# lujiarui/Str2Str

Hardware: AMD Instinct MI355X
Metric: sampled conformations/sec (whole node), 256-res chain, 100 denoise steps (higher is better)
Workload: dtype f32 (matrix products on 2-way f16 split MFMA 'f16x3': 3 products per block, fp32 accumulate, fp32-equivalent); 1 GPU; configs[1]: single 256-residue synthetic chain, 128 replicas per GPU x 100 denoise steps (+1 self-conditioning forward), probability-flow ODE, seeded synthetic weights; n_res=256, replicas_per_gpu=128, denoise_steps=100, parallelism=replica-shard x1, arith=f16x3, rng=device

## Files before the change

str2str_amd/build.py:

```python
from __future__ import annotations

import os
import shutil
import subprocess
import sys
from concurrent.futures import ThreadPoolExecutor

HERE = os.path.dirname(os.path.abspath(__file__))
ROOT = os.path.dirname(HERE)
CSRC = os.path.join(HERE, "csrc")
OBJ = os.path.join(CSRC, "build")
LIB = os.path.join(HERE, "libstr2str_hip.so")

ARCH = "gfx950"
COMMON = ["-O3", "-std=c++17", "-fPIC", f"--offload-arch={ARCH}", "-I", os.path.join(ROOT, "include"), "-I", CSRC,
          "-Wno-unused-result"]
UNITS = {
    "abi.hip": [],
    "pdb_format.cpp": [],
    "host_rng.cpp": [],
    "rigid_kernels.hip": ["-ffp-contract=off"],
    "se3_step.hip": ["-ffp-contract=off"],
    "forward_marginal.hip": ["-ffp-contract=off"],
    "ensemble_metrics.hip": ["-ffp-contract=off"],
    "ensemble_rmsd.hip": [],
    "ensemble_tm.hip": [],
    "ensemble_pca.hip": [],
    "ensemble_tica.hip": [],
    "ensemble_cluster.hip": [],
    "ensemble_lddt.hip": [],
    "ensemble_contacts.hip": ["-ffp-contract=off"],
    "ensemble_violations.hip": ["-ffp-contract=off"],
    "ensemble_ss.hip": ["-ffp-contract=off"],
    "ensemble_sasa.hip": ["-ffp-contract=off"],
    "ensemble_saxs.hip": ["-ffp-contract=off"],
    "pair_mlp.hip": ["-mllvm", "-pragma-unroll-threshold=10000000"],
    "pair_mlp_f16.hip": ["-mllvm", "-pragma-unroll-threshold=10000000", "-fno-slp-vectorize"],
    "pair_mlp_f16_b.hip": ["-mllvm", "-pragma-unroll-threshold=10000000", "-fno-slp-vectorize"],
    "pair_mlp_f16_c.hip": ["-mllvm", "-pragma-unroll-threshold=10000000", "-fno-slp-vectorize"],
    "pair_mlp_f16_d.hip": ["-mllvm", "-pragma-unroll-threshold=10000000", "-fno-slp-vectorize"],
    "pair_embed_expand.hip": [],
    "ipa_attention.hip": ["-mllvm", "-pragma-unroll-threshold=10000000"],
    "ipa_attention_f16w.hip": ["-mllvm", "-pragma-unroll-threshold=10000000", "-fno-slp-vectorize"],
    "node_gemm.hip": ["-mllvm", "-pragma-unroll-threshold=10000000", "-fno-slp-vectorize"],
    "enc_attention.hip": ["-mllvm", "-pragma-unroll-threshold=10000000", "-ffp-contract=off", "-fno-slp-vectorize"],
}


def hipcc() -> str:
    for c in (os.environ.get("HIPCC"), shutil.which("hipcc"), "/opt/rocm/bin/hipcc"):
        if c and os.path.exists(c):
            return c
    raise RuntimeError("hipcc not found (set HIPCC)")


def _stale(out: str, deps) -> bool:
    if not os.path.exists(out):
        return True
    t = os.path.getmtime(out)
    return any(os.path.getmtime(d) > t for d in deps)


def build(force: bool = False, verbose: bool = True) -> str:
    os.makedirs(OBJ, exist_ok=True)
    cc = hipcc()
    headers = [os.path.join(CSRC, f) for f in os.listdir(CSRC) if f.endswith(".h")] + [
        os.path.join(ROOT, "include", "str2str_hip.h"), os.path.abspath(__file__)]

    def compile_one(item):
        src, extra = item
        s = os.path.join(CSRC, src)
        o = os.path.join(OBJ, os.path.splitext(src)[0] + ".o")
        inc = [os.path.join(CSRC, "pair_mlp_f16.hip")] if src.startswith("pair_mlp_f16_") else []
        if force or _stale(o, [s] + inc + headers):
            if src.endswith(".cpp"):
                cmd = [cc, "-x", "c++", "-c", s, "-o", o] + [c for c in COMMON if not c.startswith("--offload-arch")] + extra
            else:
                cmd = [cc, "-x", "hip", "-c", s, "-o", o] + COMMON + extra
            if verbose:
                print(" ".join(cmd), flush=True)
            subprocess.run(cmd, check=True)
        return o

    with ThreadPoolExecutor(max_workers=min(8, len(UNITS))) as ex:
        objs = list(ex.map(compile_one, UNITS.items()))
    for f in os.listdir(OBJ):
        if f.endswith(".o") and os.path.join(OBJ, f) not in objs:
            os.remove(os.path.join(OBJ, f))
    if force or _stale(LIB, objs):
        cmd = [cc, "-shared", "-fPIC", f"--offload-arch={ARCH}", "-o", LIB] + objs
        if verbose:
            print(" ".join(cmd), flush=True)
        subprocess.run(cmd, check=True)
    return LIB


if __name__ == "__main__":
    print(build(force="--force" in sys.argv))
```

str2str_amd/csrc/pair_embed_expand.hip:

```cpp
#include <hip/hip_runtime.h>

#include <cstdlib>

#include "edge_embed_class.h"
#include "str2str_hip.h"

namespace {

typedef float f32x4 __attribute__((ext_vector_type(4)));

template <bool PROJ>
__global__ void __launch_bounds__(256) edge_embed_expand_kernel(
    const float* __restrict__ table, const int* __restrict__ fixed_cls, const float* __restrict__ bin_lower,
    const long long* __restrict__ residue_idx, const float* __restrict__ ca, const float* __restrict__ mask,
    const float* __restrict__ proj_b, float* __restrict__ out, float* __restrict__ attn_bias, float* __restrict__ pair_z,
    long long M, int N, int rel_off, int n_rel, int n_bins, int out_tiled) {
    constexpr unsigned kRec = PROJ ? s2s::kEeRecProj : s2s::kEeRecPlain;
    __shared__ __attribute__((aligned(16))) float s_bins[s2s::kEeBinSlots];
    const unsigned lane = threadIdx.x & 63, h = lane >> 5, wave = threadIdx.x >> 6;
    s2s::ee_fill_bins(s_bins, bin_lower, n_bins);
    __syncthreads();
    const long long p0 = ((long long)blockIdx.x * 4 + wave) * 32;
    if (p0 >= M) return;
    long long pl = p0 + (lane & 31);
    const bool valid = pl < M;
    pl = valid ? pl : M - 1;
    const unsigned p = (unsigned)pl;
    const unsigned bi = p / (unsigned)N, j = p - bi * (unsigned)N, bb = bi / (unsigned)N, bj = bb * (unsigned)N + j;
    const int bin = s2s::ee_pair_bin(s_bins, n_bins, ca[bi * 3 + 0], ca[bi * 3 + 1], ca[bi * 3 + 2], ca[bj * 3 + 0], ca[bj * 3 + 1], ca[bj * 3 + 2]);
    const unsigned d = (unsigned)s2s::ee_rel_row(residue_idx[bi], residue_idx[bj], rel_off, n_rel);
    const unsigned row = s2s::ee_class_row((unsigned)fixed_cls[bi], (unsigned)fixed_cls[bj], d, bin, n_rel, n_bins);
    const float em = mask ? __fmul_rn(mask[bi], mask[bj]) : 1.0f;
    const float* rec = table + (unsigned long long)row * kRec;

    if (out_tiled) {
        float* o = out + (unsigned long long)(p0 >> 5) * 4096u + lane * 4u;
        f32x4 v[16];
#pragma unroll
        for (int g = 0; g < 16; ++g) v[g] = *reinterpret_cast<const f32x4*>(rec + 8 * g + 4 * h);
#pragma unroll
        for (int g = 0; g < 16; ++g) {
            const f32x4 w = {__fmul_rn(v[g].x, em), __fmul_rn(v[g].y, em), __fmul_rn(v[g].z, em), __fmul_rn(v[g].w, em)};
            __builtin_nontemporal_store(w, reinterpret_cast<f32x4*>(o + g * 256));
        }
    } else {
        const unsigned c = lane & 31;
        f32x4 v[16];
        float e[16];
#pragma unroll
        for (int it = 0; it < 16; ++it) {
            const int n = 2 * it + (int)h;
            const unsigned rn = (unsigned)__shfl((int)row, n, 64);
            e[it] = __shfl(em, n, 64);
            v[it] = *reinterpret_cast<const f32x4*>(table + (unsigned long long)rn * kRec + 4 * c);
        }
#pragma unroll
        for (int it = 0; it < 16; ++it) {
            const long long pn = p0 + 2 * it + h;
            const f32x4 w = {__fmul_rn(v[it].x, e[it]), __fmul_rn(v[it].y, e[it]), __fmul_rn(v[it].z, e[it]), __fmul_rn(v[it].w, e[it])};
            if (pn < M) __builtin_nontemporal_store(w, reinterpret_cast<f32x4*>(out + (unsigned long long)pn * 128u + 4 * c));
        }
    }
    if constexpr (PROJ) {
        {
            f32x4 a = *reinterpret_cast<const f32x4*>(rec + 128 + 4 * h);
            const f32x4 b = *reinterpret_cast<const f32x4*>(proj_b + 4 * h);
            a = em == 0.f ? b : a;
            const long long NN = (long long)N * N;
            float* o = attn_bias + ((unsigned long long)p + 7ull * bb * (unsigned long long)NN + 4ull * h * (unsigned long long)NN);
            if (valid) { o[0] = a.x; o[NN] = a.y; o[2 * NN] = a.z; o[3 * NN] = a.w; }
        }
        const unsigned c = lane & 7;
        const f32x4 b = *reinterpret_cast<const f32x4*>(proj_b + 8 + 4 * c);
#pragma unroll
        for (int it = 0; it < 4; ++it) {
            const int n = 8 * it + (int)(lane >> 3);
            const unsigned rn = (unsigned)__shfl((int)row, n, 64);
            const float en = __shfl(em, n, 64);
            f32x4 a = *reinterpret_cast<const f32x4*>(table + (unsigned long long)rn * kRec + 136 + 4 * c);
            a = en == 0.f ? b : a;
            const long long pn = p0 + n;
            if (pn < M) *reinterpret_cast<f32x4*>(pair_z + (unsigned long long)pn * 32u + 4 * c) = a;
        }
    }
}

long long tile_aligned_samples(long long NN) {
    long long q = 32;
    while (q > 1 && (NN * (32 / q)) % 32 != 0) q /= 2;
    return 32 / q;
}

}

extern "C" int s2s_edge_embed_expand(const float* table, const int* fixed_cls, const float* bin_lower, const long long* residue_idx,
                                     const float* ca_xyz, const float* mask, const float* proj_bias_cat64, float* out, int out_tiled,
                                     float* proj_attn_bias, float* proj_pair_z, int n_samples, int n_res, int rel_offset, int n_rel,
                                     int n_bins, void* stream) {
    if (n_samples <= 0 || n_res <= 0) return 0;
    if (n_bins < 1 || n_bins > 32 || (out_tiled & ~1) || n_rel < 1) return (int)hipErrorInvalidValue;
    if ((proj_attn_bias != nullptr) != (proj_pair_z != nullptr) || (proj_attn_bias && !proj_bias_cat64)) return (int)hipErrorInvalidValue;
    const long long NN = (long long)n_res * n_res;
    if (NN >= (1ll << 31)) return (int)hipErrorInvalidValue;
    const char* cap_env = getenv("S2S_EE_MAX_PAIRS");
    long long cap = cap_env ? atoll(cap_env) : 0;
    if (cap <= 0 || cap > (1ll << 31) - 1) cap = (1ll << 31) - 1;
    long long chunk = cap / NN;
    if (out_tiled && chunk < n_samples) chunk -= chunk % tile_aligned_samples(NN);
    if (chunk < 1) return (int)hipErrorInvalidValue;
    for (long long b0 = 0; b0 < n_samples; b0 += chunk) {
        const long long nb = n_samples - b0 < chunk ? n_samples - b0 : chunk;
        const long long M = nb * NN, rows0 = b0 * n_res;
        const unsigned grid = (unsigned)((M + 127) / 128);
        const float* mk = mask ? mask + rows0 : nullptr;
        if (proj_attn_bias)
            hipLaunchKernelGGL(edge_embed_expand_kernel<true>, dim3(grid), dim3(256), 0, (hipStream_t)stream, table, fixed_cls + rows0,
                               bin_lower, residue_idx + rows0, ca_xyz + rows0 * 3, mk, proj_bias_cat64, out + b0 * NN * 128, proj_attn_bias + b0 * 8 * NN,
                               proj_pair_z + b0 * NN * 32, M, n_res, rel_offset, n_rel, n_bins, out_tiled);
        else
            hipLaunchKernelGGL(edge_embed_expand_kernel<false>, dim3(grid), dim3(256), 0, (hipStream_t)stream, table, fixed_cls + rows0,
                               bin_lower, residue_idx + rows0, ca_xyz + rows0 * 3, mk, (const float*)nullptr, out + b0 * NN * 128, (float*)nullptr,
                               (float*)nullptr, M, n_res, rel_offset, n_rel, n_bins, out_tiled);
    }
    return (int)hipGetLastError();
}
```

str2str_amd/csrc/pair_mlp_f16.hip:

```cpp
#include <hip/hip_runtime.h>

#include <cstdlib>

#include "edge_embed_class.h"
#include "f16x3.h"
#include "range_flag.h"
#include "str2str_hip.h"

#ifndef S2S_PM_PART
#define S2S_PM_PART 1
#endif

namespace {

constexpr int kStageBytes = 32 * 1024;
constexpr int kStagesBase = 30;

__device__ __forceinline__ float relu1(float x) {
    float r;
    asm("v_max_f32 %0, 0, %1" : "=v"(r) : "v"(x));
    return r;
}

struct SlotDesc { int phase, t, a, b; };
constexpr SlotDesc slot_desc(int s) {
    if (s < 8) return {0, s / 4, s % 4, 0};
    if (s < 168) {
        const int tau = s - 8, blk = tau / 16, o = tau % 16;
        if (o < 12) return {1, blk, o / 6, o % 6};
        return {0, blk + 2, o - 12, 0};
    }
    if (s < 180) return {1, 10, (s - 168) / 6, (s - 168) % 6};
    if (s < 192) return {1, 11, (s - 180) % 2, (s - 180) / 2};

    if (s < 240) return {2, 0, (s - 192) / 2, (s - 192) % 2};
    return {3, 0, s - 240, 0};
}
constexpr int sched_slot(bool proj, int ns) { return !proj ? ns : (ns < 8 ? ns : (ns < 16 ? 240 + (ns - 8) : ns - 8)); }
constexpr int blob_stage(bool proj, int st) { return !proj ? st : (st == 0 ? 0 : (st == 1 ? 30 : st - 1)); }

#define S2S_LDS_BARRIER() asm volatile("s_waitcnt lgkmcnt(0)\n\ts_barrier" ::: "memory")
__device__ float s2s_one[1] = {1.0f};


template <bool PROJ, bool STAGE>
__global__ void __launch_bounds__(256) edge_transition_f16_kernel(
    const float* __restrict__ edge, const float* __restrict__ node_ab, const float* __restrict__ node_p,
    const char* __restrict__ wblob, const float* __restrict__ b2,
    const float* __restrict__ gamma, const float* __restrict__ beta, const float* __restrict__ mask,
    float* __restrict__ out, long long M, int N, float ln_eps, int io_layout, unsigned mask_stride, const float* __restrict__ proj_b,
    float* __restrict__ proj_bias_out, float* __restrict__ proj_pz_out, int* __restrict__ range_flag, float sk) {
    constexpr int kStages = kStagesBase + (PROJ ? 1 : 0);
    constexpr int kSlots = 8 * kStages;
    constexpr int kRing = PROJ ? 4 : 2, kAhead = PROJ ? 2 : 1;
    __shared__ __attribute__((aligned(16))) char s_w[kRing][kStageBytes];
    __shared__ __attribute__((aligned(16))) float s_vec[768 + 64];
    __shared__ __attribute__((aligned(16))) float s_rows[STAGE ? 4 * 2 * 384 : 4];
    const int lane = threadIdx.x & 63, h = lane >> 5, wave = threadIdx.x >> 6;

    const unsigned voff = wave * 8192 + lane * 16;
    typedef __attribute__((address_space(3))) char lds_char;
    lds_char* lds_image[2] = {(lds_char*)&s_w[0][lane * 16], (lds_char*)&s_w[kRing / 2][lane * 16]};
    asm volatile("" : "+v"(lds_image[0]), "+v"(lds_image[1]));
    auto ring_buf = [&](int r) -> lds_char* { return PROJ ? lds_image[r >> 1] + (r & 1) * kStageBytes : lds_image[r]; };
    const __amdgpu_buffer_rsrc_t wrsrc = __builtin_amdgcn_make_buffer_rsrc((void*)wblob, 0, kStages * kStageBytes, 0x00020000);
    auto ldw = [&](unsigned vo, int so) -> f32x4 {
        const u32x4 r = __builtin_amdgcn_raw_buffer_load_b128(wrsrc, vo, so, 0);
        return f32x4{__uint_as_float(r.x), __uint_as_float(r.y), __uint_as_float(r.z), __uint_as_float(r.w)};
    };
    f32x4 c0, c1, c2, c3;
    f32x4 e0, e1, e2, e3;
    typedef __attribute__((address_space(3))) f32x4 lds_f4;
    auto cp_load_a = [&](int stage) {
        const int so = blob_stage(PROJ, stage) * kStageBytes;
        c0 = ldw(voff, so); c1 = ldw(voff + 1024, so); c2 = ldw(voff + 2048, so); c3 = ldw(voff + 3072, so);
    };
    auto cp_load_b = [&](int stage) {
        const int so = blob_stage(PROJ, stage) * kStageBytes + 4096;
        e0 = ldw(voff, so); e1 = ldw(voff + 1024, so); e2 = ldw(voff + 2048, so); e3 = ldw(voff + 3072, so);
    };
    auto cp_store_a = [&](int par) {
        lds_char* d = ring_buf(par) + wave * 8192;
        *(lds_f4*)(d) = c0; *(lds_f4*)(d + 1024) = c1; *(lds_f4*)(d + 2048) = c2; *(lds_f4*)(d + 3072) = c3;
    };
    auto cp_store_b = [&](int par) {
        lds_char* d = ring_buf(par) + (wave * 8192 + 4096);
        *(lds_f4*)(d) = e0; *(lds_f4*)(d + 1024) = e1; *(lds_f4*)(d + 2048) = e2; *(lds_f4*)(d + 3072) = e3;
    };
    auto cp_load_piece = [&](auto grp, auto kc, int stage) {
        constexpr int k = decltype(kc)::value;
        const int so = blob_stage(PROJ, stage) * kStageBytes + (decltype(grp)::value ? 4096 : 0);
        const f32x4 v = ldw(voff + 1024 * k, so);
        if constexpr (decltype(grp)::value == 0) {
            if constexpr (k == 0) c0 = v; else if constexpr (k == 1) c1 = v; else if constexpr (k == 2) c2 = v; else c3 = v;
        } else {
            if constexpr (k == 0) e0 = v; else if constexpr (k == 1) e1 = v; else if constexpr (k == 2) e2 = v; else e3 = v;
        }
    };
    auto cp_store_piece = [&](auto grp, auto kc, int par) {
        constexpr int k = decltype(kc)::value;
        lds_char* d = ring_buf(par) + (wave * 8192 + (decltype(grp)::value ? 4096 : 0) + 1024 * k);
        if constexpr (decltype(grp)::value == 0)
            *(lds_f4*)(d) = k == 0 ? c0 : (k == 1 ? c1 : (k == 2 ? c2 : c3));
        else
            *(lds_f4*)(d) = k == 0 ? e0 : (k == 1 ? e1 : (k == 2 ? e2 : e3));
    };
    cp_load_a(0);
    cp_load_b(0);

    struct PairCtx {
        unsigned p, bi, bj, boff;
        unsigned r0, aoff;
        float em_i, em_j;
        bool valid;
    };
    const unsigned NNu = (unsigned)N * (unsigned)N;
    const long long NN = (long long)N * N;
    const unsigned n_magic = N >= 2 ? (unsigned)((1ull << 32) / (unsigned)N) : 0u;
    auto div_n = [&](unsigned x, unsigned& q, unsigned& r) {
        q = N >= 2 ? __umulhi(x, n_magic) : x;
        r = x - q * (unsigned)N;
        const bool fix = r >= (unsigned)N;
        q = fix ? q + 1 : q;
        r = fix ? r - (unsigned)N : r;
    };
    auto setup = [&](long long wg_tile) -> PairCtx {
        long long pl = (wg_tile * 4 + wave) * 32 + (lane & 31);
        PairCtx c;
        c.valid = pl < M;
        if (!c.valid) pl = M - 1;
        const unsigned p = (unsigned)pl;
        unsigned bi, j, bb, i;
        div_n(p, bi, j);
        div_n(bi, bb, i);
        c.p = p;
        c.bi = bi;
        c.bj = bb * (unsigned)N + j;
        c.r0 = (unsigned)__builtin_amdgcn_readfirstlane((int)bi);
        c.aoff = (unsigned)wave * 3072u + (bi != c.r0 ? 1536u : 0u) + 16u * (unsigned)h;
        c.boff = p + 7u * bb * NNu;
        c.em_i = mask[bi * mask_stride];
        c.em_j = mask[c.bj * mask_stride];
        return c;
    };
    const bool in_tiled = io_layout & 1, out_tiled = io_layout & 2, no_out = io_layout & 4;
    const int in_step = in_tiled ? 256 : 8, out_step = out_tiled ? 256 : 8;
    auto row_of = [&](const float* base, unsigned p, bool tiled) -> const float* {
        const unsigned blk = tiled ? p >> 5 : p, mul = tiled ? 4096u : 128u;
        const unsigned in_blk = tiled ? ((lane & 32) + (p & 31)) * 4 : 4 * h;
        return base + ((unsigned long long)blk * mul + in_blk);
    };
    auto erow_of = [&](const PairCtx& c) -> const float* { return row_of(edge, c.p, in_tiled); };
    auto ldrow = [&](const float* r, int g) -> float4 {
        const f32x4 v = __builtin_nontemporal_load(reinterpret_cast<const f32x4*>(r + g * in_step));
        return make_float4(v.x, v.y, v.z, v.w);
    };
    const long long n_wt = (M + 127) / 128;
    long long wt = blockIdx.x;
    PairCtx cur = setup(wt);

    f16x8 xpl[8][2];
    float amax = 0.f;
    const float inv1 = kInvWS * sk;
    auto split4 = [&](const float (&x)[4], f16x8& ph, f16x8& pm, int at) {
        split4_f16(x, ph, pm, at, amax);
    };
    {
        float4 xv[16];
#pragma unroll
        for (int i = 0; i < 16; ++i) xv[i] = ldrow(erow_of(cur), i);
        for (int i = threadIdx.x; i < 768; i += 256)
            s_vec[i] = i < 384 ? sk * b2[i] : (i < 512 ? 0.f : (i < 640 ? gamma[i - 512] : beta[i - 640]));
        if (PROJ && threadIdx.x < 64) s_vec[768 + threadIdx.x] = proj_b[threadIdx.x];
        cp_store_a(0);
        cp_load_a(1);
        cp_store_b(0);
        if constexpr (kAhead == 2) {
            cp_load_b(1);
            cp_store_a(1);
            cp_load_a(2);
            cp_store_b(1);
        }
#pragma unroll
        for (int i = 0; i < 16; ++i) {
            const float x[4] = {xv[i].x, xv[i].y, xv[i].z, xv[i].w};
            split4(x, xpl[i >> 1][0], xpl[i >> 1][1], 4 * (i & 1));
        }
    }

    f32x16 a1t[2];
    f32x16 a2[12];
    f32x16 a3[4];
    f32x16 pq[2];
    float sa[16];
    f32x4 g_st0, g_st1, g_st2;
    const unsigned n_node_rows = (unsigned)(M / N);
    auto stage_load = [&](const PairCtx& c) {
        if constexpr (STAGE) {
            const unsigned r1 = c.r0 + 1 < n_node_rows ? c.r0 + 1 : c.r0;
            auto piece = [&](int k) -> f32x4 {
                const unsigned o = (unsigned)k * 1024u + 16u * (unsigned)lane;
                const bool second = o >= 1536u;
                const float* src = node_ab + (unsigned long long)(second ? r1 : c.r0) * 896u + ((second ? o - 1536u : o) >> 2);
                const float4 v = *reinterpret_cast<const float4*>(src);
                return f32x4{v.x, v.y, v.z, v.w};
            };
            g_st0 = piece(0); g_st1 = piece(1); g_st2 = piece(2);
        }
    };
    auto stage_store = [&]() {
        if constexpr (STAGE) {
            typedef __attribute__((address_space(3))) f32x4 lds_v4;
            lds_v4* d = (lds_v4*)((__attribute__((address_space(3))) char*)s_rows + wave * 3072 + lane * 16);
            d[0] = g_st0; d[64] = g_st1; d[128] = g_st2;
        }
    };
    auto seeds_piece = [&](const PairCtx& c, int t, int rq) {
        if constexpr (STAGE) {
            const f32x4 x = *(const lds_f4*)((__attribute__((address_space(3))) const char*)s_rows + c.aoff + (32 * t + 8 * rq) * 4);
            sa[4 * rq + 0] = x[0]; sa[4 * rq + 1] = x[1]; sa[4 * rq + 2] = x[2]; sa[4 * rq + 3] = x[3];
        } else {
            const float4 x = ldg4(node_ab + (unsigned long long)c.bi * 896u + 32 * t, rq, h);
            sa[4 * rq + 0] = x.x; sa[4 * rq + 1] = x.y; sa[4 * rq + 2] = x.z; sa[4 * rq + 3] = x.w;
        }
    };
    auto seedc_piece = [&](const PairCtx& c, int t, int rq) {
        const float4 y = ldg4(node_ab + (unsigned long long)c.bj * 896u + 384 + 32 * t, rq, h);
        a1t[t & 1][4 * rq + 0] = y.x; a1t[t & 1][4 * rq + 1] = y.y; a1t[t & 1][4 * rq + 2] = y.z; a1t[t & 1][4 * rq + 3] = y.w;
    };
    auto seeds_load = [&](const PairCtx& c, int t) {
#pragma unroll
        for (int rq = 0; rq < 4; ++rq) seeds_piece(c, t, rq);
    };
    stage_load(cur);
    stage_store();
    seeds_load(cur, 0);
#pragma unroll
    for (int rq = 0; rq < 4; ++rq) { seedc_piece(cur, 0, rq); seedc_piece(cur, 1, rq); }

    f16x8 fr[2][4];
    f16x8 xp[2][2];
    auto fetch = [&](int par, int slot_in_stage, f16x8 (&f)[4]) {
        typedef __attribute__((address_space(3))) f16x8 lds_frag;
        const lds_frag* s = (const lds_frag*)ring_buf(par) + slot_in_stage * 4 * 64;
        f[0] = s[0]; f[2] = s[128]; f[3] = s[192]; f[1] = s[64];
    };
    auto s_quarter = [&](const f32x16& tile_acc, auto qc) {
        constexpr int qd = decltype(qc)::value;
        float x[4];
#pragma unroll
        for (int j = 0; j < 4; ++j) x[j] = fmaxf(__builtin_fmaf(tile_acc[4 * qd + j], inv1, sa[4 * qd + j]), 0.f);
        split4(x, xp[qd >> 1][0], xp[qd >> 1][1], 4 * (qd & 1));
    };
    auto s_half = [&](const f32x16& tile_acc, auto qc, auto hc) {
        constexpr int qd = decltype(qc)::value, j0 = 4 * qd + 2 * decltype(hc)::value;
        const float x0 = fmaxf(__builtin_fmaf(tile_acc[j0], inv1, sa[j0]), 0.f);
        const float x1 = fmaxf(__builtin_fmaf(tile_acc[j0 + 1], inv1, sa[j0 + 1]), 0.f);
        split2_f16(x0, x1, xp[qd >> 1][0], xp[qd >> 1][1], 4 * (qd & 1) + 2 * decltype(hc)::value, amax);
    };
    float rs[64];
    auto row_load2 = [&](const float* r, float (&dst)[64], int g0) {
#pragma unroll
        for (int g = g0; g < g0 + 2; ++g) {
            const float4 v = ldg4(r, g, h);
            dst[4 * g + 0] = v.x; dst[4 * g + 1] = v.y; dst[4 * g + 2] = v.z; dst[4 * g + 3] = v.w;
        }
    };
    const f32x16 zero16 = {0.f, 0.f, 0.f, 0.f, 0.f, 0.f, 0.f, 0.f, 0.f, 0.f, 0.f, 0.f, 0.f, 0.f, 0.f, 0.f};
    S2S_LDS_BARRIER();
    fetch(0, 0, fr[0]);

    PairCtx prv = cur;
    prv.valid = false;
    prv.em_i = 0.f;
    float ln_sum = 0.f, ln_var = 0.f, ln_mean = 0.f, ln_rstd = 0.f, ln_em = 0.f;
    float* ln_orow = out;
    f16x8 xln[8][2];
    auto ln_add = [&](auto qc) {
        constexpr int q = decltype(qc)::value, t = q / 4, rq = q % 4;
#pragma unroll
        for (int j = 0; j < 4; ++j) ln_sum += a3[t][4 * rq + j];
    };
    auto ln_dev = [&](auto qc) {
        constexpr int q = decltype(qc)::value, t = q / 4, rq = q % 4;
#pragma unroll
        for (int j = 0; j < 4; ++j) {
            const float dd = a3[t][4 * rq + j] - ln_mean;
            ln_var += dd * dd;
        }
    };
    auto ln_out = [&](auto qc, const float4& ga, const float4& be) {
        constexpr int q = decltype(qc)::value, t = q / 4, rq = q % 4;
        float4 o;
        o.x = ((a3[t][4 * rq + 0] - ln_mean) * ln_rstd * ga.x + be.x) * ln_em;
        o.y = ((a3[t][4 * rq + 1] - ln_mean) * ln_rstd * ga.y + be.y) * ln_em;
        o.z = ((a3[t][4 * rq + 2] - ln_mean) * ln_rstd * ga.z + be.z) * ln_em;
        o.w = ((a3[t][4 * rq + 3] - ln_mean) * ln_rstd * ga.w + be.w) * ln_em;
        if (prv.valid && !no_out) {
            __builtin_nontemporal_store(f32x4{o.x, o.y, o.z, o.w}, reinterpret_cast<f32x4*>(ln_orow + q * out_step));
        }
        if constexpr (PROJ) {
            const float x[4] = {o.x, o.y, o.z, o.w};
            split4(x, xln[2 * t + (rq >> 1)][0], xln[2 * t + (rq >> 1)][1], 4 * (rq & 1));
        }
    };
    auto proj_store = [&](auto gc) {
        constexpr int g = decltype(gc)::value;
        if (prv.valid) {
            const float4 bq = ldg4(s_vec + 768, g, h);
            if constexpr (g == 0) {
                float* o = proj_bias_out + ((unsigned long long)prv.boff + 4 * h * NN);
                o[0] = __builtin_fmaf(pq[0][0], kInvWS, bq.x);
                o[NN] = __builtin_fmaf(pq[0][1], kInvWS, bq.y);
                o[2 * NN] = __builtin_fmaf(pq[0][2], kInvWS, bq.z);
                o[3 * NN] = __builtin_fmaf(pq[0][3], kInvWS, bq.w);
            } else {
                constexpr int t = g >> 2, rq = g & 3;
                *reinterpret_cast<float4*>(proj_pz_out + (unsigned long long)prv.p * 32u + 8 * (g - 1) + 4 * h) =
                    make_float4(__builtin_fmaf(pq[t][4 * rq + 0], kInvWS, bq.x), __builtin_fmaf(pq[t][4 * rq + 1], kInvWS, bq.y),
                                __builtin_fmaf(pq[t][4 * rq + 2], kInvWS, bq.z), __builtin_fmaf(pq[t][4 * rq + 3], kInvWS, bq.w));
            }
        }
    };
#pragma unroll
    for (int t = 0; t < 4; ++t) a3[t] = zero16;

    constexpr int kHead = PROJ ? 16 : 15;
    long long wt_next = wt;
    bool has_next = false;
    PairCtx nxt = cur;
    float4 xv[16];
    f16x8 xpn[8][2];
    f16x8 xq[8][2];
    auto slot = [&](auto sc) {
        constexpr int ns = decltype(sc)::value;
        constexpr int s = sched_slot(PROJ, ns);
        constexpr SlotDesc d = slot_desc(s);
        constexpr int stage = ns / 8, ss = ns % 8, par = stage & (kRing - 1);
        constexpr int st_next = (stage + 1) % kStages, st_fill = (stage + kAhead) % kStages;
#ifdef S2S_ET_ALL_BARRIERS
        constexpr bool barrier_here = true;
#else
        constexpr bool barrier_here = !PROJ || (st_next & 1) == 0 || st_next == kStages - 2;
#endif

        if constexpr (ss < 7) {
            fetch(par, ss + 1, fr[(ns + 1) & 1]);
        } else {
            if constexpr (barrier_here) S2S_LDS_BARRIER();
            fetch(st_next & (kRing - 1), 0, fr[(ns + 1) & 1]);
        }
        constexpr int kXv0 = 208;
        if constexpr (s == kXv0) nxt = setup(has_next ? wt_next : wt);
        if constexpr (s == kXv0 + 3) stage_load(nxt);
        if constexpr (s == kXv0 + 8) stage_store();
        if constexpr (s > kXv0 && s <= kXv0 + 16 && ((s & 3) == 1 || (s & 3) == 2)) {
            constexpr int i = 4 * ((s - kXv0) / 4) + 2 * ((s & 3) - 1);
            const float* er = erow_of(nxt);
            xv[i] = ldrow(er, i);
            xv[i + 1] = ldrow(er, i + 1);
        }
        if constexpr (s == 236) seeds_load(nxt, 0);
        if constexpr (s == 237) { seedc_piece(nxt, 0, 0); seedc_piece(nxt, 0, 1); seedc_piece(nxt, 0, 2); seedc_piece(nxt, 0, 3); }
        if constexpr (s == 238) { seedc_piece(nxt, 1, 0); seedc_piece(nxt, 1, 1); seedc_piece(nxt, 1, 2); seedc_piece(nxt, 1, 3); }
        constexpr bool seeds_slot = d.phase == 1 && d.a == 1 && d.b == 0 && d.t + 1 < 12;
        if constexpr (s >= 184 && s < 192) row_load2(node_p + (unsigned long long)cur.bi * 128u, rs, 2 * (s - 184));
        constexpr int ep_blk = (s >= 184 && s < 192) ? 0 : ((s >= 192 && s < 224) ? 1 + (s - 192) / 16 : -1);
        constexpr int ep_q = ep_blk == 0 ? 2 * (s - 184) : (s - 192) % 16;
        float4 ep_b = {0.f, 0.f, 0.f, 0.f}, ep_b1 = {0.f, 0.f, 0.f, 0.f};
        if constexpr (ep_blk >= 0) ep_b = ldg4(s_vec + 128 * ep_blk, ep_q, h);
        if constexpr (ep_blk == 0) ep_b1 = ldg4(s_vec, ep_q + 1, h);
        constexpr int ln_k = ns == 7 ? 0 : ((PROJ && d.phase == 3 && d.a < 7) ? d.a + 1 : ((!PROJ && ns >= 8 && ns < 15) ? ns - 7 : -1));
        float4 lnv[4] = {};
        if constexpr (ln_k >= 0) {
#pragma unroll
            for (int k = 0; k < 2; ++k) { lnv[2 * k] = ldg4(s_vec + 512, 2 * ln_k + k, h); lnv[2 * k + 1] = ldg4(s_vec + 640, 2 * ln_k + k, h); }
        }
        constexpr int kGSlot = 182, kGPer = 2;
        if constexpr (s >= kGSlot && s < kGSlot + 16 / kGPer) {
#pragma unroll
            for (int u = 0; u < kGPer; ++u) {
                constexpr int p0 = (s - kGSlot) * kGPer;
                const int t3 = (p0 + u) / 4, rq = (p0 + u) % 4;
                const float4 v = ldg4(node_ab + (unsigned long long)cur.bj * 896u + 768 + 32 * t3, rq, h);
                a3[t3][4 * rq + 0] = v.x; a3[t3][4 * rq + 1] = v.y; a3[t3][4 * rq + 2] = v.z; a3[t3][4 * rq + 3] = v.w;
            }
        }
        __builtin_amdgcn_sched_barrier(0);

        const f16x8 (&f)[4] = fr[ns & 1];
        auto mfma_i = [&](auto ic) {
            constexpr int i = decltype(ic)::value;
            if constexpr (d.phase == 0) {
                f32x16& acc = a1t[d.t & 1];
                const f16x8 (&x)[2] = xpl[2 * d.a + (i >= 3)];
                constexpr int fa = (i == 0 ? 1 : (i < 3 ? 0 : (i == 3 ? 3 : 2))), xa = (i == 1 || i == 4) ? 1 : 0;
                acc = mfma_f16(f[fa], x[xa], acc);
            } else {
                constexpr bool fin = d.phase == 2, prj = d.phase == 3;
                constexpr bool first = i < 2 && (prj ? d.a == 0 : (fin ? false : (d.t == 0 && d.a == 0)));
                f32x16& t = prj ? pq[i & 1] : (fin ? a3[2 * d.b + (i & 1)] : a2[2 * d.b + (i & 1)]);
                const f16x8 (&x)[2] = prj ? xln[d.a] : (fin ? ((d.a >> 3) == 1 ? xq[d.a & 7] : xpl[d.a & 7]) : xp[d.a]);
                constexpr int fa = 2 * (i & 1) + (i < 2 ? 1 : 0), xa = (i == 2 || i == 3) ? 1 : 0;
                if constexpr (first) t = mfma_f16(f[fa], x[xa], zero16); else t = mfma_f16(f[fa], x[xa], t);
            }
        };
        auto ep_half = [&](auto qc, auto hc, const float4& bq) {
            constexpr int q = decltype(qc)::value, hh = decltype(hc)::value, t = q / 4, rq = q % 4, j0 = 4 * rq + 2 * hh, e0 = 4 * (rq & 1) + 2 * hh;
            const f32x16& a = a2[4 * (ep_blk < 0 ? 0 : ep_blk) + t];
            f16x8 (&P)[2] = ep_blk == 1 ? xq[2 * t + (rq >> 1)] : xpl[2 * t + (rq >> 1)];
            float r0 = 0.f, r1 = 0.f;
            if constexpr (ep_blk == 0) {
                const unsigned hw = __builtin_bit_cast(u32x4, P[0])[e0 / 2], lw = __builtin_bit_cast(u32x4, P[1])[e0 / 2];
                asm("v_fma_mix_f32 %0, %1, 1.0, %2 op_sel_hi:[1,0,1]" : "=v"(r0) : "v"(hw), "v"(lw));
                asm("v_fma_mix_f32 %0, %1, 1.0, %2 op_sel:[1,0,1] op_sel_hi:[1,0,1]" : "=v"(r1) : "v"(hw), "v"(lw));
            } else if constexpr (ep_blk == 1) {
                r0 = rs[16 * t + j0];
                r1 = rs[16 * t + j0 + 1];
            }
            float x0 = fmaxf(__builtin_fmaf(a[j0], kInvWS, hh ? bq.z : bq.x), 0.f), x1 = fmaxf(__builtin_fmaf(a[j0 + 1], kInvWS, hh ? bq.w : bq.y), 0.f);
            if constexpr (ep_blk != 2) {
                x0 = __builtin_fmaf(r0, sk, x0);
                x1 = __builtin_fmaf(r1, sk, x1);
            }
            split2_f16(x0, x1, P[0], P[1], e0, amax);
        };
        static_for<0, 6>([&](auto ic) {
            constexpr int i = decltype(ic)::value;
            mfma_i(ic);
            if constexpr (i < 4) {
                if constexpr (ss == 0) cp_load_piece(IC<1>{}, ic, st_fill);
                if constexpr (ss == 4) cp_load_piece(IC<0>{}, ic, (stage + kAhead + 1) % kStages);
                if constexpr (ss == 1) cp_store_piece(IC<0>{}, IC<3 - i>{}, st_fill & (kRing - 1));
                if constexpr (ss == 5) cp_store_piece(IC<1>{}, IC<3 - i>{}, st_fill & (kRing - 1));
            }
            if constexpr (seeds_slot && i < 4) seeds_piece(cur, d.t + 1, i);
            if constexpr (seeds_slot && i < 4 && d.t + 2 < 12) seedc_piece(cur, d.t + 2, i);
            if constexpr (d.phase == 0 && d.t >= 1 && (i == 2 || i == 4)) s_half(a1t[(d.t - 1) & 1], IC<d.a>{}, IC<(i - 2) / 2>{});
            if constexpr (ep_blk > 0 && (i == 2 || i == 4)) ep_half(IC<ep_q>{}, IC<(i - 2) / 2>{}, ep_b);
            if constexpr (ep_blk == 0 && i >= 1 && i <= 4) {
                if constexpr (i <= 2) ep_half(IC<ep_q>{}, IC<i - 1>{}, ep_b); else ep_half(IC<ep_q + 1>{}, IC<i - 3>{}, ep_b1);
            }
            if constexpr (s >= 228 && s < 236 && i >= 1 && i <= 4) {
                constexpr int k = s - 228, e = 2 * (i - 1);
                const float4 v = xv[2 * k + (e >> 2)];
                if constexpr ((e & 2) == 0) split2_f16(v.x, v.y, xpn[k][0], xpn[k][1], e, amax);
                else split2_f16(v.z, v.w, xpn[k][0], xpn[k][1], e, amax);
            }
            if constexpr (ns < 4 && i < 4) ln_add(IC<4 * ns + i>{});
            if constexpr (ns == 4 && i == 0) ln_mean = xhalf_sum(ln_sum) * (1.0f / 128);
            if constexpr ((ns == 4 || ns == 5) && (i == 1 || i == 3 || i == 5)) { ln_dev(IC<6 * (ns - 4) + i - 1>{}); ln_dev(IC<6 * (ns - 4) + i>{}); }
            if constexpr (ns == 6 && (i == 0 || i == 1)) { ln_dev(IC<12 + 2 * i>{}); ln_dev(IC<12 + 2 * i + 1>{}); }
            if constexpr (ns == 6 && i == 3) {
                ln_rstd = 1.0f / sqrtf(xhalf_sum(ln_var) * (1.0f / 128) + ln_eps * ((kWS * sk) * (kWS * sk)));
                ln_em = prv.em_i * prv.em_j;
                ln_orow = const_cast<float*>(row_of(out, prv.p, out_tiled));
                ln_sum = 0.f;
                ln_var = 0.f;
            }
            if constexpr (ln_k >= 0 && (i == 1 || i == 3)) ln_out(IC<2 * ln_k + (i - 1) / 2>{}, lnv[i - 1], lnv[i]);
            if constexpr (PROJ && ns == kHead && i < 5) proj_store(ic);
            __builtin_amdgcn_sched_barrier(0);
        });

        if constexpr (s == 179) {
            s_quarter(a1t[1], IC<0>{}); s_quarter(a1t[1], IC<1>{}); s_quarter(a1t[1], IC<2>{}); s_quarter(a1t[1], IC<3>{});
        }
    };
    for (;;) {
    wt_next = wt + gridDim.x;
    has_next = wt_next < n_wt;
    static_for<0, kSlots>(slot);

    prv = cur;
#pragma unroll
    for (int i = 0; i < 8; ++i) { xpl[i][0] = xpn[i][0]; xpl[i][1] = xpn[i][1]; }
    if (!has_next) break;
    cur = nxt;
    wt = wt_next;
    }
    static_for<0, kHead>(slot);
    if constexpr (PROJ) { proj_store(IC<0>{}); proj_store(IC<1>{}); proj_store(IC<2>{}); proj_store(IC<3>{}); proj_store(IC<4>{}); }
    s2s::range_report(range_flag, amax, s2s::kRangeEdgeTransition);
}


template <bool PROJ, bool TABLE = false>
__global__ void __launch_bounds__(256) edge_embed_f16_kernel(
    const float* __restrict__ node_a, const float* __restrict__ node_b, const float* __restrict__ rel_tab,
    const float* __restrict__ bin_tab, const float* __restrict__ bin_lower, const long long* __restrict__ residue_idx,
    const float* __restrict__ ca, const char* __restrict__ wblob, const float* __restrict__ b2, const float* __restrict__ b3,
    const float* __restrict__ gamma, const float* __restrict__ beta, const float* __restrict__ mask, float* __restrict__ out,
    long long M, int N, int rel_off, int n_rel, int n_bins, float ln_eps, int out_tiled, const float* __restrict__ proj_b,
    float* __restrict__ proj_bias_out, float* __restrict__ proj_pz_out, int* __restrict__ range_flag) {
    constexpr int kStages = PROJ ? 5 : 4;
    constexpr int kSlots = 8 * kStages;
    __shared__ __attribute__((aligned(16))) char s_w[2][kStageBytes];
    __shared__ __attribute__((aligned(16))) float s_vec[512 + 64];
    __shared__ __attribute__((aligned(16))) float s_bins[s2s::kEeBinSlots];
    const int lane = threadIdx.x & 63, h = lane >> 5, wave = threadIdx.x >> 6;

    const unsigned voff = wave * 8192 + lane * 16;
    typedef __attribute__((address_space(3))) char lds_char;
    lds_char* lds_image[2] = {(lds_char*)&s_w[0][lane * 16], (lds_char*)&s_w[1][lane * 16]};
    asm volatile("" : "+v"(lds_image[0]), "+v"(lds_image[1]));
    const __amdgpu_buffer_rsrc_t wrsrc = __builtin_amdgcn_make_buffer_rsrc((void*)wblob, 0, kStages * kStageBytes, 0x00020000);
    auto ldw = [&](unsigned vo, int so) -> f32x4 {
        const u32x4 r = __builtin_amdgcn_raw_buffer_load_b128(wrsrc, vo, so, 0);
        return f32x4{__uint_as_float(r.x), __uint_as_float(r.y), __uint_as_float(r.z), __uint_as_float(r.w)};
    };
    f32x4 c0, c1, c2, c3, e0, e1, e2, e3;
    typedef __attribute__((address_space(3))) f32x4 lds_f4;
    auto cp_load_a = [&](int stage) {
        const int so = stage * kStageBytes;
        c0 = ldw(voff, so); c1 = ldw(voff + 1024, so); c2 = ldw(voff + 2048, so); c3 = ldw(voff + 3072, so);
    };
    auto cp_load_b = [&](int stage) {
        const int so = stage * kStageBytes + 4096;
        e0 = ldw(voff, so); e1 = ldw(voff + 1024, so); e2 = ldw(voff + 2048, so); e3 = ldw(voff + 3072, so);
    };
    auto cp_store_a = [&](int par) {
        lds_char* d = lds_image[par] + wave * 8192;
        *(lds_f4*)(d + 3072) = c3; *(lds_f4*)(d + 2048) = c2; *(lds_f4*)(d + 1024) = c1; *(lds_f4*)(d) = c0;
    };
    auto cp_store_b = [&](int par) {
        lds_char* d = lds_image[par] + (wave * 8192 + 4096);
        *(lds_f4*)(d + 3072) = e3; *(lds_f4*)(d + 2048) = e2; *(lds_f4*)(d + 1024) = e1; *(lds_f4*)(d) = e0;
    };
    cp_load_a(0);
    cp_load_b(0);

    struct Ctx {
        const float* ra;
        unsigned vb, vr, vk;
        float kb;
        long long p, boff;
        float em;
        bool valid;
    };
    const long long NN = (long long)N * N;
    const __amdgpu_buffer_rsrc_t rs_b = __builtin_amdgcn_make_buffer_rsrc((void*)node_b, 0, (unsigned)((TABLE ? (long long)N : M / N) * 512), 0x00020000);
    const __amdgpu_buffer_rsrc_t rs_r = __builtin_amdgcn_make_buffer_rsrc((void*)rel_tab, 0, n_rel * 512, 0x00020000);
    const __amdgpu_buffer_rsrc_t rs_k = __builtin_amdgcn_make_buffer_rsrc((void*)bin_tab, 0, n_bins * 512, 0x00020000);
    struct Raw {
        long long p, bi, bj, bb;
        float ax, ay, az, bx, by, bz;
        long long ii, ij;
        float mi, mj;
        bool valid;
    };
    const unsigned n_magic = N >= 2 ? (unsigned)((1ull << 32) / (unsigned)N) : 0u;
    auto div_n = [&](unsigned x, unsigned& q, unsigned& r) {
        q = N >= 2 ? __umulhi(x, n_magic) : x;
        r = x - q * (unsigned)N;
        const bool fix = r >= (unsigned)N;
        q = fix ? q + 1 : q;
        r = fix ? r - (unsigned)N : r;
    };
    const float* mask_or_any = mask ? mask : ca;
    auto setup_a = [&](long long wg_tile) -> Raw {
        long long p = (wg_tile * 4 + wave) * 32 + (lane & 31);
        Raw r;
        r.valid = p < M;
        p = r.valid ? p : M - 1;
        r.p = p;
        if constexpr (TABLE) {
            const unsigned nb1 = (unsigned)n_bins + 1u, q = (unsigned)p / nb1, cls = q / (unsigned)n_rel;
            r.bi = cls >> 1; r.bj = cls & 1u; r.bb = 0;
            r.ii = q - cls * (unsigned)n_rel; r.ij = (unsigned)p - q * nb1;
            r.ax = r.ay = r.az = r.bx = r.by = r.bz = 0.f;
            r.mi = r.mj = 1.f;
            return r;
        }
        unsigned bi, j, bb, i;
        div_n((unsigned)p, bi, j);
        div_n(bi, bb, i);
        r.bi = bi; r.bb = bb; r.bj = bb * (unsigned)N + j;
        r.ax = ca[r.bi * 3 + 0]; r.ay = ca[r.bi * 3 + 1]; r.az = ca[r.bi * 3 + 2];
        r.bx = ca[r.bj * 3 + 0]; r.by = ca[r.bj * 3 + 1]; r.bz = ca[r.bj * 3 + 2];
        r.ii = residue_idx[r.bi];
        r.ij = residue_idx[r.bj];
        r.mi = mask_or_any[r.bi];
        r.mj = mask_or_any[r.bj];
        return r;
    };
    auto setup_b = [&](const Raw& r) -> Ctx {
        Ctx c;
        c.valid = r.valid;
        const int bin = TABLE ? (int)r.ij - 1 : s2s::ee_pair_bin(s_bins, n_bins, r.ax, r.ay, r.az, r.bx, r.by, r.bz);
        const long long d = TABLE ? r.ii : s2s::ee_rel_row(r.ii, r.ij, rel_off, n_rel);
        c.ra = node_a + r.bi * 128;
        const unsigned jj = (unsigned)(r.bj - r.bb * N);
        c.vb = ((unsigned)r.bb * 32u * (unsigned)N + (unsigned)h * (unsigned)N + jj) * 16u;
        c.vr = ((unsigned)h * (unsigned)n_rel + (unsigned)d) * 16u;
        c.vk = ((unsigned)h * (unsigned)n_bins + (unsigned)(bin < 0 ? 0 : bin)) * 16u;
        c.kb = bin < 0 ? 0.f : 1.f;
        c.p = r.p;
        c.boff = r.p + 7 * r.bb * NN;
        c.em = (!TABLE && mask) ? r.mi * r.mj : 1.0f;
        return c;
    };
    float amax = 0.f;
    auto split4 = [&](const float (&x)[4], f16x8& ph, f16x8& pm, int at) {
        split4_f16(x, ph, pm, at, amax);
    };
    float g1[64];
    auto row_set = [&](const float* r) {
#pragma unroll
        for (int G = 0; G < 16; ++G) {
            const float4 v = ldg4(r, G, h);
            g1[4 * G + 0] = v.x; g1[4 * G + 1] = v.y; g1[4 * G + 2] = v.z; g1[4 * G + 3] = v.w;
        }
    };
    float tmp[64];
    auto row_cb = [&](const __amdgpu_buffer_rsrc_t& rs, unsigned vo, int rows, float (&dst)[64], int G0, int G1) {
#pragma unroll
        for (int G = G0; G < G1; ++G) {
            const u32x4 v = __builtin_amdgcn_raw_buffer_load_b128(rs, vo, G * 32 * rows, 0);
            dst[4 * G + 0] = __uint_as_float(v.x); dst[4 * G + 1] = __uint_as_float(v.y);
            dst[4 * G + 2] = __uint_as_float(v.z); dst[4 * G + 3] = __uint_as_float(v.w);
        }
    };
    auto row_add = [&](float scale) {
#pragma unroll
        for (int i = 63; i >= 0; --i) {
            g1[i] = __fmaf_rn(scale, tmp[i], g1[i]);
            asm volatile("" : "+v"(g1[i]));
        }
    };
    auto g1_split = [&](f16x8 (&dst)[2], int ks) {
        const float x0[4] = {relu1(g1[8 * ks + 0]), relu1(g1[8 * ks + 1]), relu1(g1[8 * ks + 2]), relu1(g1[8 * ks + 3])};
        const float x1[4] = {relu1(g1[8 * ks + 4]), relu1(g1[8 * ks + 5]), relu1(g1[8 * ks + 6]), relu1(g1[8 * ks + 7])};
        split4(x0, dst[0], dst[1], 0);
        split4(x1, dst[0], dst[1], 4);
    };

    const long long n_wt = (M + 127) / 128;
    long long wt = blockIdx.x;
    if constexpr (!TABLE) s2s::ee_fill_bins(s_bins, bin_lower, n_bins);
    __syncthreads();
    Ctx cur = setup_b(setup_a(wt));
    f16x8 xp[8][2];
    {
        row_set(cur.ra);
        for (int i = threadIdx.x; i < 512; i += 256)
            s_vec[i] = i < 128 ? kWS * b2[i] : (i < 256 ? kWS * b3[i - 128] : (i < 384 ? gamma[i - 256] : beta[i - 384]));
        if (PROJ && threadIdx.x < 64) s_vec[512 + threadIdx.x] = proj_b[threadIdx.x];
        cp_store_a(0);
        cp_load_a(1);
        cp_store_b(0);
        row_cb(rs_b, cur.vb, N, tmp, 0, 16); row_add(1.0f);
        row_cb(rs_r, cur.vr, n_rel, tmp, 0, 16); row_add(1.0f);
        row_cb(rs_k, cur.vk, n_bins, tmp, 0, 16); row_add(cur.kb);
#pragma unroll
        for (int ks = 0; ks < 8; ++ks) g1_split(xp[ks], ks);
    }
    f32x16 a2[4], a3[4], pq[2];
    f16x8 fr[2][4];
    auto fetch = [&](int par, int slot_in_stage, f16x8 (&f)[4]) {
        typedef __attribute__((address_space(3))) f16x8 lds_frag;
        const lds_frag* s = (const lds_frag*)lds_image[par] + slot_in_stage * 4 * 64;
        f[0] = s[0]; f[2] = s[128]; f[3] = s[192]; f[1] = s[64];
    };
    const f32x16 zero16 = {0.f, 0.f, 0.f, 0.f, 0.f, 0.f, 0.f, 0.f, 0.f, 0.f, 0.f, 0.f, 0.f, 0.f, 0.f, 0.f};
    auto pin_frag = [&](f16x8 (&x)[2]) { asm volatile("" : "+v"(x[0]), "+v"(x[1])); };
    auto bias16 = [&](const float* vec, int t) -> f32x16 {
        const float4 b0 = ldg4(vec, 4 * t, h), b1 = ldg4(vec, 4 * t + 1, h), b2v = ldg4(vec, 4 * t + 2, h), b3v = ldg4(vec, 4 * t + 3, h);
        return f32x16{b0.x, b0.y, b0.z, b0.w, b1.x, b1.y, b1.z, b1.w, b2v.x, b2v.y, b2v.z, b2v.w, b3v.x, b3v.y, b3v.z, b3v.w};
    };
    auto l2_piece = [&](auto kc) {
        constexpr int k = decltype(kc)::value, t = k / 2;
#pragma unroll
        for (int u = 0; u < 2; ++u) {
            const int rq = 2 * (k & 1) + u;
            const float xx[4] = {relu1(a2[t][4 * rq + 0]) * kInvWS, relu1(a2[t][4 * rq + 1]) * kInvWS,
                                 relu1(a2[t][4 * rq + 2]) * kInvWS, relu1(a2[t][4 * rq + 3]) * kInvWS};
            split4(xx, xp[k][0], xp[k][1], 4 * u);
        }
        pin_frag(xp[k]);
    };
    float ln_mean = 0.f, ln_rstd = 0.f;
    constexpr unsigned kRec = TABLE ? (PROJ ? s2s::kEeRecProj : s2s::kEeRecPlain) : 128u;
    const unsigned out_lane = out_tiled ? lane * 16u : (unsigned)((lane & 31) * (kRec * 4) + h * 16), out_step = out_tiled ? 1024u : 32u;
    f16x8 xq[2][2];
    __amdgpu_buffer_rsrc_t rs_out;
    auto out_rsrc = [&](long long wg_tile) {
        const long long p0 = (wg_tile * 4 + __builtin_amdgcn_readfirstlane(wave)) * 32;
        const long long left = M - p0;
        rs_out = __builtin_amdgcn_make_buffer_rsrc((void*)(out + (p0 < M ? p0 : 0) * kRec), 0,
                                                   (unsigned)(left <= 0 ? 0 : (left < 32 && !out_tiled ? left : 32)) * (kRec * 4u), 0x00020000);
    };
    float4 lga[2], lbe[2];
    auto ln_load = [&](auto kc) {
        constexpr int k = decltype(kc)::value;
#pragma unroll
        for (int u = 0; u < 2; ++u) {
            const int g = 4 * (k / 2) + 2 * (k & 1) + u;
            lga[u] = ldg4(s_vec + 256, g, h);
            lbe[u] = ldg4(s_vec + 384, g, h);
        }
    };
    auto ln_piece = [&](auto kc, const Ctx& c) {
        constexpr int k = decltype(kc)::value, t = k / 2;
#pragma unroll
        for (int u = 0; u < 2; ++u) {
            const int rq = 2 * (k & 1) + u, g = 4 * t + rq;
            const float4 ga = lga[u], be = lbe[u];
            float4 o;
            o.x = __fmul_rn(__fmaf_rn(__fmul_rn(a3[t][4 * rq + 0] - ln_mean, ln_rstd), ga.x, be.x), c.em);
            o.y = __fmul_rn(__fmaf_rn(__fmul_rn(a3[t][4 * rq + 1] - ln_mean, ln_rstd), ga.y, be.y), c.em);
            o.z = __fmul_rn(__fmaf_rn(__fmul_rn(a3[t][4 * rq + 2] - ln_mean, ln_rstd), ga.z, be.z), c.em);
            o.w = __fmul_rn(__fmaf_rn(__fmul_rn(a3[t][4 * rq + 3] - ln_mean, ln_rstd), ga.w, be.w), c.em);
            __builtin_amdgcn_raw_buffer_store_b128(u32x4{__float_as_uint(o.x), __float_as_uint(o.y), __float_as_uint(o.z), __float_as_uint(o.w)},
                                                   rs_out, out_lane + (unsigned)g * out_step, 0, 0);
            if constexpr (PROJ) {
                const float xx[4] = {o.x, o.y, o.z, o.w};
                split4(xx, xq[k & 1][0], xq[k & 1][1], 4 * u);
            }
        }
        if constexpr (PROJ) pin_frag(xq[k & 1]);
    };
    auto row_load8 = [&](const float* r, float (&dst)[64], int half) {
#pragma unroll
        for (int G = 8 * half; G < 8 * half + 8; ++G) {
            const float4 v = ldg4(r, G, h);
            dst[4 * G + 0] = v.x; dst[4 * G + 1] = v.y; dst[4 * G + 2] = v.z; dst[4 * G + 3] = v.w;
        }
    };
    S2S_LDS_BARRIER();
    fetch(0, 0, fr[0]);
    f32x16 initA0 = bias16(s_vec, 0), initA1 = bias16(s_vec, 1), initB0, initB1;
    Raw nraw = setup_a(wt + gridDim.x < n_wt ? wt + gridDim.x : wt);

    for (;;) {
    const long long wt_next = wt + gridDim.x;
    const bool has_next = wt_next < n_wt;
    Ctx nxt = cur;
    f16x8 xl[2];
    static_for<0, kSlots>([&](auto sc) {
        constexpr int s = decltype(sc)::value;
        constexpr int stage = s / 8, ss = s % 8, par = stage & 1;
        constexpr int layer = s / 16;
        constexpr int ks = layer < 2 ? (s % 16) / 2 : s - 32;
        constexpr int pr = layer < 2 ? s % 2 : 0;
        if constexpr (s == kSlots - 1) { initA0 = bias16(s_vec, 0); initA1 = bias16(s_vec, 1); }
        if constexpr (s == 0) { initB0 = bias16(s_vec, 2); initB1 = bias16(s_vec, 3); }
        if constexpr (s == 15) { initA0 = bias16(s_vec + 128, 0); initA1 = bias16(s_vec + 128, 1); }
        if constexpr (s == 16) { initB0 = bias16(s_vec + 128, 2); initB1 = bias16(s_vec + 128, 3); }
        if constexpr (PROJ && s >= 31 && s < 39) ln_load(IC<s - 31>{});
        if constexpr (ss < 7) {
            fetch(par, ss + 1, fr[(s + 1) & 1]);
        } else {
            S2S_LDS_BARRIER();
            fetch(par ^ 1, 0, fr[(s + 1) & 1]);
        }
        if constexpr (s == 30) out_rsrc(wt);
        if constexpr (s == 5) row_load8(nxt.ra, g1, 0);
        if constexpr (s == 6) row_load8(nxt.ra, g1, 1);
        if constexpr (s == 7) row_cb(rs_b, nxt.vb, N, tmp, 0, 8);
        if constexpr (s == 8) row_cb(rs_b, nxt.vb, N, tmp, 8, 16);
        if constexpr (s == 13) row_cb(rs_r, nxt.vr, n_rel, tmp, 0, 8);
        if constexpr (s == 14) row_cb(rs_r, nxt.vr, n_rel, tmp, 8, 16);
        if constexpr (s == 18) row_cb(rs_k, nxt.vk, n_bins, tmp, 0, 8);
        if constexpr (s == 19) row_cb(rs_k, nxt.vk, n_bins, tmp, 8, 16);
        __builtin_amdgcn_sched_barrier(0);

        const f16x8 (&f)[4] = fr[s & 1];
        const f16x8 (&x)[2] = layer < 2 ? xp[ks] : xq[ks & 1];
        f32x16& t0 = layer == 0 ? a2[2 * pr] : (layer == 1 ? a3[2 * pr] : pq[0]);
        f32x16& t1 = layer == 0 ? a2[2 * pr + 1] : (layer == 1 ? a3[2 * pr + 1] : pq[1]);
        if constexpr (ks == 0) {
            if constexpr (layer < 2) {
                t0 = mfma_f16(f[1], x[0], pr == 0 ? initA0 : initB0); t1 = mfma_f16(f[3], x[0], pr == 0 ? initA1 : initB1);
            } else {
                t0 = mfma_f16(f[1], x[0], zero16); t1 = mfma_f16(f[3], x[0], zero16);
            }
        } else {
            t0 = mfma_f16(f[1], x[0], t0); t1 = mfma_f16(f[3], x[0], t1);
        }
        t0 = mfma_f16(f[0], x[1], t0); t1 = mfma_f16(f[2], x[1], t1);
        t0 = mfma_f16(f[0], x[0], t0); t1 = mfma_f16(f[2], x[0], t1);
        if constexpr (s == 1) nxt = setup_b(nraw);
        if constexpr (s == 26) nraw = setup_a(wt_next + gridDim.x < n_wt ? wt_next + gridDim.x : wt_next);
        if constexpr (s == 12) row_add(1.0f);
        if constexpr (s == 17) row_add(1.0f);
        if constexpr (s == 22) row_add(nxt.kb);
        if constexpr (s >= 16 && s <= 28 && s % 2 == 0) l2_piece(IC<(s - 14) / 2>{});
        if constexpr (s == 15) l2_piece(IC<0>{});
        if constexpr (s >= 24 && s < 31) { g1_split(xp[s - 24], s - 24); pin_frag(xp[s - 24]); }
        if constexpr (s == 23) { g1_split(xl, 7); pin_frag(xl); }
        if constexpr (PROJ && s >= 32 && s < 39) ln_piece(IC<s - 31>{}, cur);
        if constexpr (ss == 0) cp_load_b((stage + 1) % kStages);
        if constexpr (ss == 4) cp_load_a((stage + 2) % kStages);
        if constexpr (ss == 1) cp_store_a(par ^ 1);
        if constexpr (ss == 5) cp_store_b(par ^ 1);
        constexpr int copy_kind = (ss == 0 || ss == 4) ? 0x020 : ((ss == 1 || ss == 5) ? 0x200 : 0);
#pragma unroll
        for (int i = 0; i < 6; ++i) {
            __builtin_amdgcn_sched_group_barrier(0x008, 1, 0);
            if (copy_kind != 0 && i < 4) __builtin_amdgcn_sched_group_barrier(copy_kind, 1, 0);
            __builtin_amdgcn_sched_group_barrier(0x002, 8, 0);
        }
        __builtin_amdgcn_sched_barrier(0);

        if constexpr (s == 31) {
            float sum = 0.f;
#pragma unroll
            for (int t = 0; t < 4; ++t)
#pragma unroll
                for (int r = 0; r < 16; ++r) sum += a3[t][r];
            ln_mean = __fmul_rn(xhalf_sum(sum), 1.0f / 128);
            float var = 0.f;
#pragma unroll
            for (int t = 0; t < 4; ++t)
#pragma unroll
                for (int r = 0; r < 16; ++r) {
                    const float dd = a3[t][r] - ln_mean;
                    var = __fmaf_rn(dd, dd, var);
                }
            ln_rstd = 1.0f / sqrtf(__fmaf_rn(xhalf_sum(var), 1.0f / 128, ln_eps * (kWS * kWS)));
            if constexpr (PROJ) {
                ln_piece(IC<0>{}, cur);
            } else {
                static_for<0, 8>([&](auto kc) { ln_load(kc); ln_piece(kc, cur); });
            }
        }
    });
    if constexpr (PROJ) {
        if (cur.valid) {
            const float4 b0 = ldg4(s_vec + 512, 0, h);
            float* o = TABLE ? out + cur.p * kRec + 128 + 4 * h : proj_bias_out + cur.boff + 4 * h * NN;
            const long long hs = TABLE ? 1 : NN;
            float* pz = TABLE ? out + cur.p * kRec + 136 : proj_pz_out + cur.p * 32;
            o[0] = __builtin_fmaf(pq[0][0], kInvWS, b0.x);
            o[hs] = __builtin_fmaf(pq[0][1], kInvWS, b0.y);
            o[2 * hs] = __builtin_fmaf(pq[0][2], kInvWS, b0.z);
            o[3 * hs] = __builtin_fmaf(pq[0][3], kInvWS, b0.w);
#pragma unroll
            for (int g = 1; g <= 4; ++g) {
                const int t = g >> 2, rq = g & 3;
                const float4 bq = ldg4(s_vec + 512, g, h);
                *reinterpret_cast<float4*>(pz + 8 * (g - 1) + 4 * h) =
                    make_float4(__builtin_fmaf(pq[t][4 * rq + 0], kInvWS, bq.x), __builtin_fmaf(pq[t][4 * rq + 1], kInvWS, bq.y),
                                __builtin_fmaf(pq[t][4 * rq + 2], kInvWS, bq.z), __builtin_fmaf(pq[t][4 * rq + 3], kInvWS, bq.w));
            }
        }
    }
    if (!has_next) break;
    cur = nxt;
    wt = wt_next;
    xp[7][0] = xl[0]; xp[7][1] = xl[1];
    if constexpr (kStages % 2 == 1) {
        lds_char* sw = lds_image[0];
        lds_image[0] = lds_image[1];
        lds_image[1] = sw;
    }
    }
    s2s::range_report(range_flag, amax, s2s::kRangeEdgeEmbed);
}


long long tile_aligned_samples(long long NN) {
    long long q = 32;
    while (q > 1 && (NN * (32 / q)) % 32 != 0) q /= 2;
    return 32 / q;
}

int cu_count() {
    int dev = 0, n_cu = 0;
    if (hipGetDevice(&dev) != hipSuccess || hipDeviceGetAttribute(&n_cu, hipDeviceAttributeMultiprocessorCount, dev) != hipSuccess || n_cu <= 0)
        return 256;
    return n_cu;
}

template <bool STAGE>
int et_launch(const float* edge, const float* node_ab, const float* node_p, const void* weight_stream, const float* b2,
              const float* ln_gamma, const float* ln_beta, const float* mask, float* out, int n_samples, int n_res, float ln_eps,
              int io_layout, const float* proj_bias_cat64, float* proj_attn_bias, float* proj_pair_z, int prescale_exp, int* range_words,
              void* stream) {
    if (n_samples <= 0 || n_res <= 0) return 0;
    if ((io_layout & ~7) || ((io_layout & 4) && !proj_attn_bias) || (!(io_layout & 4) && !out)) return (int)hipErrorInvalidValue;
    if (prescale_exp < 0 || prescale_exp > 15) return (int)hipErrorInvalidValue;
    const float sk = ldexpf(1.0f, -prescale_exp);
    const long long NN = (long long)n_res * n_res;
    const char* cap_env = getenv("S2S_ET_MAX_PAIRS");
    long long cap = cap_env ? atoll(cap_env) : 0;
    if (cap <= 0 || cap > (1ll << 29) - 1) cap = (1ll << 29) - 1;
    long long chunk = cap / NN;
    if ((io_layout & 3) && chunk < n_samples) chunk -= chunk % tile_aligned_samples(NN);
    if (chunk < 1) return (int)hipErrorInvalidValue;
    const float* one = nullptr;
    if (hipGetSymbolAddress((void**)&one, HIP_SYMBOL(s2s_one)) != hipSuccess) return (int)hipErrorInvalidValue;
    const int n_cu = cu_count();
    for (long long b0 = 0; b0 < n_samples; b0 += chunk) {
        const long long nb = n_samples - b0 < chunk ? n_samples - b0 : chunk;
        const long long M = nb * NN, rows0 = b0 * n_res;
        const long long wg_tiles = (M + 127) / 128;
        const long long grid = wg_tiles < n_cu ? wg_tiles : n_cu;
        const float* e = edge + b0 * NN * 128;
        const float* nab = node_ab + rows0 * 896;
        const float* np = node_p + rows0 * 128;
        const float* mk = mask ? mask + rows0 : one;
        const unsigned mks = mask ? 1u : 0u;
        float* o = out ? out + b0 * NN * 128 : nullptr;
        auto k_proj = &edge_transition_f16_kernel<true, STAGE>;
        auto k_plain = &edge_transition_f16_kernel<false, STAGE>;
        if (proj_attn_bias)
            hipLaunchKernelGGL(k_proj, dim3((unsigned)grid), dim3(256), 0, (hipStream_t)stream, e, nab, np,
                               (const char*)weight_stream, b2, ln_gamma, ln_beta, mk, o, M, n_res, ln_eps, io_layout, mks, proj_bias_cat64,
                               proj_attn_bias + b0 * 8 * NN, proj_pair_z + b0 * NN * 32, range_words, sk);
        else
            hipLaunchKernelGGL(k_plain, dim3((unsigned)grid), dim3(256), 0, (hipStream_t)stream, e, nab, np,
                               (const char*)weight_stream, b2, ln_gamma, ln_beta, mk, o, M, n_res, ln_eps, io_layout, mks,
                               (const float*)nullptr, (float*)nullptr, (float*)nullptr, range_words, sk);
    }
    return (int)hipGetLastError();
}

}

#define S2S_ET_ARGS const float* edge, const float* node_ab, const float* node_p, const void* weight_stream, const float* b2, \
                    const float* ln_gamma, const float* ln_beta, const float* mask, float* out, int n_samples, int n_res, float ln_eps, \
                    int io_layout, const float* proj_bias_cat64, float* proj_attn_bias, float* proj_pair_z, int prescale_exp, \
                    int* range_words, void* stream
#define S2S_ET_PASS edge, node_ab, node_p, weight_stream, b2, ln_gamma, ln_beta, mask, out, n_samples, n_res, ln_eps, io_layout, \
                    proj_bias_cat64, proj_attn_bias, proj_pair_z, prescale_exp, range_words, stream
extern "C" __attribute__((visibility("hidden"))) int s2s_et_f16x3_short_chains(S2S_ET_ARGS);
#if S2S_PM_PART == 2
extern "C" int s2s_et_f16x3_short_chains(S2S_ET_ARGS) { return et_launch<false>(S2S_ET_PASS); }
#endif
#if S2S_PM_PART == 1
extern "C" int s2s_edge_transition_f16x3(S2S_ET_ARGS) {
    return n_res >= 32 ? et_launch<true>(S2S_ET_PASS) : s2s_et_f16x3_short_chains(S2S_ET_PASS);
}
#endif

#if S2S_PM_PART == 3
extern "C" int s2s_edge_embed_f16x3(const float* node_a, const float* node_b, const float* rel_table, const float* bin_table,
                                     const float* bin_lower, const long long* residue_idx, const float* ca_xyz,
                                     const void* weight_stream, const float* b2, const float* b3, const float* ln_gamma,
                                     const float* ln_beta, const float* mask, float* out, int n_samples, int n_res,
                                     int rel_offset, int n_rel, int n_bins, float ln_eps, int out_tiled, const float* proj_bias_cat64,
                                     float* proj_attn_bias, float* proj_pair_z, int* range_words, void* stream) {
    if (n_samples <= 0 || n_res <= 0) return 0;
    if (n_bins > 32 || (out_tiled & ~1)) return (int)hipErrorInvalidValue;
    const long long NN = (long long)n_res * n_res;
    if (NN >= (1ll << 31) || (long long)n_rel * 512 >= (1ll << 32)) return (int)hipErrorInvalidValue;
    const char* cap_env = getenv("S2S_EE_MAX_PAIRS");
    long long cap = cap_env ? atoll(cap_env) : 0;
    if (cap <= 0 || cap > (1ll << 31) - 1) cap = (1ll << 31) - 1;
    long long chunk = cap / NN;
    const long long rows_cap = ((1ll << 32) - 1) / ((long long)n_res * 512);
    if (rows_cap < chunk) chunk = rows_cap;
    if (out_tiled && chunk < n_samples) chunk -= chunk % tile_aligned_samples(NN);
    if (chunk < 1) return (int)hipErrorInvalidValue;
    const int n_cu = cu_count();
    for (long long b0 = 0; b0 < n_samples; b0 += chunk) {
        const long long nb = n_samples - b0 < chunk ? n_samples - b0 : chunk;
        const long long M = nb * NN, rows0 = b0 * n_res;
        const long long wg_tiles = (M + 127) / 128;
        const long long grid = wg_tiles < n_cu ? wg_tiles : n_cu;
        const float* na = node_a + rows0 * 128;
        const float* nbp = node_b + rows0 * 128;
        const long long* ridx = residue_idx + rows0;
        const float* cap = ca_xyz + rows0 * 3;
        const float* mk = mask ? mask + rows0 : nullptr;
        float* o = out + b0 * NN * 128;
        if (proj_attn_bias)
            hipLaunchKernelGGL(edge_embed_f16_kernel<true>, dim3((unsigned)grid), dim3(256), 0, (hipStream_t)stream, na, nbp,
                               rel_table, bin_table, bin_lower, ridx, cap, (const char*)weight_stream, b2, b3, ln_gamma, ln_beta,
                               mk, o, M, n_res, rel_offset, n_rel, n_bins, ln_eps, out_tiled, proj_bias_cat64,
                               proj_attn_bias + b0 * 8 * NN, proj_pair_z + b0 * NN * 32, range_words);
        else
            hipLaunchKernelGGL(edge_embed_f16_kernel<false>, dim3((unsigned)grid), dim3(256), 0, (hipStream_t)stream, na, nbp,
                               rel_table, bin_table, bin_lower, ridx, cap, (const char*)weight_stream, b2, b3, ln_gamma, ln_beta,
                               mk, o, M, n_res, rel_offset, n_rel, n_bins, ln_eps, out_tiled, (const float*)nullptr, (float*)nullptr,
                               (float*)nullptr, range_words);
    }
    return (int)hipGetLastError();
}
#endif

#if S2S_PM_PART == 4
extern "C" int s2s_edge_embed_classes_f16x3(const float* node_a2, const float* node_b2, const float* rel_table, const float* bin_table,
                                             const void* weight_stream, const float* b2, const float* b3, const float* ln_gamma,
                                             const float* ln_beta, float* table, int n_fixed, int n_rel, int n_bins, float ln_eps,
                                             const float* proj_bias_cat64, int* range_words, void* stream) {
    if (n_fixed < 1 || n_fixed > 2 || n_rel < 1 || n_bins < 1 || n_bins > 32) return (int)hipErrorInvalidValue;
    const long long M = (long long)(n_fixed == 2 ? 4 : 1) * n_rel * (n_bins + 1);
    if (M * s2s::kEeRecProj * 4 >= (1ll << 32) || (long long)n_rel * 512 >= (1ll << 32)) return (int)hipErrorInvalidValue;
    const long long wg_tiles = (M + 127) / 128;
    const int n_cu = cu_count();
    const long long grid = wg_tiles < n_cu ? wg_tiles : n_cu;
    if (proj_bias_cat64)
        hipLaunchKernelGGL((edge_embed_f16_kernel<true, true>), dim3((unsigned)grid), dim3(256), 0, (hipStream_t)stream, node_a2, node_b2,
                           rel_table, bin_table, (const float*)nullptr, (const long long*)nullptr, (const float*)nullptr,
                           (const char*)weight_stream, b2, b3, ln_gamma, ln_beta, (const float*)nullptr, table, M, n_fixed, 0, n_rel, n_bins,
                           ln_eps, 0, proj_bias_cat64, (float*)nullptr, (float*)nullptr, range_words);
    else
        hipLaunchKernelGGL((edge_embed_f16_kernel<false, true>), dim3((unsigned)grid), dim3(256), 0, (hipStream_t)stream, node_a2, node_b2,
                           rel_table, bin_table, (const float*)nullptr, (const long long*)nullptr, (const float*)nullptr,
                           (const char*)weight_stream, b2, b3, ln_gamma, ln_beta, (const float*)nullptr, table, M, n_fixed, 0, n_rel, n_bins,
                           ln_eps, 0, (const float*)nullptr, (float*)nullptr, (float*)nullptr, range_words);
    return (int)hipGetLastError();
}
#endif
```

str2str_amd/models/net/denoising_ipa.py:

```python
from __future__ import annotations

import math
import os
from functools import partial
from typing import Optional

import torch
import torch.nn.functional as F
from torch import nn

from ... import ops
from ...arith import default_arith
from ...common.all_atom import compute_backbone
from ...common.rigid_utils import Rigid
from .ipa import TranslationIPA
from .layers import DerivedCache, centred


def get_positional_embedding(indices: torch.Tensor, embedding_dim: int, max_len: int = 2056) -> torch.Tensor:
    K = torch.arange(embedding_dim // 2, device=indices.device)
    arg = indices[..., None] * math.pi / (max_len ** (2 * K[None] / embedding_dim))
    return torch.cat([torch.sin(arg), torch.cos(arg)], dim=-1)


def get_timestep_embedding(timesteps: torch.Tensor, embedding_dim: int, max_len: int = 10000) -> torch.Tensor:
    assert timesteps.ndim == 1
    timesteps = timesteps * max_len
    half = embedding_dim // 2
    freq = torch.exp(torch.arange(half, dtype=torch.float, device=timesteps.device) * -(math.log(max_len) / (half - 1)))
    emb = timesteps.float()[:, None] * freq[None, :]
    emb = torch.cat([torch.sin(emb), torch.cos(emb)], dim=1)
    if embedding_dim % 2 == 1:
        emb = F.pad(emb, (0, 1), mode="constant")
    return emb


class EmbeddingModule(nn.Module):
    launch_switches = ("arith", "node_arith")
    launch_modes = ("ee_classes",)

    def __init__(self, init_embed_size: int, node_embed_size: int, edge_embed_size: int, num_bins: int = 22,
                 min_bin: float = 1e-5, max_bin: float = 20.0, self_conditioning: bool = True):
        super().__init__()
        pos_embed_size = t_embed_size = init_embed_size
        node_in = t_embed_size + 1 + pos_embed_size
        edge_in = (t_embed_size + 1) * 2 + pos_embed_size
        self.node_embed = nn.Sequential(
            nn.Linear(node_in, node_embed_size), nn.ReLU(), nn.Linear(node_embed_size, node_embed_size), nn.ReLU(),
            nn.Linear(node_embed_size, node_embed_size), nn.LayerNorm(node_embed_size),
        )
        self.self_conditioning = self_conditioning
        if self_conditioning:
            edge_in += num_bins
        self.edge_embed = nn.Sequential(
            nn.Linear(edge_in, edge_embed_size), nn.ReLU(), nn.Linear(edge_embed_size, edge_embed_size), nn.ReLU(),
            nn.Linear(edge_embed_size, edge_embed_size), nn.LayerNorm(edge_embed_size),
        )
        self.time_embed = partial(get_timestep_embedding, embedding_dim=t_embed_size)
        self.position_embed = partial(get_positional_embedding, embedding_dim=pos_embed_size)
        self._dims = (init_embed_size, num_bins, float(min_bin), float(max_bin), edge_embed_size)
        self._wcache, self._w16cache, self._proj_cache, self._idx_cache, self._fixed_cache = (DerivedCache() for _ in range(5))
        self.arith = default_arith()
        self.node_arith = default_arith()
        self.ee_classes = os.environ.get("S2S_EE_CLASSES", "auto")
        if self.ee_classes not in ("auto", "0", "1"):
            raise ValueError(f"S2S_EE_CLASSES={self.ee_classes!r}: expected auto, 0 or 1")
        self._mask01_cache = DerivedCache()

    def _weights(self):
        e0, e2, e4 = self.edge_embed[0], self.edge_embed[2], self.edge_embed[4]
        ie, nb = self._dims[0], self._dims[1]
        t1 = ie + 1

        def build():
            w0 = e0.weight.float()
            n0 = self.node_embed[0]
            wn = n0.weight.float()
            out = {
                "w_row_t": w0[:, :ie].contiguous(), "w_row_f": w0[:, ie].contiguous(),
                "w_col_t": w0[:, t1:t1 + ie].contiguous(), "w_col_f": w0[:, t1 + ie].contiguous(),
                "w_rel": w0[:, 2 * t1:2 * t1 + ie].contiguous(), "b0": e0.bias.float().contiguous(),
                "wn_t": wn[:, :ie].contiguous(), "wn_f": wn[:, ie].contiguous(), "wn_pos": wn[:, t1:t1 + ie].contiguous(),
                "bn0": n0.bias.float().contiguous(),
                "w_t_cat": torch.cat([wn[:, :ie], w0[:, :ie], w0[:, t1:t1 + ie]], dim=0).contiguous(),
                "b_t_cat": torch.cat([n0.bias.float(), e0.bias.float(), torch.zeros_like(e0.bias.float())]).contiguous(),
                "w3c": centred(e4.weight), "b3c": centred(e4.bias),
                "w2p": ops.pack_weight(e2.weight.float()), "w3p": ops.pack_weight(centred(e4.weight)),
                "node_mlp": [ops.pack_node_layer(self.node_embed[2].weight, self.node_embed[2].bias),
                             ops.pack_node_layer(self.node_embed[4].weight, self.node_embed[4].bias, True)],
            }
            if self.self_conditioning:
                out["bin_tab"] = w0[:, 2 * t1 + ie:2 * t1 + ie + nb].t().contiguous()
            else:
                out["bin_tab"] = w0.new_zeros(1, w0.shape[0])
            out["bin_tab_cb"] = ops.column_blocked(out["bin_tab"])
            out["bin_lower"] = torch.linspace(self._dims[2], self._dims[3], nb).to(w0.device)
            return out

        ne = self.node_embed
        return self._wcache.get([e0.weight, e0.bias, e2.weight, e4.weight, e4.bias, ne[0].weight, ne[0].bias, ne[2].weight, ne[2].bias,
                                 ne[4].weight, ne[4].bias], build)

    def _fixed_terms(self, fixed_mask: torch.Tensor, w: dict, dev, node_pos: torch.Tensor):
        def build():
            fixed = fixed_mask.to(dev)[..., None].float()
            B, L = fixed.shape[:2]
            vals = torch.unique(fixed).cpu().tolist()
            cls = None
            if vals and all(v in (0.0, 1.0) for v in vals):
                f2 = torch.tensor(vals, device=dev, dtype=torch.float32).view(1, -1, 1)
                cls = {"n_fixed": len(vals),
                       "fixed_cls": ((fixed[..., 0] > 0) if len(vals) == 2 else torch.zeros_like(fixed[..., 0])).to(torch.int32).contiguous(),
                       "fa2": (f2 * w["w_row_f"]).contiguous(),
                       "fb2": (f2[:, None] * w["w_col_f"].view(1, 32, 1, 4)).expand(1, 32, len(vals), 4).contiguous(),
                       "nc2": torch.zeros(len(vals), w["wn_f"].shape[0], device=dev)}
            return ((fixed * w["wn_f"] + node_pos).contiguous(), (fixed * w["w_row_f"]).contiguous(),
                    ((fixed[:, None] * w["w_col_f"].view(1, 32, 1, 4)).expand(B, 32, L, 4).contiguous(), (fixed * w["w_col_f"]).contiguous()), cls)

        return self._fixed_cache.get([fixed_mask, w["wn_f"], node_pos], build)

    def _mask_is_01(self, node_mask: Optional[torch.Tensor]) -> bool:
        if node_mask is None:
            return True
        return self._mask01_cache.get([node_mask], lambda: (bool(((node_mask == 0) | (node_mask == 1)).all()),))[0]

    def time_images(self, t_emb: torch.Tensor) -> torch.Tensor:
        w = self._weights()
        t_emb = t_emb.to(w["b0"].device).reshape(-1, t_emb.shape[-1]).float()
        return ((w["w_t_cat"][None] * t_emb[:, None, :]).sum(-1) + w["b_t_cat"]).contiguous()

    def _index_tables(self, residue_idx: torch.Tensor, w_rel: torch.Tensor, wn_pos: torch.Tensor):
        return self._tables(residue_idx, w_rel, wn_pos)[:4]

    def _tables(self, residue_idx, w_rel, wn_pos):
        def build():
            idx_cpu = residue_idx.detach().cpu()
            span = int(idx_cpu.max() - idx_cpu.min())
            d = torch.arange(-span, span + 1)
            dev = w_rel.device
            rel = _table_linear(self.position_embed(d).float().to(dev), w_rel)
            node_pos = _table_linear(self.position_embed(idx_cpu).float().to(dev), wn_pos)
            return rel, span, node_pos, residue_idx.to(dev).contiguous(), ops.column_blocked(rel)

        return self._idx_cache.get([residue_idx, w_rel, wn_pos], build)

    def forward(self, *args, **kw):
        node_embed, _, edge_embed, proj = self.embed(*args, **kw)
        return (node_embed, edge_embed) if proj is None else (node_embed, edge_embed, proj)

    def embed(self, residue_idx, t, fixed_mask, self_conditioning_ca, node_mask: Optional[torch.Tensor] = None,
              next_proj=None, t_emb: Optional[torch.Tensor] = None, edge_layout: str = "rowmajor", t_img: Optional[torch.Tensor] = None):
        w = self._weights()
        dev = w["b0"].device
        if dev.type != "cuda":
            raise ops.HipLibraryError("EmbeddingModule runs on the HIP device only (no CPU fallback)")
        if self._dims[4] != 128:
            raise ops.HipLibraryError("edge_embed kernel is built for edge_embed_size=128")
        B, L = residue_idx.shape
        rel_tab, span, node_pos, idx_dev, rel_cb = self._tables(residue_idx, w["w_rel"], w["wn_pos"])
        if t_img is not None:
            t_emb = None
        elif t_emb is not None:
            t_emb = t_emb.to(dev).reshape(-1, t_emb.shape[-1])
        else:
            t_u, t_inv = torch.unique(t.detach().reshape(-1), return_inverse=True)
            t_emb = self.time_embed(t_u)[t_inv].to(dev)
        ne = self.node_embed
        mask = None if node_mask is None else node_mask.to(dev).float().contiguous()
        nn_, ne_ = w["wn_t"].shape[0], w["w_row_t"].shape[0]
        single_t = t_img is not None or t_emb.shape[0] == 1
        M = B * L
        f16 = self.arith == "f16x3"
        cls = None
        if single_t:
            per_sample = t_img is not None and t_img.ndim == 2 and t_img.shape[0] == B and B > 1
            img = (t_img if per_sample else t_img.reshape(-1)) if t_img is not None else (w["w_t_cat"] * t_emb).sum(-1) + w["b_t_cat"]
            Fn, Fa, Fb, cls = self._fixed_terms(fixed_mask, w, dev, node_pos)
            h_act, node_a, node_b = torch.ops.str2str_amd.embed_assemble(img.contiguous(), Fn, Fa, Fb[0] if f16 else Fb[1], B, L,
                                                                         self.node_arith == "f16x3", f16)
        else:
            fixed = fixed_mask.to(dev)[..., None].float()
            tl = lambda wt, b=None: _table_linear(t_emb, wt, b)
            h = F.relu(tl(w["wn_t"], w["bn0"])[:, None, :] + fixed * w["wn_f"] + node_pos)
            h_act = ops.to_act(h.reshape(M, -1).contiguous(), self.node_arith)
        nw = w["node_mlp"]
        node_embed, node_act = ops.node_apply_chain(h_act, nw, M, (True, False), ln=(ne[5].weight, ne[5].bias, ne[5].eps),
                                                          post_mask=None if mask is None else mask.reshape(M), want_xp=True)
        node_embed = node_embed.view(B, L, -1)
        if not single_t:
            node_a = (tl(w["w_row_t"], w["b0"])[:, None, :] + fixed * w["w_row_f"]).expand(B, L, -1).contiguous()
            if f16:
                node_b = (tl(w["w_col_t"]).view(-1, 32, 1, 4) + fixed[:, None] * w["w_col_f"].view(1, 32, 1, 4)).expand(B, 32, L, 4).contiguous()
            else:
                node_b = (tl(w["w_col_t"])[:, None, :] + fixed * w["w_col_f"]).expand(B, L, -1).contiguous()
        ca = self_conditioning_ca.to(dev).float().contiguous() if self.self_conditioning else node_a.new_zeros(B, L, 3)
        e2, e4, ln = self.edge_embed[2], self.edge_embed[4], self.edge_embed[5]
        if f16:
            e2w = e2.weight
            ws = self._w16cache.get([e2w, w["w3c"]], lambda: ops.pack_f16x3_embed_stream(e2w.float(), w["w3c"]))
            proj = None
            if next_proj is not None:
                stream = self._proj_cache.get([ws, next_proj["wp_f16x2"]], lambda: torch.cat([ws, next_proj["wp_f16x2"]]))
                proj = (stream, next_proj["b64"])
            by_class = cls is not None and ops.edge_embed_classes_eligible(
                self.ee_classes, self.arith, single_t and not per_sample, cls["n_fixed"], self._mask_is_01(node_mask), rel_cb.shape[1],
                w["bin_tab_cb"].shape[1], B, L)
            if by_class:
                _, node_a2, node_b2 = torch.ops.str2str_amd.embed_assemble(img.contiguous(), cls["nc2"], cls["fa2"], cls["fb2"], 1,
                                                                           cls["n_fixed"], False, True)
                edge_embed = ops.edge_embed_classes_f16x3(node_a2, node_b2, cls["fixed_cls"], rel_cb, w["bin_tab_cb"], w["bin_lower"], idx_dev,
                                                          ca, ws, e2.bias, w["b3c"], ln.weight, ln.bias, mask, span, ln.eps, proj=proj,
                                                          out_layout=edge_layout)
            else:
                edge_embed = ops.edge_embed_f16x3(node_a, node_b, rel_cb, w["bin_tab_cb"], w["bin_lower"], idx_dev, ca, ws, e2.bias,
                                                  w["b3c"], ln.weight, ln.bias, mask, span, ln.eps, proj=proj, column_blocked_tables=True,
                                                  out_layout=edge_layout)
        else:
            if edge_layout != "rowmajor":
                raise ops.HipLibraryError("EmbeddingModule: the tiled pair layout belongs to the f16x3 kernels")
            edge_embed = ops.edge_embed(node_a, node_b, rel_tab, w["bin_tab"], w["bin_lower"], idx_dev, ca, w["w2p"],
                                        w["w3p"], e2.bias, w["b3c"], ln.weight, ln.bias, mask, span, ln.eps,
                                        proj=None if next_proj is None else (next_proj["wp"], next_proj["b64"]))
        if next_proj is not None:
            edge_embed, *proj = edge_embed
            return node_embed, node_act, edge_embed, tuple(proj)
        return node_embed, node_act, edge_embed, None


def _table_linear(x: torch.Tensor, w: torch.Tensor, b: Optional[torch.Tensor] = None) -> torch.Tensor:
    layer = ops.pack_node_layer(w, b if b is not None else torch.zeros(w.shape[0], device=w.device))
    lead, n = x.shape[:-1], x.numel() // x.shape[-1]
    y, _ = ops.node_apply(x.reshape(n, x.shape[-1]).float().contiguous(), layer, n)
    return y[:, : w.shape[0]].reshape(*lead, w.shape[0]).contiguous()


class DenoisingNet(nn.Module):
    def __init__(self, embedder: nn.Module, translator: nn.Module):
        super().__init__()
        self.embedder = embedder
        self.translator = translator
        self.backbone_in_forward = True

    @staticmethod
    def blend_psi(psi: torch.Tensor, torsion_angles_sin_cos: torch.Tensor, fixed_mask: torch.Tensor) -> torch.Tensor:
        gt_psi = torsion_angles_sin_cos.to(psi.device)[..., 2, :]
        fixed_mask = fixed_mask.to(psi.device).type(torch.float)
        return gt_psi * fixed_mask[..., None] + psi * (1 - fixed_mask[..., None])

    def forward(self, batch: dict, as_tensor_7: bool = False, defer_psi_blend: bool = False) -> dict:
        dev = next(self.parameters()).device
        if dev.type != "cuda":
            raise ops.HipLibraryError(
                "DenoisingNet.forward needs the HIP device (MI355X): the sampling path has no CPU fallback")
        node_mask = batch["residue_mask"].to(dev).type(torch.float)
        fixed_mask = batch["fixed_mask"].to(dev).type(torch.float)
        fuse = getattr(self.translator, "fuse_pair_projection", False)
        et0 = self.translator.trunk["edge_transition_0"] if "edge_transition_0" in getattr(self.translator, "trunk", {}) else None
        tiled = fuse and getattr(self.embedder, "arith", None) == "f16x3" and getattr(et0, "arith", None) == "f16x3"
        node_embed, node_act, edge_embed, first_proj = self.embedder.embed(
            residue_idx=batch["residue_idx"], t=batch["t"], fixed_mask=fixed_mask, self_conditioning_ca=batch["sc_ca_t"], node_mask=node_mask,
            t_emb=batch.get("t_emb"), t_img=batch.get("t_img"), next_proj=self.translator.trunk["ipa_0"].pair_proj_weights() if fuse else None,
            **({"edge_layout": "tiled"} if tiled else {}))
        tb = dict(batch)
        tb["residue_mask"], tb["fixed_mask"] = node_mask, fixed_mask
        tb["rigids_t"] = batch["rigids_t"].to(dev)
        tb["_node_embed_act"] = node_act
        model_out = self.translator(node_embed, edge_embed, tb, **({"_first_proj": first_proj} if fuse else {}))
        if model_out.get("psi_blended") or defer_psi_blend:
            psi_pred = model_out["psi"]
        else:
            psi_pred = self.blend_psi(model_out["psi"], batch["torsion_angles_sin_cos"], fixed_mask)
        rigids_pred = model_out["out_rigids"]
        out = {"rigids": rigids_pred, "psi": psi_pred, "rigids7": model_out["out_rigids7"]}
        if defer_psi_blend and not model_out.get("psi_blended"):
            out["psi_deferred"] = True
        if self.backbone_in_forward:
            aatype = batch["aatype"].to(dev) if "aatype" in batch else None
            bb = compute_backbone(rigids_pred, psi_pred, aatype=aatype, _rigids7=model_out["out_rigids7"])
            out["atom37"], out["atom14"] = bb[0], bb[-1]
        if as_tensor_7:
            out["rigids"] = model_out["out_rigids7"]
        return out
```

str2str_amd/models/net/ipa.py:

```python
from __future__ import annotations

import math
import os
from typing import Optional

import torch
import torch.nn as nn
import torch.nn.functional as F

from ... import ops
from ...arith import default_arith
from ...common.rigid_utils import Rigid, Rotation
from .layers import BackboneUpdate, DerivedCache, EdgeTransition, Linear, NodeTransition, TorsionAngleHead


class InvariantPointAttention(nn.Module):
    launch_switches = ("arith", "fold")

    def __init__(self, c_s: int, c_z: int, c_hidden: int, no_heads: int, no_qk_points: int, no_v_points: int,
                 inf: float = 1e5, eps: float = 1e-8):
        super().__init__()
        self.c_s, self.c_z, self.c_hidden = c_s, c_z, c_hidden
        self.no_heads, self.no_qk_points, self.no_v_points = no_heads, no_qk_points, no_v_points
        self.inf, self.eps = inf, eps
        hc = c_hidden * no_heads
        self.linear_q = Linear(c_s, hc)
        self.linear_kv = Linear(c_s, 2 * hc)
        self.linear_q_points = Linear(c_s, no_heads * no_qk_points * 3)
        self.linear_kv_points = Linear(c_s, no_heads * (no_qk_points + no_v_points) * 3)
        self.linear_b = Linear(c_z, no_heads)
        self.down_z = Linear(c_z, c_z // 4)
        self.head_weights = nn.Parameter(torch.full((no_heads,), 0.541324854612918))
        self.linear_out = Linear(no_heads * (c_z // 4 + c_hidden + no_v_points * 4), c_s, init="final")
        self.softmax = nn.Softmax(dim=-1)
        self.softplus = nn.Softplus()
        self.arith = default_arith()
        self.fold = os.environ.get("S2S_IPA_FOLD", "1") != "0"
        self._last_folded = False
        self._cache, self._packs = DerivedCache(), DerivedCache()

    def _derived(self):
        def build():
            wcat = torch.cat([self.linear_b.weight, self.down_z.weight], dim=0).float()
            bcat = torch.cat([self.linear_b.bias, self.down_z.bias]).float()
            b64 = bcat.new_zeros(64)
            b64[: bcat.numel()] = bcat
            hw = F.softplus(self.head_weights.float()) * math.sqrt(1.0 / (3 * (self.no_qk_points * 9.0 / 2)))
            wcat64 = wcat.new_zeros(64, wcat.shape[1])
            wcat64[: wcat.shape[0]] = wcat
            return ops.LazyDict({"wp": ops.pack_weight(wcat), "b64": b64.contiguous(), "hw": hw.contiguous()},
                                wp_f16x2=lambda d: ops.pack_f16x2_layer(wcat64, "chain").reshape(-1).view(torch.int16).contiguous())

        return self._cache.get([self.linear_b.weight, self.linear_b.bias, self.down_z.weight, self.down_z.bias,
                                self.head_weights], build)

    def node_packs(self):
        def build():
            H, C = self.no_heads, self.c_hidden
            pk = ops.pack_node_layer
            wkv = self.linear_kv.weight.view(H, 2, C, -1)
            bkv = self.linear_kv.bias.view(H, 2, C)
            d = {"q": pk(self.linear_q.weight, self.linear_q.bias), "kv": pk(self.linear_kv.weight, self.linear_kv.bias),
                 "k": pk(wkv[:, 0].reshape(H * C, -1), bkv[:, 0].reshape(-1)),
                 "v": pk(wkv[:, 1].reshape(H * C, -1), bkv[:, 1].reshape(-1)),
                 "qp": pk(self.linear_q_points.weight, self.linear_q_points.bias),
                 "kvp": pk(self.linear_kv_points.weight, self.linear_kv_points.bias),
                 "out": pk(self.linear_out.weight, self.linear_out.bias, True)}
            if self.c_s == C:
                d.update(self._folded_packs(wkv, bkv))
            return d

        return self._packs.get([p for lin in (self.linear_q, self.linear_kv, self.linear_q_points, self.linear_kv_points,
                                              self.linear_out) for p in (lin.weight, lin.bias)], build)

    def _folded_packs(self, wkv, bkv):
        H, C, cs = self.no_heads, self.c_hidden, self.c_s
        dev = self.linear_q.weight.device
        c64 = lambda t: t.detach().double().cpu()
        wq, bq = c64(self.linear_q.weight).view(H, C, cs), c64(self.linear_q.bias).view(H, C)
        wk, wv, bv = c64(wkv[:, 0]), c64(wkv[:, 1]), c64(bkv[:, 1])
        w_qf = torch.einsum("hca,hcb->hab", wk, wq).reshape(H * cs, cs).float().to(dev)
        b_qf = torch.einsum("hca,hc->ha", wk, bq).reshape(-1).float().to(dev)
        wo = c64(self.linear_out.weight)
        wo_o = wo[:, : H * C].view(-1, H, C)
        w_of = torch.cat([torch.einsum("ohc,hca->oha", wo_o, wv).reshape(-1, H * cs), wo[:, H * C:]], dim=1).float().to(dev)
        b_of = (c64(self.linear_out.bias) + torch.einsum("ohc,hc->o", wo_o, bv)).float().to(dev)
        return {"qf": ops.pack_node_layer(w_qf, b_qf), "outf": ops.pack_node_layer(w_of, b_of, True)}

    def use_f16(self, n_res: int, n_rows: int = 0) -> bool:
        if self.arith != "f16x3":
            return False
        shape_ok = (self.c_hidden == 256 and self.no_qk_points == 8 and self.no_v_points == 12 and self.c_z // 4 == 32
                    and self.no_heads == 8)
        rows_pad = (n_rows // max(n_res, 1)) * ops.padded_len(n_res)
        return shape_ok and rows_pad * 12288 < (1 << 32) and (n_res % 32 == 0 or n_rows * n_res * 32 < (1 << 31))

    def attention_f16(self, s_xp, B: int, N: int, r7, mask, pair_proj):
        w, d, M, H = self.node_packs(), self._derived(), B * N, self.no_heads
        if self.folded:
            return self._attention_f16_folded(s_xp, B, N, r7, mask, pair_proj, w, d)
        if w["v"]["tg"] != 8:
            raise ops.HipLibraryError("s2s_node_linear_vfrag is instantiated for 8 tiles per column block")
        NP = ops.padded_len(N)
        rmap, Mo = ((NP, N), B * NP) if NP != N else (None, M)
        K = torch.ops.str2str_amd
        names = ("q", "k", "v", "qp", "kvp")
        var = {n: (("w", w[n]["tg"]) if n == "v" else ops.small_rows_variant(w[n], M)) for n in names}
        dims = [x for n in names for x in (w[n]["k"], w[n]["n"], var[n][1])]
        q_xp, k_xp, v_vf, qp, kvp = K.ipa_projections(s_xp, *[[w[n][var[n][0]], w[n]["b"]] for n in names], dims, M, Mo, *(rmap or (0, 0)))
        pts = K.ipa_prep_points_f16(r7.view(B, N, 7), qp, kvp, d["hw"], H, self.no_qk_points, self.no_v_points, self.c_hidden)
        attn_bias, pair_z = pair_proj
        feats, feats_xp = K.ipa_attention_f16w(q_xp, k_xp, v_vf, *pts, attn_bias, pair_z, mask, r7, H, self.c_hidden,
                                               self.no_qk_points, self.no_v_points, self.c_z // 4, self.inf, self.eps, True)
        c0 = H * self.c_hidden
        f2 = feats.view(M, -1)
        K.pack_planes(f2, c0, f2.shape[1] - c0, feats_xp, f2.shape[1], c0)
        return feats_xp

    def _attention_f16_folded(self, s_xp, B, N, r7, mask, pair_proj, w, d):
        M, H = B * N, self.no_heads
        NP = ops.padded_len(N)
        rmap, Mo = ((NP, N), B * NP) if NP != N else (None, M)
        K = torch.ops.str2str_amd
        names = ("qf", "qp", "kvp")
        var = {n: ops.small_rows_variant(w[n], M) for n in names}
        dims = [x for n in ("qf", None, None, "qp", "kvp") for x in ((w[n]["k"], w[n]["n"], var[n][1]) if n else (0, 0, 0))]
        q_xp, _, _, qp, kvp = K.ipa_projections(s_xp, [w["qf"][var["qf"][0]], w["qf"]["b"]], [], [], [w["qp"][var["qp"][0]], w["qp"]["b"]],
                                                [w["kvp"][var["kvp"][0]], w["kvp"]["b"]], dims, M, Mo, *(rmap or (0, 0)))
        *pts, k_sh, v_sh = K.ipa_prep_points_shared_kv(r7.view(B, N, 7), qp, kvp, d["hw"], s_xp, H, self.no_qk_points, self.no_v_points,
                                                       self.c_hidden)
        attn_bias, pair_z = pair_proj
        feats, feats_xp = K.ipa_attention_f16w(q_xp, s_xp if k_sh is None else k_sh, v_sh, *pts, attn_bias, pair_z, mask, r7, H,
                                               self.c_hidden, self.no_qk_points, self.no_v_points, self.c_z // 4, self.inf, self.eps, True)
        c0 = H * self.c_hidden
        f2 = feats.view(M, -1)
        K.pack_planes(f2, c0, f2.shape[1] - c0, feats_xp, f2.shape[1], c0)
        return feats_xp

    @property
    def folded(self) -> bool:
        return self.fold and self.c_s == self.c_hidden and self.no_heads == 8

    def out_pack(self, feats_a) -> dict:
        w = self.node_packs()
        return w["outf"] if (self.folded and self._last_folded) else w["out"]

    def attention_f32(self, s_act, B: int, N: int, r7, mask, pair_proj):
        w, d, M, H = self.node_packs(), self._derived(), B * N, self.no_heads
        lin = lambda x: ops.node_apply(s_act, x, M)[0]
        q, kv, qp, kvp = lin(w["q"]), lin(w["kv"]), lin(w["qp"]), lin(w["kvp"])
        q_pts, k_pts, v_pts = torch.ops.str2str_amd.ipa_prep_points(r7.view(B, N, 7), qp.view(B, N, -1), kvp.view(B, N, -1), H,
                                                                    self.no_qk_points, self.no_v_points)
        attn_bias, pair_z = pair_proj
        feats = ops.ipa_attention(q.view(B, N, H, -1), kv.view(B, N, H, -1), q_pts, k_pts, v_pts, attn_bias, pair_z, mask, r7,
                                  d["hw"], H, self.c_hidden, self.no_qk_points, self.no_v_points, self.c_z // 4, self.inf,
                                  self.eps, logits_inplace=True)
        return ops.pack_planes(feats.view(M, -1)) if s_act.dtype == torch.int16 else feats.view(M, -1)

    def attention(self, s_act, B: int, N: int, r7, mask, pair_proj):
        self._last_folded = False
        if s_act.dtype == torch.int16 and self.use_f16(N, B * N):
            self._last_folded = self.folded
            return self.attention_f16(s_act, B, N, r7, mask, pair_proj)
        return self.attention_f32(s_act, B, N, r7, mask, pair_proj)

    def pair_proj_weights(self):
        return self._derived()

    def forward(self, s: torch.Tensor, z: torch.Tensor, r, mask: torch.Tensor, _rigids7: Optional[torch.Tensor] = None,
                _pair_proj=None):
        if not s.is_cuda:
            raise ops.HipLibraryError("InvariantPointAttention runs on the HIP device only (no CPU fallback)")
        if self.no_heads != 8 or self.c_z != 128:
            raise ops.HipLibraryError("IPA kernels are built for the reference configuration (H=8, c_z=128)")
        d = self._derived()
        r7 = (_rigids7 if _rigids7 is not None else r.to_tensor_7()).type(torch.float32).contiguous()
        mask = mask.type(torch.float32).contiguous()
        B, N = s.shape[:2]
        pp = _pair_proj if _pair_proj is not None else ops.pair_project(z.contiguous(), d["wp"], d["b64"])
        feats_a = self.attention(ops.to_act(s.reshape(B * N, -1).float().contiguous(), self.arith), B, N, r7, mask, pp)
        out, _ = ops.node_apply(feats_a, self.out_pack(feats_a), B * N)
        return out.view(B, N, -1)


class TranslationIPA(nn.Module):
    launch_switches = ("exact_padding", "fuse_pair_projection", "arith")

    def __init__(self, c_s: int, c_z: int, coordinate_scaling: float, no_ipa_blocks: int, skip_embed_size: int,
                 transformer_num_heads: int = 4, transformer_num_layers: int = 2, c_hidden: int = 256, no_heads: int = 8,
                 no_qk_points: int = 8, no_v_points: int = 12, dropout: float = 0.0):
        super().__init__()
        self.coordinate_scaling = coordinate_scaling
        self.scale_pos = lambda x: x * coordinate_scaling
        self.scale_rigids = lambda x: x.apply_trans_fn(self.scale_pos)
        self.unscale_pos = lambda x: x / coordinate_scaling
        self.unscale_rigids = lambda x: x.apply_trans_fn(self.unscale_pos)
        self.trunk = nn.ModuleDict()
        self.num_blocks = no_ipa_blocks
        for b in range(no_ipa_blocks):
            self.trunk[f"ipa_{b}"] = InvariantPointAttention(c_s=c_s, c_z=c_z, c_hidden=c_hidden, no_heads=no_heads,
                                                            no_qk_points=no_qk_points, no_v_points=no_v_points)
            self.trunk[f"ipa_ln_{b}"] = nn.LayerNorm(c_s)
            self.trunk[f"skip_embed_{b}"] = Linear(c_s, skip_embed_size, init="final")
            d = c_s + skip_embed_size
            layer = nn.TransformerEncoderLayer(d_model=d, nhead=transformer_num_heads, dim_feedforward=d)
            self.trunk[f"transformer_{b}"] = nn.TransformerEncoder(layer, transformer_num_layers, enable_nested_tensor=False)
            self.trunk[f"linear_{b}"] = Linear(d, c_s, init="final")
            self.trunk[f"node_transition_{b}"] = NodeTransition(c_s)
            self.trunk[f"bb_update_{b}"] = BackboneUpdate(c_s)
            if b < no_ipa_blocks - 1:
                self.trunk[f"edge_transition_{b}"] = EdgeTransition(node_embed_size=c_s, edge_embed_in=c_z,
                                                                    edge_embed_out=c_z)
        self.torsion_pred = TorsionAngleHead(c_s, 1)
        self._wcache, self._mask_cache = DerivedCache(), DerivedCache()
        self.exact_padding = False
        self.fuse_pair_projection = True
        self.arith = default_arith()

    def _node_weights(self):
        def build():
            T = self.trunk
            pk = lambda lin, whole=False: ops.pack_node_layer(lin.weight, lin.bias, whole)
            out = {}
            for b in range(self.num_blocks):
                d = {"skip": pk(T[f"skip_embed_{b}"]), "lin": pk(T[f"linear_{b}"]), "bb": pk(T[f"bb_update_{b}"].linear)}
                nt = T[f"node_transition_{b}"]
                d["nt1"], d["nt2"], d["nt3"] = pk(nt.linear_1), pk(nt.linear_2), pk(nt.linear_3, True)
                d["layers"] = []
                for layer in T[f"transformer_{b}"].layers:
                    att = layer.self_attn
                    d["layers"].append({"in": ops.pack_node_layer(att.in_proj_weight, att.in_proj_bias), "o": pk(att.out_proj, True),
                                        "l1": pk(layer.linear1), "l2": pk(layer.linear2, True)})
                out[b] = d
            tp = self.torsion_pred
            out["tor"] = {"l1": pk(tp.linear_1), "l2": pk(tp.linear_2), "fin": pk(tp.linear_final)}
            return out

        return self._wcache.get(list(self.parameters()), build)

    def _mask_terms(self, residue_mask: torch.Tensor, fixed_mask: torch.Tensor):
        def build():
            node_mask = residue_mask.type(torch.float).contiguous()
            fixed = fixed_mask.type(torch.float).contiguous()
            diffuse_mask = ((1 - fixed) * node_mask).contiguous()
            pad = 1.0 - node_mask
            key_bias = (torch.where(pad > 0, float("-inf"), 0.0) if self.exact_padding else pad).float().contiguous()
            return node_mask, diffuse_mask, key_bias, fixed.reshape(-1)

        return self._mask_cache.get([residue_mask, fixed_mask], build, bool(self.exact_padding))

    def forward(self, node_embed: torch.Tensor, edge_embed: torch.Tensor, batch: dict, _first_proj=None) -> dict:
        if not node_embed.is_cuda:
            raise ops.HipLibraryError("TranslationIPA runs on the HIP device only (no CPU fallback)")
        T, W = self.trunk, self._node_weights()
        f16 = self.arith == "f16x3"
        B, N, C = node_embed.shape
        M = B * N
        dev = node_embed.device
        node_mask, diffuse_mask, key_bias, fixed_flat = self._mask_terms(batch["residue_mask"], batch["fixed_mask"])
        nm, dm = node_mask.reshape(M), diffuse_mask.reshape(M)
        init7 = batch["rigids_t"].type(torch.float).contiguous()
        curr7 = torch.ops.str2str_amd.rigid_scale_trans(init7, self.coordinate_scaling, False)
        proj = _first_proj

        def lin(x, w, **kw):
            return ops.node_apply(x, w, M, **kw)

        s_f32 = node_embed.reshape(M, C).float().contiguous()
        init_a = batch.get("_node_embed_act")
        if init_a is None or (init_a.dtype == torch.int16) != f16:
            init_a = ops.to_act(s_f32, self.arith)
        s_a = init_a
        D = C + T["skip_embed_0"].out_features
        xbuf = []
        for b in range(self.num_blocks):
            xf = torch.empty(M, D, device=dev, dtype=torch.float32)
            xbuf.append((xf, ops.xp_alloc(M, D, dev) if f16 else xf))
        skip_done = None
        if f16 and 2 <= self.num_blocks <= 6:
            skip_done = ops.node_apply_multi(init_a, [(W[b]["skip"], dict(out_f32=xbuf[b][0], out_col0=C, out_xp=xbuf[b][1], out_xp_k=D, out_xp_k0=C))
                                                      for b in range(self.num_blocks)], M)
        for b in range(self.num_blocks):
            w, ipa = W[b], T[f"ipa_{b}"]
            if proj is None:
                d = ipa._derived()
                if isinstance(edge_embed, ops.PairTiled):
                    edge_embed = ops.pair_untiled(edge_embed)
                proj = torch.ops.str2str_amd.pair_project(edge_embed.contiguous(), d["wp"], d["b64"])
            feats_a = ipa.attention(s_a, B, N, curr7, node_mask, tuple(proj))
            proj = None
            ln = T[f"ipa_ln_{b}"]
            x_f32, x_a = xbuf[b]
            lin(feats_a, ipa.out_pack(feats_a), pre_mask=nm, residual=s_f32, ln=(ln.weight, ln.bias, ln.eps), out_f32=x_f32,
                out_xp=x_a, out_xp_k=D)
            if skip_done is None:
                lin(init_a, w["skip"], out_f32=x_f32, out_col0=C, out_xp=x_a, out_xp_k=D, out_xp_k0=C)
            xf, xx = x_f32, x_a
            for layer, lw in zip(T[f"transformer_{b}"].layers, w["layers"]):
                qkv, _ = lin(xx, lw["in"])
                sa_f32, sa_xp = torch.ops.str2str_amd.encoder_attention(qkv, key_bias, B, N, layer.self_attn.num_heads, not f16, f16, self.arith)
                x1 = torch.empty(M, D, device=dev, dtype=torch.float32)
                xf, xx = ops.node_apply_chain(sa_xp if f16 else sa_f32, [lw["o"], lw["l1"], lw["l2"]], M, (False, True, False),
                                              first_residual=xf, first_out_f32=x1, first_ln=(layer.norm1.weight, layer.norm1.bias, layer.norm1.eps),
                                              residual=x1, ln=(layer.norm2.weight, layer.norm2.bias, layer.norm2.eps), want_xp=True)
            nt = T[f"node_transition_{b}"]
            n_f32 = torch.empty(M, C, device=dev, dtype=torch.float32)
            s_f32, s_a = ops.node_apply_chain(xx, [w["lin"], w["nt1"], w["nt2"], w["nt3"]], M, (False, True, True, False),
                                              first_residual=x_f32, first_out_f32=n_f32, residual=n_f32,
                                              ln=(nt.ln.weight, nt.ln.bias, nt.ln.eps), post_mask=nm, want_xp=True)
            has_et = b < self.num_blocks - 1
            et = T[f"edge_transition_{b}"] if has_et else None
            specs = [(w["bb"], dict(pre_scale=dm))]
            if has_et:
                nl = et.node_layers()
                if et.arith == "f16x3":
                    node_ab16, ab_specs = et.ab16_specs(nl, True, M, s_a.device)
                    specs += [(nl["init"], {})] + ab_specs
                else:
                    specs += [(nl["init"], {}), (nl["ab_s"], {})]
            else:
                specs += [(W["tor"]["l1"], dict(relu=True, want_f32=False, want_xp=True))]
            outs = ops.node_apply_multi(s_a, specs, M)
            upd = outs[0][0]
            curr7 = torch.ops.str2str_amd.rigid_compose_update(curr7, upd, diffuse_mask)
            if has_et:
                n_p, node_ab = outs[1][0], (node_ab16 if et.arith == "f16x3" else outs[2][0])
                nxt = T[f"ipa_{b + 1}"].pair_proj_weights() if self.fuse_pair_projection else None
                et16 = et.arith == "f16x3"
                last = b == self.num_blocks - 2
                nxt16 = (not last) and T[f"edge_transition_{b + 1}"].arith == "f16x3"
                lay = "rowmajor" if not (et16 and nxt is not None) else ("none" if last else ("tiled" if nxt16 else "rowmajor"))
                if not et16 and isinstance(edge_embed, ops.PairTiled):
                    edge_embed = ops.pair_untiled(edge_embed)
                res = et.pair_mlp(edge_embed, node_ab.view(B, N, -1), n_p.view(B, N, -1), node_mask, nxt,
                                  **({"out_layout": lay} if lay != "rowmajor" else {}), **({"ab_kernel_form": True} if et16 else {}))
                if nxt is not None:
                    edge_embed, *proj = res
                else:
                    edge_embed = res
        wt = W["tor"]
        t1 = outs[1][1]
        _, t2 = lin(t1, wt["l2"], residual=s_f32, want_f32=False, want_xp=True)
        gt = batch.get("torsion_angles_sin_cos")
        blend = gt is not None and gt.is_cuda and gt.dtype == torch.float32 and gt.ndim == 4
        psi = torch.ops.str2str_amd.torsion_head(lin(t2, wt["fin"])[0], M, True, self.torsion_pred.eps,
                                                 gt[..., 2, :] if blend else None, fixed_flat if blend else None).view(B, N, 2)
        out7 = torch.ops.str2str_amd.rigid_scale_trans(curr7, self.coordinate_scaling, True)
        return {
            "psi_blended": blend,
            "in_rigids": Rigid.from_tensor_7(init7),
            "out_rigids": Rigid(Rotation(quats=out7[..., :4], normalize_quats=False), out7[..., 4:]),
            "out_rigids7": out7,
            "psi": psi,
        }
```

str2str_amd/models/net/layers.py:

```python
from __future__ import annotations

import math
import operator
import os
from typing import Optional

import torch
import torch.nn as nn
import torch.nn.functional as F

from ... import ops
from ...arith import default_arith


def _trunc_normal_(w: torch.Tensor, scale: float):
    fan_in = w.shape[1]
    std = math.sqrt(scale / max(1, fan_in)) / 0.87962566103423978
    with torch.no_grad():
        nn.init.trunc_normal_(w, mean=0.0, std=std, a=-2.0 * std, b=2.0 * std)


class DerivedCache:

    def __init__(self):
        self._key = self._val = None
        self._src = ()

    def get(self, sources, build, *extra):
        key = (tuple([(p.data_ptr(), p._version, p.shape, p.dtype, p.device) for p in sources]), extra)
        if key != self._key or any(map(operator.is_not, self._src, sources)):
            with torch.no_grad():
                self._val = build()
            self._key, self._src = key, tuple(sources)
        return self._val

    def held(self):
        return self._val, self._src


def centred(w: torch.Tensor) -> torch.Tensor:
    w64 = w.detach().double().cpu()
    return (w64 - w64.mean(dim=0, keepdim=True)).float().to(w.device).contiguous()


class Linear(nn.Linear):
    def __init__(self, in_dim: int, out_dim: int, bias: bool = True, init: str = "default", init_fn=None):
        super().__init__(in_dim, out_dim, bias=bias)
        self._pack = DerivedCache()
        with torch.no_grad():
            if bias:
                self.bias.fill_(0)
            if init_fn is not None:
                init_fn(self.weight, self.bias)
            elif init == "default":
                _trunc_normal_(self.weight, 1.0)
            elif init == "relu":
                _trunc_normal_(self.weight, 2.0)
            elif init == "glorot":
                nn.init.xavier_uniform_(self.weight, gain=1)
            elif init == "gating":
                self.weight.fill_(0.0)
                if bias:
                    self.bias.fill_(1.0)
            elif init == "normal":
                nn.init.kaiming_normal_(self.weight, nonlinearity="linear")
            elif init == "final":
                self.weight.fill_(0.0)
            else:
                raise ValueError("Invalid init string.")

    def forward(self, x: torch.Tensor) -> torch.Tensor:
        if not x.is_cuda:
            raise ops.HipLibraryError("Linear.forward runs on the HIP device only (the package has no CPU / BLAS matrix path; "
                                      "CPU restatements live under oracle/ for the tests)")
        srcs = [self.weight] if self.bias is None else [self.weight, self.bias]
        layer = self._pack.get(srcs, lambda: ops.pack_node_layer(self.weight, self.bias))
        if self.in_features % 32:
            raise ops.HipLibraryError(f"Linear.forward: the node kernel wants in_features in multiples of 32 (got {self.in_features})")
        lead, M = x.shape[:-1], x.numel() // x.shape[-1]
        y, _ = ops.node_apply(ops.to_act(x.reshape(M, x.shape[-1]).float().contiguous(), default_arith()), layer, M)
        return y[:, : self.out_features].reshape(*lead, self.out_features)


class NodeTransition(nn.Module):
    def __init__(self, dim: int):
        super().__init__()
        self.dim = dim
        self.linear_1 = Linear(dim, dim, init="relu")
        self.linear_2 = Linear(dim, dim, init="relu")
        self.linear_3 = Linear(dim, dim, init="final")
        self.relu = nn.ReLU()
        self.ln = nn.LayerNorm(dim)

    def forward(self, s: torch.Tensor) -> torch.Tensor:
        x = F.relu(self.linear_1(s))
        x = F.relu(self.linear_2(x))
        return self.ln(self.linear_3(x) + s)


class EdgeTransition(nn.Module):
    launch_switches = ("arith", "prescale_exp")

    def __init__(self, node_embed_size: int, edge_embed_in: int, edge_embed_out: int, num_layers: int = 2,
                 node_dilation: int = 2):
        super().__init__()
        bias_embed_size = node_embed_size // node_dilation
        self.initial_embed = Linear(node_embed_size, bias_embed_size, init="relu")
        hidden = bias_embed_size * 2 + edge_embed_in
        layers = []
        for _ in range(num_layers):
            layers += [Linear(hidden, hidden, init="relu"), nn.ReLU()]
        self.trunk = nn.Sequential(*layers)
        self.final_layer = Linear(hidden, edge_embed_out, init="final")
        self.layer_norm = nn.LayerNorm(edge_embed_out)
        self._shape = (edge_embed_in, bias_embed_size, hidden, edge_embed_out, num_layers)
        self._cache, self._cache32, self._proj_cache, self._node_cache, self._c32, self._bf_cache = (DerivedCache() for _ in range(6))
        self.arith = default_arith()
        self.prescale_exp = 0

    def _packed(self):
        w1, w2, wf = self.trunk[0], self.trunk[2], self.final_layer
        ce = self._shape[0]
        return self._cache.get([w1.weight, w2.weight, wf.weight], lambda: {
            "wstream_f16": ops.pack_f16x3_stream(w1.weight[:, :ce].float(), w2.weight.float(), centred(wf.weight))})

    def _packed_f32(self):
        w1, w2, wf = self.trunk[0], self.trunk[2], self.final_layer
        ce = self._shape[0]
        return self._cache32.get([w1.weight, w2.weight, wf.weight], lambda: {
            "w1p": ops.pack_weight(w1.weight[:, :ce].float(), tile_major=True),
            "w2p": ops.pack_weight(w2.weight.float(), tile_major=True),
            "wfp": ops.pack_weight(centred(wf.weight), tile_major=True)})

    def _bf_centred(self):
        bf = self.final_layer.bias
        return self._bf_cache.get([bf], lambda: centred(bf))

    def node_layers(self):
        w1, ie, wf = self.trunk[0], self.initial_embed, self.final_layer

        def build():
            ce, cb = self._shape[0], self._shape[1]
            w_ab = torch.cat([w1.weight[:, ce:ce + cb].float(), w1.weight[:, ce + cb:].float(), centred(wf.weight[:, ce + cb:])], dim=0).contiguous()
            b_ab = torch.cat([w1.bias.float(), torch.zeros_like(w1.bias).float(), centred(wf.bias)]).contiguous()
            w64, ie64 = w_ab.detach().double().cpu(), ie.weight.detach().double().cpu()
            w_abs = (w64 @ ie64).float().to(w_ab.device)
            b_abs = (w64 @ ie.bias.detach().double().cpu() + b_ab.detach().double().cpu()).float().to(w_ab.device)
            h2 = self._shape[2]
            return {"init": ops.pack_node_layer(ie.weight, ie.bias), "ab": ops.pack_node_layer(w_ab, b_ab),
                    "ab_s": ops.pack_node_layer(w_abs, b_abs),
                    "abA": ops.pack_node_layer(w_ab[:h2].contiguous(), b_ab[:h2].contiguous()),
                    "abB": ops.pack_node_layer(w_ab[h2:].contiguous(), 32.0 * b_ab[h2:]),
                    "ab_sA": ops.pack_node_layer(w_abs[:h2].contiguous(), b_abs[:h2].contiguous()),
                    "ab_sB": ops.pack_node_layer(w_abs[h2:].contiguous(), 32.0 * b_abs[h2:])}

        return self._node_cache.get([w1.weight, w1.bias, ie.weight, ie.bias, wf.weight, wf.bias], build)

    def ab16_specs(self, nl: dict, from_s: bool, n_rows: int, device):
        ab = torch.empty(n_rows, 896, device=device, dtype=torch.float32)
        c32 = self._c32.get([], lambda: torch.full((n_rows,), 32.0, device=device, dtype=torch.float32), int(n_rows), str(device))
        ka, kb = ("ab_sA", "ab_sB") if from_s else ("abA", "abB")
        return ab, [(nl[ka], dict(out_f32=ab, out_col0=0)), (nl[kb], dict(out_f32=ab, out_col0=384, pre_scale=c32))]

    def node_parts(self, s_act, n_rows: int, kernel_form: bool = False):
        nl = self.node_layers()
        n_p, n_pa = ops.node_apply(s_act, nl["init"], n_rows, want_xp=True)
        if kernel_form:
            node_ab, specs = self.ab16_specs(nl, False, n_rows, n_p.device)
            for layer, kw in specs:
                ops.node_apply(n_pa, layer, n_rows, **kw)
        else:
            node_ab, _ = ops.node_apply(n_pa, nl["ab"], n_rows)
        return n_p, node_ab

    def forward(self, node_embed: torch.Tensor, edge_embed: torch.Tensor, edge_mask_1d: Optional[torch.Tensor] = None,
                next_proj=None):
        B, N = node_embed.shape[:2]
        n_p, node_ab = self.node_parts(ops.to_act(node_embed.reshape(B * N, -1).float().contiguous(), self.arith), B * N)
        return self.pair_mlp(edge_embed, node_ab.view(B, N, -1), n_p.view(B, N, -1), edge_mask_1d, next_proj)

    def pair_mlp(self, edge_embed, node_ab, n_p, edge_mask_1d=None, next_proj=None, out_layout: str = "rowmajor", ab_kernel_form: bool = False):
        if self._shape != (128, 128, 384, 128, 2):
            raise ops.HipLibraryError(f"EdgeTransition kernel is built for c_z=128, c_s=256 (got {self._shape})")
        mask = None if edge_mask_1d is None else edge_mask_1d.type(torch.float32).contiguous()
        if self.arith == "f16x3":
            pk = self._packed()
            proj = None
            if next_proj is not None:
                stream = self._proj_cache.get([pk["wstream_f16"], next_proj["wp_f16x2"]],
                                              lambda: torch.cat([pk["wstream_f16"], next_proj["wp_f16x2"]]))
                proj = (stream, next_proj["b64"])
            tiled_in = isinstance(edge_embed, ops.PairTiled)
            B, N = edge_embed.shape[0], edge_embed.shape[1]
            z, bias, pz = torch.ops.str2str_amd.edge_transition_f16x3_chain(
                edge_embed.buf if tiled_in else edge_embed.contiguous(), tiled_in, B, N, node_ab, n_p,
                pk["wstream_f16"] if proj is None else proj[0], self.trunk[2].bias, self.layer_norm.weight,
                self.layer_norm.bias, mask, self.layer_norm.eps, None if proj is None else proj[1], out_layout, int(self.prescale_exp),
                bool(ab_kernel_form))
            if out_layout == "tiled":
                z = ops.PairTiled(B, N, buf=z)
            return z if proj is None else (z, bias, pz)
        if out_layout != "rowmajor" or isinstance(edge_embed, ops.PairTiled) or ab_kernel_form:
            raise ops.HipLibraryError("EdgeTransition: the tiled pair layout and the scaled node_ab belong to the f16x3 kernels")
        pk = self._packed_f32()
        return ops.edge_transition(edge_embed.contiguous(), node_ab[..., :768].contiguous(), n_p, pk["w1p"], pk["w2p"], pk["wfp"],
                                   self.trunk[2].bias, self._bf_centred(), self.layer_norm.weight,
                                   self.layer_norm.bias, mask, self.layer_norm.eps,
                                   proj=None if next_proj is None else (next_proj["wp"], next_proj["b64"]))


class TorsionAngleHead(nn.Module):
    def __init__(self, in_dim: int, n_torsion_angles: int, eps: float = 1e-8):
        super().__init__()
        self.linear_1 = Linear(in_dim, in_dim, init="relu")
        self.linear_2 = Linear(in_dim, in_dim, init="relu")
        self.linear_3 = Linear(in_dim, in_dim, init="final")
        self.linear_final = Linear(in_dim, n_torsion_angles * 2, init="final")
        self.relu = nn.ReLU()
        self.eps = eps

    def forward(self, s: torch.Tensor) -> torch.Tensor:
        x = self.linear_2(F.relu(self.linear_1(s))) + s
        u = self.linear_final(x)
        return u / torch.sqrt(torch.clamp(torch.sum(u**2, dim=-1, keepdim=True), min=self.eps))


class BackboneUpdate(nn.Module):
    def __init__(self, c_s: int):
        super().__init__()
        self.c_s = c_s
        self.linear = Linear(c_s, 6, init="final")

    def forward(self, s: torch.Tensor) -> torch.Tensor:
        return self.linear(s)
```

str2str_amd/ops/__init__.py:

```python
from .attention import encoder_attention, ipa_attention, ipa_attention_f16, ipa_prep_points, ipa_prep_points_f16
from .binding import ABI_VERSION, EXPORTS, LIB_PATH, HipLibraryError, KernelTimer, WeightRangeError, load_library
from .ensemble import (CLUSTER_MAX_N, CONTACT_MAX_RES, LDDT_MAX_RES, PCA_MAX_RES, RMSD_LAUNCH_PAIRS, SASA_MAX_POINTS, SASA_MAX_RES, SAXS_MAX_Q, SAXS_MAX_RES,
                       SAXS_MAX_TYPES, SS_MAX_RES, TM_MAX_RES, VIOL_MAX_RES, apply_xform, backbone_sasa, backbone_violations, ca_aligned_mean, ca_contact_map, ca_covariance, ca_fit_transforms, ca_project, ca_contact_stats, ca_lddt_matrix, ca_native_contacts, ca_native_q, ca_lddt_per_residue, ca_pairwise_distances, ca_pwd_js, ca_rmsd_matrix,
                       ca_sample_stats, ca_scattering, ca_superpose, ca_tm_matrix, ca_tm_superpose, cluster_adjacency, cluster_gromos,
                       lddt_workspace_bytes, rmsd_row_chunk, secondary_structure, sphere_points,
                       TICA_MAX_FEATURES, feature_project, lagged_covariances, lagged_mean, tica_groups)
from .geometry import forward_marginal, frames_to_backbone, rigid_compose_update, rigid_scale_trans, se3_step, torsion_head
from .hostio import (float64_normal_outputs, format_pdb_models, host_rng_can_discard, host_rng_discard_float64_normals,
                     host_rng_fast_forward_ok, merge_pdb_files, write_pdb_models)
from .node import (CHAIN_WIDTHS, NARROW_MAX_WORK, SMALL_ROWS, embed_assemble, ipa_projections, node_apply,
                   node_apply_chain, node_apply_multi, node_chain, node_linear, node_linear_f32, node_linear_multi, node_linear_vfrag,
                   pack_planes, row_layernorm, small_rows_variant, to_act)
from .packing import (NODE_TG, LazyDict, PairTiled, act_alloc, column_blocked, fragment_order, node_tiles, pack_f16x2_layer, pack_f16x3_embed_stream,
                      pack_f16x3_stream, pack_node_layer, pack_node_weight, pack_node_weight_f32, pack_weight, padded_len, pair_tiled,
                      pair_untiled, unpack_planes, vf_alloc, xp_alloc)
from .pair import (EE_CLASS_R, edge_embed, edge_embed_class_of_row, edge_embed_class_row, edge_embed_class_rows, edge_embed_classes_eligible,
                   edge_embed_classes_f16x3, edge_embed_f16x3, edge_transition, edge_transition_f16x3, pair_project)
from .range_guard import (RANGE_BITS, RANGE_FAMILIES, range_families, range_flag, range_flag_names, range_flag_read, range_flag_reset,
                          range_headroom)
from .torch_ops import register_torch_ops

__all__ = [
    "ABI_VERSION", "EXPORTS", "LIB_PATH", "HipLibraryError", "KernelTimer", "WeightRangeError", "load_library",
    "RANGE_BITS", "RANGE_FAMILIES", "range_families", "range_flag", "range_flag_names", "range_flag_read", "range_flag_reset", "range_headroom",
    "NODE_TG", "LazyDict", "PairTiled", "act_alloc", "column_blocked", "fragment_order", "node_tiles", "pack_f16x2_layer", "pack_f16x3_embed_stream",
    "pack_f16x3_stream", "pack_node_layer", "pack_node_weight", "pack_node_weight_f32", "pack_weight", "padded_len", "pair_tiled", "pair_untiled",
    "unpack_planes", "vf_alloc", "xp_alloc",
    "edge_embed", "edge_embed_f16x3", "edge_transition", "edge_transition_f16x3", "pair_project",
    "EE_CLASS_R", "edge_embed_class_of_row", "edge_embed_class_row", "edge_embed_class_rows", "edge_embed_classes_eligible", "edge_embed_classes_f16x3",
    "encoder_attention", "ipa_attention", "ipa_attention_f16", "ipa_prep_points", "ipa_prep_points_f16",
    "CHAIN_WIDTHS", "NARROW_MAX_WORK", "SMALL_ROWS", "embed_assemble", "ipa_projections", "node_apply",
    "node_apply_chain", "node_apply_multi", "node_chain", "node_linear", "node_linear_f32", "node_linear_multi", "node_linear_vfrag", "pack_planes",
    "row_layernorm", "small_rows_variant", "to_act",
    "forward_marginal", "frames_to_backbone", "rigid_compose_update", "rigid_scale_trans", "se3_step", "torsion_head",
    "RMSD_LAUNCH_PAIRS", "apply_xform", "ca_pairwise_distances", "ca_pwd_js", "ca_rmsd_matrix", "ca_sample_stats", "ca_superpose", "rmsd_row_chunk",
    "TM_MAX_RES", "ca_tm_matrix", "ca_tm_superpose",
    "LDDT_MAX_RES", "ca_lddt_matrix", "ca_lddt_per_residue", "lddt_workspace_bytes",
    "VIOL_MAX_RES", "backbone_violations",
    "SS_MAX_RES", "secondary_structure",
    "SASA_MAX_POINTS", "SASA_MAX_RES", "backbone_sasa", "sphere_points",
    "SAXS_MAX_Q", "SAXS_MAX_RES", "SAXS_MAX_TYPES", "ca_scattering",
    "CONTACT_MAX_RES", "ca_contact_map", "ca_contact_stats", "ca_native_contacts", "ca_native_q",
    "PCA_MAX_RES", "ca_aligned_mean", "ca_covariance", "ca_fit_transforms", "ca_project",
    "TICA_MAX_FEATURES", "feature_project", "lagged_covariances", "lagged_mean", "tica_groups",
    "CLUSTER_MAX_N", "cluster_adjacency", "cluster_gromos",
    "float64_normal_outputs", "format_pdb_models", "host_rng_can_discard", "host_rng_discard_float64_normals", "host_rng_fast_forward_ok",
    "merge_pdb_files", "write_pdb_models",
    "register_torch_ops",
]

register_torch_ops()
```

str2str_amd/ops/packing.py:

```python
from typing import Optional

import torch

from .binding import HipLibraryError, WeightRangeError


def _pad_rows32(w: torch.Tensor) -> torch.Tensor:
    pad = (-w.shape[0]) % 32
    return torch.cat([w, w.new_zeros(pad, w.shape[1])], dim=0) if pad else w


def pack_weight(w: torch.Tensor, tile_major: bool = False) -> torch.Tensor:
    k = w.shape[1]
    if k % 8:
        raise ValueError("K must be a multiple of 8")
    w = _pad_rows32(w)
    t, s4 = w.shape[0] // 32, k // 8
    perm = (0, 2, 3, 1, 4) if tile_major else (2, 0, 3, 1, 4)
    return w.reshape(t, 32, s4, 2, 4).permute(*perm).contiguous().reshape(-1)


def fragment_order(w: torch.Tensor, kind: str) -> torch.Tensor:
    mout, k = w.shape
    if mout % 32 or k % 32:
        raise ValueError("Mout and K must be multiples of 32")
    T, KS = mout // 32, k // 16
    ks = torch.arange(KS)[:, None, None]
    g = torch.arange(2)[None, :, None]
    j = torch.arange(8)[None, None, :]
    if kind == "row":
        lab = 16 * ks + 8 * g + j
    elif kind == "chain":
        r = 8 * (ks & 1) + j
        lab = 32 * (ks >> 1) + (r & 3) + 8 * (r >> 2) + 4 * g
    else:
        raise ValueError(kind)
    wg = w.float()[:, lab.to(w.device)]
    return wg.reshape(T, 32, KS, 2, 8).permute(2, 0, 3, 1, 4).reshape(KS, T, 64, 8).contiguous()


def pack_f16x2_layer(w: torch.Tensor, kind: str = "chain") -> torch.Tensor:
    wmax = float(w.detach().abs().max()) if w.numel() else 0.0
    if not (32.0 * wmax < 65504.0):
        raise WeightRangeError(f"|w| up to {wmax:.4g}: 32 w does not fit f16 (f16x3 weight packing)")
    planes = fragment_order(w, kind) * 32.0
    h = planes.to(torch.float16)
    ls = (planes - h.float()).to(torch.float16)
    return torch.stack([h, ls], dim=2).contiguous()


def pack_f16x3_stream(w1_edge: torch.Tensor, w2: torch.Tensor, wf: torch.Tensor) -> torch.Tensor:
    l1, l2, lf = pack_f16x2_layer(w1_edge), pack_f16x2_layer(w2), pack_f16x2_layer(wf)
    A = lambda t: l1[:, t]
    B = lambda t: l2[2 * t:2 * t + 2]
    pieces = [A(0), A(1)]
    for t in range(10):
        pieces += [B(t), A(t + 2)]
    b11 = B(11)
    pieces += [B(10), b11.reshape(2, 6, 2, *b11.shape[2:]).transpose(0, 1), lf]
    blob = torch.cat([x.contiguous().reshape(-1) for x in pieces]).view(torch.int16).contiguous()
    assert blob.numel() * 2 == 30 * 32 * 1024, blob.numel()
    return blob


class PairTiled:
    __slots__ = ("buf", "B", "N")

    def __init__(self, B: int, N: int, device=None, buf: Optional[torch.Tensor] = None):
        self.B, self.N = int(B), int(N)
        n = -(-(self.B * self.N * self.N) // 32) * 32 * 128
        self.buf = torch.empty(n, device=device, dtype=torch.float32) if buf is None else buf
        if self.buf.numel() != n or self.buf.dtype != torch.float32 or not self.buf.is_contiguous():
            raise HipLibraryError("PairTiled: buffer must be a contiguous fp32 tensor of whole 32-pair blocks")

    shape = property(lambda self: (self.B, self.N, self.N, 128))
    device = property(lambda self: self.buf.device)
    is_cuda = property(lambda self: self.buf.is_cuda)

    def data_ptr(self):
        return self.buf.data_ptr()

    def contiguous(self):
        return self


def pair_tiled(z: torch.Tensor) -> PairTiled:
    B, N = z.shape[0], z.shape[1]
    M = B * N * N
    t = PairTiled(B, N, z.device)
    zp = torch.zeros(t.buf.numel() // 128, 128, device=z.device, dtype=torch.float32)
    zp[:M] = z.reshape(M, 128)
    t.buf.copy_(zp.view(-1, 32, 16, 2, 4).permute(0, 2, 3, 1, 4).reshape(-1))
    return t


def pair_untiled(t: PairTiled) -> torch.Tensor:
    M = t.B * t.N * t.N
    return t.buf.view(-1, 16, 2, 32, 4).permute(0, 3, 1, 2, 4).reshape(-1, 128)[:M].reshape(t.B, t.N, t.N, 128).contiguous()


def column_blocked(t: torch.Tensor) -> torch.Tensor:
    *lead, rows, ch = t.shape
    return t.reshape(*lead, rows, ch // 4, 4).transpose(-3, -2).contiguous()


def pack_f16x3_embed_stream(w2: torch.Tensor, w3: torch.Tensor) -> torch.Tensor:
    blob = torch.cat([pack_f16x2_layer(w2, "chain").reshape(-1), pack_f16x2_layer(w3, "chain").reshape(-1)])
    blob = blob.view(torch.int16).contiguous()
    assert blob.numel() * 2 == 4 * 32 * 1024
    return blob


def padded_len(n_res: int) -> int:
    return (n_res + 31) // 32 * 32


NODE_TG = (10, 8, 6, 5, 4, 2, 1)


def node_tiles(n_out: int, whole_row: bool = False) -> int:
    if n_out % 32:
        raise ValueError("n_out must be a multiple of 32 (pad the weight)")
    t = n_out // 32
    if whole_row:
        if t not in NODE_TG:
            raise HipLibraryError(f"no node_linear instantiation holds a whole row of {n_out} columns")
        return t
    return next(g for g in NODE_TG if t % g == 0)


def pack_node_weight(w: torch.Tensor, tiles_per_block: int) -> torch.Tensor:
    w, k = _pad_rows32(w), w.shape[1]
    if k % 32 or (w.shape[0] // 32) % tiles_per_block:
        raise ValueError("k_in must be a multiple of 32 and n_out/32 of tiles_per_block")
    fr = pack_f16x2_layer(w.float(), "chain")
    KS, T = fr.shape[:2]
    fr = fr.reshape(KS, T // tiles_per_block, tiles_per_block, 2, 64, 8).permute(1, 0, 2, 3, 4, 5)
    return fr.contiguous().view(torch.int16).reshape(-1)


def pack_node_weight_f32(w: torch.Tensor, tiles_per_block: int) -> torch.Tensor:
    w, k = _pad_rows32(w), w.shape[1]
    if k % 8 or (w.shape[0] // 32) % tiles_per_block:
        raise ValueError("k_in must be a multiple of 8 and n_out/32 of tiles_per_block")
    T, S4 = w.shape[0] // 32, k // 8
    fr = w.float().reshape(T // tiles_per_block, tiles_per_block, 32, S4, 2, 4).permute(0, 3, 1, 4, 2, 5)
    return fr.contiguous().reshape(-1)


def pack_node_layer(w: torch.Tensor, bias, whole_row: bool = False) -> dict:
    n_out, k = w.shape
    n_pad = -(-n_out // 32) * 32
    tg = node_tiles(n_pad, whole_row=whole_row)
    b = w.new_zeros(n_pad, dtype=torch.float32)
    if bias is not None:
        b[:n_out] = bias.detach().float()
    t = n_pad // 32
    tg_s = tg if whole_row else (2 if t % 2 == 0 else tg)
    w = w.detach()

    def blocks(d, tiles):
        return d["w"] if tiles == tg else pack_node_weight(w.float(), tiles)

    return LazyDict({"b": b.contiguous(), "n": n_pad, "k": k, "tg": tg, "tg_s": tg_s}, w=lambda d: pack_node_weight(w.float(), tg),
                    w_s=lambda d: blocks(d, tg_s), w_row=lambda d: blocks(d, t), w_n=lambda d: blocks(d, 2),
                    w32=lambda d: pack_node_weight_f32(w.float(), tg))


class LazyDict(dict):

    def __init__(self, eager: dict, **lazy):
        super().__init__(eager)
        self._lazy = lazy

    def __missing__(self, key):
        if key not in self._lazy:
            raise KeyError(key)
        self[key] = self._lazy[key](self)
        return self[key]


def xp_alloc(n_rows: int, k: int, device) -> torch.Tensor:
    return torch.empty(((n_rows + 31) // 32) * (k // 16) * 2 * 64 * 8, dtype=torch.int16, device=device)


def vf_alloc(n_rows: int, n_out: int, device) -> torch.Tensor:
    return torch.empty(((n_rows + 31) // 32) * (n_out // 32) * 2 * 2 * 64 * 8, dtype=torch.int16, device=device)


def act_alloc(n_rows: int, k: int, device, arith: str) -> torch.Tensor:
    return xp_alloc(n_rows, k, device) if arith == "f16x3" else torch.empty(n_rows, k, device=device, dtype=torch.float32)


def unpack_planes(xp: torch.Tensor, n_rows: int, k: int) -> torch.Tensor:
    KS = k // 16
    fr = xp.view(torch.float16).reshape(-1, KS, 2, 2, 32, 8).float().sum(2)
    ks = torch.arange(KS)[:, None, None]
    g = torch.arange(2)[None, :, None]
    j = torch.arange(8)[None, None, :]
    r = 8 * (ks & 1) + j
    chan = (32 * (ks >> 1) + (r & 3) + 8 * (r >> 2) + 4 * g).to(xp.device)
    out = torch.zeros(fr.shape[0], 32, k, device=xp.device)
    out[:, :, chan.reshape(-1)] = fr.permute(0, 3, 1, 2, 4).reshape(fr.shape[0], 32, -1)
    return out.reshape(-1, k)[:n_rows]
```

str2str_amd/ops/pair.py:

```python
import torch

from .binding import HipLibraryError, _check, _p, _req, _req_all, _req_opt, _stream, _timed, load_library
from .packing import PairTiled, column_blocked
from .range_guard import range_flag


def _proj_outputs(proj, B, N, dev, dtype=torch.float32, name="proj.wp"):
    if proj is None:
        return None, None, None, None
    w, b64 = proj
    _req(w, dtype, name); _req(b64, name="proj.b64")
    return w, b64, torch.empty(B, 8, N, N, device=dev, dtype=torch.float32), torch.empty(B, N, N, 32, device=dev, dtype=torch.float32)


def edge_transition_f16x3(edge, node_ab, node_p, wstream, b2, gamma, beta, mask, ln_eps=1e-5, out=None, proj=None,
                          out_layout: str = "rowmajor", prescale_exp: int = 0, ab_kernel_form: bool = False):
    lib = load_library()
    B, N = edge.shape[0], edge.shape[1]
    in_tiled = isinstance(edge, PairTiled)
    if not 0 <= int(prescale_exp) <= 15:
        raise HipLibraryError(f"edge_transition_f16x3: prescale_exp {prescale_exp} outside 0 .. 15")
    if tuple(edge.shape) != (B, N, N, 128) or tuple(node_ab.shape) != (B, N, 896) or tuple(node_p.shape) != (B, N, 128):
        raise HipLibraryError(f"edge_transition_f16x3: bad shapes (edge {tuple(edge.shape)}, node_ab {tuple(node_ab.shape)}, node_p {tuple(node_p.shape)}): "
                              "edge is [B, N, N, 128], node_p [B, N, 128] and node_ab [B, N, 896] = EdgeTransition.node_parts (row half | column half | "
                              "j-side residual through the final layer; the 768-column form of earlier ABI versions is not accepted)")
    if not ab_kernel_form or prescale_exp:
        sc = node_ab.new_ones(896)
        sc[:384] = 2.0 ** -int(prescale_exp)
        sc[384:768] = 1.0 if ab_kernel_form else 32.0
        sc[768:] = (1.0 if ab_kernel_form else 32.0) * 2.0 ** -int(prescale_exp)
        node_ab = node_ab * sc
        if not ab_kernel_form:
            node_ab[..., 768:] -= node_ab[..., 768:].mean(dim=-1, keepdim=True)
    if out_layout not in ("rowmajor", "tiled", "none") or (out_layout == "none" and proj is None):
        raise HipLibraryError(f"edge_transition_f16x3: out_layout {out_layout!r}" + (" needs proj" if out_layout == "none" else ""))
    _req(edge.buf if in_tiled else edge, name="edge")
    _req_all(node_ab=node_ab, node_p=node_p, b2=b2, gamma=gamma, beta=beta)
    pw, pb, pbias, ppz = _proj_outputs(proj, B, N, edge.device, torch.int16, "wstream")
    wstream = _req(wstream, torch.int16, "wstream") if proj is None else pw
    if wstream.numel() * 2 != (31 if proj is not None else 30) * 32 * 1024:
        raise HipLibraryError("edge_transition_f16x3: weight stream has the wrong number of stages")
    _req_opt(mask=mask)
    if out_layout == "none":
        out = None
    elif out is None:
        out = PairTiled(B, N, edge.device) if out_layout == "tiled" else torch.empty(B, N, N, 128, device=edge.device, dtype=torch.float32)
    elif out.data_ptr() == edge.data_ptr():
        raise HipLibraryError("edge_transition: out may not alias edge")
    elif isinstance(out, PairTiled) != (out_layout == "tiled"):
        raise HipLibraryError("edge_transition_f16x3: out does not have the requested layout")
    io = (1 if in_tiled else 0) | {"rowmajor": 0, "tiled": 2, "none": 4}[out_layout]
    _check(_timed("s2s_edge_transition", lambda: lib.s2s_edge_transition_f16x3(
        _p(edge.buf if in_tiled else edge), _p(node_ab), _p(node_p), _p(wstream), _p(b2), _p(gamma), _p(beta), _p(mask),
        _p(out.buf if isinstance(out, PairTiled) else out), B, N, ln_eps, io, _p(pb), _p(pbias), _p(ppz), int(prescale_exp), _p(range_flag()),
        _stream())), "s2s_edge_transition_f16x3")
    return out if proj is None else (out, pbias, ppz)


def edge_transition(edge, node_ab, node_p, w1p, w2p, wfp, b2, bf, gamma, beta, mask, ln_eps=1e-5, out=None, proj=None):
    lib = load_library()
    B, N = edge.shape[0], edge.shape[1]
    _req(edge, name="edge")
    if edge.shape != (B, N, N, 128) or node_ab.shape != (B, N, 768) or node_p.shape != (B, N, 128):
        raise HipLibraryError(f"edge_transition: bad shapes {tuple(edge.shape)} {tuple(node_ab.shape)} {tuple(node_p.shape)}")
    _req_all(node_ab=node_ab, node_p=node_p, w1p=w1p, w2p=w2p, wfp=wfp, b2=b2, bf=bf, gamma=gamma, beta=beta)
    _req_opt(mask=mask)
    if out is None:
        out = torch.empty_like(edge)
    elif out.data_ptr() == edge.data_ptr():
        raise HipLibraryError("edge_transition: out may not alias edge")
    _req(out, name="out")
    pw, pb, pbias, ppz = _proj_outputs(proj, B, N, edge.device)
    _check(_timed("s2s_edge_transition", lambda: lib.s2s_edge_transition(
        _p(edge), _p(node_ab), _p(node_p), _p(w1p), _p(w2p), _p(wfp), _p(b2), _p(bf), _p(gamma), _p(beta), _p(mask),
        _p(out), B, N, ln_eps, _p(pw), _p(pb), _p(pbias), _p(ppz), _stream())), "s2s_edge_transition")
    return out if proj is None else (out, pbias, ppz)


def edge_embed(node_a, node_b, rel_table, bin_table, bin_lower, residue_idx, ca, w2p, w3p, b2, b3, gamma, beta, mask,
               rel_offset: int, ln_eps=1e-5, out=None, proj=None):
    lib = load_library()
    B, N = node_a.shape[0], node_a.shape[1]
    _req_all(node_a=node_a, node_b=node_b, rel_table=rel_table, bin_table=bin_table, bin_lower=bin_lower, ca=ca, w2p=w2p, w3p=w3p, b2=b2, b3=b3,
             gamma=gamma, beta=beta)
    _req(residue_idx, torch.int64, "residue_idx")
    _req_opt(mask=mask)
    out = torch.empty(B, N, N, 128, device=node_a.device, dtype=torch.float32) if out is None else out
    pw, pb, pbias, ppz = _proj_outputs(proj, B, N, node_a.device)
    _check(lib.s2s_edge_embed(_p(node_a), _p(node_b), _p(rel_table), _p(bin_table), _p(bin_lower), _p(residue_idx), _p(ca),
                              _p(w2p), _p(w3p), _p(b2), _p(b3), _p(gamma), _p(beta), _p(mask), _p(out), B, N,
                              int(rel_offset), rel_table.shape[0], bin_table.shape[0], ln_eps, _p(pw), _p(pb), _p(pbias),
                              _p(ppz), _stream()), "s2s_edge_embed")
    return out if proj is None else (out, pbias, ppz)


def edge_embed_f16x3(node_a, node_b, rel_table, bin_table, bin_lower, residue_idx, ca, wstream, b2, b3, gamma, beta, mask,
                     rel_offset: int, ln_eps=1e-5, out=None, proj=None, column_blocked_tables=False, out_layout: str = "rowmajor"):
    lib = load_library()
    B, N = node_a.shape[0], node_a.shape[1]
    if not column_blocked_tables:
        node_b, rel_table, bin_table = column_blocked(node_b), column_blocked(rel_table), column_blocked(bin_table)
    if node_b.shape != (B, 32, N, 4) or rel_table.shape[0] != 32 or bin_table.shape[0] != 32:
        raise HipLibraryError("edge_embed_f16x3: tables are not column-blocked [.., 32, rows, 4]")
    _req_all(node_a=node_a, node_b=node_b, rel_table=rel_table, bin_table=bin_table, bin_lower=bin_lower, ca=ca, b2=b2, b3=b3, gamma=gamma, beta=beta)
    _req(residue_idx, torch.int64, "residue_idx")
    pw, pb, pbias, ppz = _proj_outputs(proj, B, N, node_a.device, torch.int16, "wstream")
    wstream = _req(wstream, torch.int16, "wstream") if proj is None else pw
    if wstream.numel() * 2 != (5 if proj is not None else 4) * 32 * 1024:
        raise HipLibraryError("s2s_edge_embed_f16x3: weight stream has the wrong number of stages")
    _req_opt(mask=mask)
    if out_layout not in ("rowmajor", "tiled"):
        raise HipLibraryError(f"edge_embed_f16x3: out_layout {out_layout!r}")
    tiled = out_layout == "tiled"
    if out is None:
        out = PairTiled(B, N, node_a.device) if tiled else torch.empty(B, N, N, 128, device=node_a.device, dtype=torch.float32)
    elif isinstance(out, PairTiled) != tiled:
        raise HipLibraryError("edge_embed_f16x3: out does not have the requested layout")
    _check(_timed("s2s_edge_embed", lambda: lib.s2s_edge_embed_f16x3(
        _p(node_a), _p(node_b), _p(rel_table), _p(bin_table), _p(bin_lower), _p(residue_idx), _p(ca), _p(wstream), _p(b2), _p(b3),
        _p(gamma), _p(beta), _p(mask), _p(out.buf if tiled else out), B, N, int(rel_offset), rel_table.shape[1], bin_table.shape[1],
        ln_eps, 1 if tiled else 0, _p(pb), _p(pbias), _p(ppz), _p(range_flag()), _stream())), "s2s_edge_embed_f16x3")
    return out if proj is None else (out, pbias, ppz)


EE_CLASS_R = 12


def edge_embed_class_rows(n_fixed: int, n_rel: int, n_bins: int) -> int:
    if n_fixed not in (1, 2):
        raise HipLibraryError(f"edge_embed classes: {n_fixed} fixed-mask values (a 0/1 mask has one or two)")
    return (4 if n_fixed == 2 else 1) * n_rel * (n_bins + 1)


def edge_embed_class_row(fa: int, fb: int, d: int, bin_: int, n_rel: int, n_bins: int) -> int:
    return ((fa * 2 + fb) * n_rel + d) * (n_bins + 1) + (bin_ + 1)


def edge_embed_class_of_row(r: int, n_rel: int, n_bins: int):
    q, b1 = divmod(r, n_bins + 1)
    c, d = divmod(q, n_rel)
    return c >> 1, c & 1, d, b1 - 1


def edge_embed_classes_eligible(mode: str, arith: str, one_timestep: bool, n_fixed, mask_is_01: bool, n_rel: int, n_bins: int,
                                B: int, N: int, R: int = EE_CLASS_R) -> bool:
    if mode not in ("auto", "0", "1"):
        raise ValueError(f"S2S_EE_CLASSES={mode!r}: expected auto, 0 or 1")
    if mode == "0" or arith != "f16x3" or not one_timestep or n_fixed not in (1, 2) or not mask_is_01:
        return False
    rows = edge_embed_class_rows(n_fixed, n_rel, n_bins)
    if rows * 168 * 4 >= 2 ** 32:
        return False
    return mode == "1" or rows * R <= B * N * N


def edge_embed_classes_f16x3(node_a2, node_b2, fixed_cls, rel_table, bin_table, bin_lower, residue_idx, ca, wstream, b2, b3, gamma, beta,
                             mask, rel_offset: int, ln_eps=1e-5, out=None, proj=None, out_layout: str = "rowmajor"):
    lib = load_library()
    B, N = fixed_cls.shape
    n_fixed, n_rel, n_bins = node_a2.numel() // 128, rel_table.shape[1], bin_table.shape[1]
    if node_b2.numel() != n_fixed * 128 or rel_table.shape[0] != 32 or bin_table.shape[0] != 32:
        raise HipLibraryError("edge_embed_classes_f16x3: operands are not [n_fixed,128] / column-blocked [32, rows, 4]")
    rows = edge_embed_class_rows(n_fixed, n_rel, n_bins)
    _req_all(node_a2=node_a2, node_b2=node_b2, rel_table=rel_table, bin_table=bin_table, bin_lower=bin_lower, ca=ca, b2=b2, b3=b3, gamma=gamma,
             beta=beta)
    _req(residue_idx, torch.int64, "residue_idx"); _req(fixed_cls, torch.int32, "fixed_cls")
    if tuple(residue_idx.shape) != (B, N) or ca.numel() != B * N * 3:
        raise HipLibraryError("edge_embed_classes_f16x3: residue_idx / ca do not match fixed_cls [B, N]")
    dev = node_a2.device
    pw, pb, pbias, ppz = _proj_outputs(proj, B, N, dev, torch.int16, "wstream")
    wstream = _req(wstream, torch.int16, "wstream") if proj is None else pw
    if wstream.numel() * 2 != (5 if proj is not None else 4) * 32 * 1024:
        raise HipLibraryError("s2s_edge_embed_classes_f16x3: weight stream has the wrong number of stages")
    _req_opt(mask=mask)
    if out_layout not in ("rowmajor", "tiled"):
        raise HipLibraryError(f"edge_embed_classes_f16x3: out_layout {out_layout!r}")
    tiled = out_layout == "tiled"
    if out is None:
        out = PairTiled(B, N, dev) if tiled else torch.empty(B, N, N, 128, device=dev, dtype=torch.float32)
    elif isinstance(out, PairTiled) != tiled:
        raise HipLibraryError("edge_embed_classes_f16x3: out does not have the requested layout")
    table = torch.empty(rows, 168 if proj is not None else 128, device=dev, dtype=torch.float32)

    def launch():
        rc = lib.s2s_edge_embed_classes_f16x3(_p(node_a2), _p(node_b2), _p(rel_table), _p(bin_table), _p(wstream), _p(b2), _p(b3), _p(gamma),
                                              _p(beta), _p(table), n_fixed, n_rel, n_bins, ln_eps, _p(pb), _p(range_flag()), _stream())
        return rc or lib.s2s_edge_embed_expand(_p(table), _p(fixed_cls), _p(bin_lower), _p(residue_idx), _p(ca), _p(mask), _p(pb),
                                               _p(out.buf if tiled else out), 1 if tiled else 0, _p(pbias), _p(ppz), B, N, int(rel_offset),
                                               n_rel, n_bins, _stream())

    _check(_timed("s2s_edge_embed", launch), "s2s_edge_embed_classes_f16x3 / s2s_edge_embed_expand")
    return out if proj is None else (out, pbias, ppz)


def pair_project(edge, wp, bias64, attn_bias=None, pair_z=None):
    lib = load_library()
    B, N = edge.shape[0], edge.shape[1]
    _req(edge, name="edge"); _req(wp, name="wp"); _req(bias64, name="bias64")
    attn_bias = torch.empty(B, 8, N, N, device=edge.device, dtype=torch.float32) if attn_bias is None else attn_bias
    pair_z = torch.empty(B, N, N, 32, device=edge.device, dtype=torch.float32) if pair_z is None else pair_z
    _check(lib.s2s_pair_project(_p(edge), _p(wp), _p(bias64), _p(attn_bias), _p(pair_z), B, N, _stream()), "s2s_pair_project")
    return attn_bias, pair_z
```

str2str_amd/ops/torch_ops.py:

```python
import torch

from .attention import encoder_attention, ipa_attention, ipa_attention_f16, ipa_prep_points, ipa_prep_points_f16
from .binding import _opt_int
from .geometry import forward_marginal, frames_to_backbone, rigid_compose_update, rigid_scale_trans, se3_step, torsion_head
from .node import (embed_assemble, ipa_projections, node_chain, node_linear, node_linear_f32, node_linear_multi, node_linear_vfrag, pack_planes,
                   row_layernorm)
from .packing import PairTiled
from .pair import edge_embed, edge_embed_classes_f16x3, edge_embed_f16x3, edge_transition, edge_transition_f16x3, pair_project

_registered = False


def _ln3(g, b, eps):
    return None if g is None else (g, b, eps)


def _op_node_linear(xp, wpk, bias, n_rows, k_in, n_out, tiles, pre_scale=None, relu=False, pre_mask=None, residual=None, ln_gamma=None,
                    ln_beta=None, ln_eps=0.0, post_mask=None, out_f32=None, out_col0=0, want_f32=True, out_xp=None, out_xp_k=-1,
                    out_xp_k0=0, want_xp=False, map_pad=0, map_src=0):
    return node_linear(xp, wpk, bias, n_rows, k_in, n_out, tiles, pre_scale=pre_scale, relu=relu, pre_mask=pre_mask, residual=residual,
                       ln=_ln3(ln_gamma, ln_beta, ln_eps), post_mask=post_mask, out_f32=out_f32, out_col0=out_col0, want_f32=want_f32,
                       out_xp=out_xp, out_xp_k=_opt_int(out_xp_k), out_xp_k0=out_xp_k0, want_xp=want_xp,
                       row_map=(map_pad, map_src) if map_pad else None)


def _op_node_linear_f32(x, wpk32, bias, n_rows, k_in, n_out, tiles, pre_scale=None, relu=False, pre_mask=None, residual=None, ln_gamma=None,
                        ln_beta=None, ln_eps=0.0, post_mask=None, out=None, out_col0=0):
    return node_linear_f32(x, wpk32, bias, n_rows, k_in, n_out, tiles, pre_scale=pre_scale, relu=relu, pre_mask=pre_mask,
                           residual=residual, ln=_ln3(ln_gamma, ln_beta, ln_eps), post_mask=post_mask, out=out, out_col0=out_col0)


def _op_edge_transition_f16x3_chain(edge, in_tiled, B, N, node_ab, node_p, wstream, b2, gamma, beta, mask, ln_eps, proj_bias64,
                                    out_layout, prescale_exp=0, ab_kernel_form=False):
    e = PairTiled(B, N, buf=edge) if in_tiled else edge
    r = edge_transition_f16x3(e, node_ab, node_p, wstream, b2, gamma, beta, mask, ln_eps,
                              proj=None if proj_bias64 is None else (wstream, proj_bias64), out_layout=out_layout, prescale_exp=prescale_exp,
                              ab_kernel_form=ab_kernel_form)
    z, bias, pz = r if proj_bias64 is not None else (r, None, None)
    return (z.buf if isinstance(z, PairTiled) else z), bias, pz


_TORCH_OPS = {
    "edge_transition(Tensor edge, Tensor node_ab, Tensor node_p, Tensor w1p, Tensor w2p, Tensor wfp, Tensor b2, "
    "Tensor bf, Tensor gamma, Tensor beta, Tensor? mask, float ln_eps) -> Tensor": lambda *a: edge_transition(*a),
    "edge_transition_f16x3(Tensor edge, Tensor node_ab, Tensor node_p, Tensor wstream, Tensor b2, "
    "Tensor gamma, Tensor beta, Tensor? mask, float ln_eps, int prescale_exp=0) -> Tensor":
        lambda e, nab, np_, ws, b2, g, b, m, eps, pe=0: edge_transition_f16x3(e, nab, np_, ws, b2, g, b, m, eps, prescale_exp=pe),
    "edge_transition_f16x3_chain(Tensor edge, bool in_tiled, int B, int N, Tensor node_ab, Tensor node_p, Tensor wstream, Tensor b2, "
    "Tensor gamma, Tensor beta, Tensor? mask, float ln_eps, Tensor? proj_bias64, str out_layout, int prescale_exp=0, "
    "bool ab_kernel_form=False) -> (Tensor?, Tensor?, Tensor?)": _op_edge_transition_f16x3_chain,
    "edge_embed(Tensor node_a, Tensor node_b, Tensor rel_table, Tensor bin_table, Tensor bin_lower, Tensor residue_idx, Tensor ca, "
    "Tensor w2p, Tensor w3p, Tensor b2, Tensor b3, Tensor gamma, Tensor beta, Tensor? mask, int rel_offset, float ln_eps) -> Tensor":
        lambda *a: edge_embed(*a),
    "edge_embed_f16x3(Tensor node_a, Tensor node_b, Tensor rel_table, Tensor bin_table, Tensor bin_lower, Tensor residue_idx, Tensor ca, "
    "Tensor wstream, Tensor b2, Tensor b3, Tensor gamma, Tensor beta, Tensor? mask, int rel_offset, float ln_eps) -> Tensor":
        lambda *a: edge_embed_f16x3(*a),
    "edge_embed_classes_f16x3(Tensor node_a2, Tensor node_b2, Tensor fixed_cls, Tensor rel_table, Tensor bin_table, Tensor bin_lower, "
    "Tensor residue_idx, Tensor ca, Tensor wstream, Tensor b2, Tensor b3, Tensor gamma, Tensor beta, Tensor? mask, int rel_offset, "
    "float ln_eps) -> Tensor": lambda *a: edge_embed_classes_f16x3(*a),
    "pair_project(Tensor edge, Tensor wp, Tensor bias64) -> (Tensor, Tensor)": lambda *a: pair_project(*a),
    "ipa_prep_points(Tensor rigids7, Tensor q_pts_lin, Tensor kv_pts_lin, int n_heads=8, int n_qk=8, int n_v=12) -> (Tensor, Tensor, Tensor)":
        lambda *a: ipa_prep_points(*a),
    "ipa_attention(Tensor q, Tensor kv, Tensor q_pts, Tensor k_pts, Tensor v_pts, Tensor attn_bias, Tensor pair_z, "
    "Tensor mask, Tensor rigids7, Tensor head_w) -> Tensor": lambda *a: ipa_attention(*a),
    "ipa_prep_points_f16(Tensor rigids7, Tensor q_pts_lin, Tensor kv_pts_lin, Tensor head_w, int n_heads=8, int n_qk=8, int n_v=12, "
    "int c_hidden=256) -> (Tensor, Tensor, Tensor, Tensor, Tensor)": lambda *a: ipa_prep_points_f16(*a),
    "ipa_prep_points_shared_kv(Tensor rigids7, Tensor q_pts_lin, Tensor kv_pts_lin, Tensor head_w, Tensor s_xp, int n_heads=8, int n_qk=8, "
    "int n_v=12, int c_hidden=256) -> (Tensor, Tensor, Tensor, Tensor, Tensor, Tensor?, Tensor)":
        lambda r7, qp, kvp, hw, s_xp, h=8, nq=8, nv=12, c=256: ipa_prep_points_f16(r7, qp, kvp, hw, h, nq, nv, c, s_xp),
    "ipa_attention_f16w(Tensor q_xp, Tensor k_xp, Tensor v_vf, Tensor qp_xp, Tensor kp_xp, Tensor vp_vf, Tensor q2, Tensor k2, "
    "Tensor(a!) attn_bias, Tensor pair_z, Tensor mask, Tensor rigids7, int n_heads=8, int c_hidden=256, int n_qk=8, int n_v=12, int c_pz=32, "
    "float inf=1e5, float eps=1e-8, bool logits_inplace=False) -> (Tensor, Tensor)":
        lambda q, k, v, qp, kp, vp, q2, k2, ab, pz, m, r7, *rest: ipa_attention_f16(q, k, v, (qp, kp, vp, q2, k2), ab, pz, m, r7, *rest),
    "encoder_attention(Tensor qkv, Tensor? key_bias, int n_samples, int n_res, int n_heads=4, bool want_f32=False, bool want_xp=True, "
    "str arith='f32') -> (Tensor?, Tensor?)": lambda *a: encoder_attention(*a),
    "node_linear(Tensor xp, Tensor wpk, Tensor? bias, int n_rows, int k_in, int n_out, int tiles, Tensor? pre_scale=None, bool relu=False, "
    "Tensor? pre_mask=None, Tensor? residual=None, Tensor? ln_gamma=None, Tensor? ln_beta=None, float ln_eps=0.0, Tensor? post_mask=None, "
    "Tensor(a!)? out_f32=None, int out_col0=0, bool want_f32=True, Tensor(b!)? out_xp=None, int out_xp_k=-1, int out_xp_k0=0, "
    "bool want_xp=False, int map_pad=0, int map_src=0) -> (Tensor?, Tensor?)": _op_node_linear,
    "node_linear_f32(Tensor x, Tensor wpk32, Tensor? bias, int n_rows, int k_in, int n_out, int tiles, Tensor? pre_scale=None, "
    "bool relu=False, Tensor? pre_mask=None, Tensor? residual=None, Tensor? ln_gamma=None, Tensor? ln_beta=None, float ln_eps=0.0, "
    "Tensor? post_mask=None, Tensor(a!)? out=None, int out_col0=0) -> Tensor": _op_node_linear_f32,
    "node_linear_vfrag(Tensor xp, Tensor wpk, Tensor? bias, int n_rows, int k_in, int n_out, int tiles_per_head=8, int map_pad=0, "
    "int map_src=0) -> Tensor":
        lambda xp, w, b, m, k, n, tph=8, mp=0, ms=0: node_linear_vfrag(xp, w, b, m, k, n, tph, row_map=(mp, ms) if mp else None),
    "ipa_projections(Tensor s_xp, Tensor[] q, Tensor[] k, Tensor[] v, Tensor[] qp, Tensor[] kvp, int[] dims, int n_rows, int n_rows_padded, "
    "int map_pad=0, int map_src=0) -> (Tensor, Tensor?, Tensor?, Tensor, Tensor)":
        lambda s_xp, q, k, v, qp, kvp, dims, m, mo, mp=0, ms=0: ipa_projections(
            s_xp, *[({"w": t[0], "b": t[1], "k": dims[3 * i], "n": dims[3 * i + 1], "tg": dims[3 * i + 2]} if len(t) else None)
                    for i, t in enumerate((q, k, v, qp, kvp))],
            m, mo, (mp, ms) if mp else None),
    "embed_assemble(Tensor t_img, Tensor node_const, Tensor fa, Tensor fb, int n_samples, int n_res, bool planes, bool b_col_blocked) "
    "-> (Tensor, Tensor, Tensor)": lambda *a: embed_assemble(*a),
    "node_linear_multi(Tensor xp, Tensor[] w, Tensor[] bias, Tensor[] pre_scale, int[] dims, Tensor(a!)[] out_f32, Tensor(b!)[] out_xp) -> ()":
        lambda *a: node_linear_multi(*a),
    "node_chain(Tensor xp, Tensor[] w_row, Tensor[] bias, bool[] relu, int n_rows, int width, Tensor? pre_mask=None, Tensor? residual=None, "
    "Tensor? ln_gamma=None, Tensor? ln_beta=None, float ln_eps=0.0, Tensor? post_mask=None, Tensor(a!)? out_f32=None, int out_col0=0, "
    "bool want_f32=True, Tensor(b!)? out_xp=None, int out_xp_k=-1, int out_xp_k0=0, bool want_xp=False, int k_in0=-1, "
    "Tensor? mid_residual=None, Tensor(c!)? mid_out_f32=None, Tensor? mid_ln_gamma=None, Tensor? mid_ln_beta=None, float mid_ln_eps=0.0) "
    "-> (Tensor?, Tensor?)":
        lambda xp, w, b, r, m, wd, pm=None, res=None, g=None, be=None, eps=0.0, pom=None, of=None, oc=0, wf=True, ox=None, ok=-1, ok0=0, wx=False,
        k0=-1, mr=None, mo=None, mg=None, mb=None, me=0.0: node_chain(
            xp, w, b, r, m, wd, pm, res, g, be, eps, pom, of, oc, wf, ox, _opt_int(ok), ok0, wx, _opt_int(k0), mr, mo, _ln3(mg, mb, me)),
    "row_layernorm(Tensor x, int n_rows, int n_cols, Tensor gamma, Tensor beta, float eps, Tensor? post_mask=None, Tensor(a!)? out_f32=None, "
    "int out_col0=0, bool want_f32=True, Tensor(b!)? out_xp=None, int out_xp_k=-1, int out_xp_k0=0, bool want_xp=False) -> (Tensor?, Tensor?)":
        lambda x, m, n, g, b, eps, pm=None, of=None, oc=0, wf=True, ox=None, ok=-1, ok0=0, wx=False: row_layernorm(
            x, m, n, g, b, eps, pm, of, oc, wf, ox, _opt_int(ok), ok0, wx),
    "pack_planes(Tensor x, int col0=0, int n_cols=-1, Tensor(a!)? out=None, int out_k=-1, int k0=0, Tensor? row_scale=None) -> Tensor":
        lambda x, c0=0, nc=-1, out=None, ok=-1, k0=0, rs=None: pack_planes(x, c0, _opt_int(nc), out, _opt_int(ok), k0, rs),
    "se3_step(Tensor x0_7, Tensor xt_7, Tensor mask, Tensor diffuse_mask, Tensor params8, float dt) -> Tensor":
        lambda x0, xt, m, dm, p8, dt: se3_step(x0, xt, m, dm, p8, dt)[0],
    "forward_marginal(Tensor? rigids0_4x4, Tensor z_axis, Tensor u01, Tensor z_trans, Tensor cdf_rows, Tensor row_of_sample, "
    "Tensor omega_grid, Tensor? params2, Tensor? diffuse_mask=None, float coordinate_scaling=0.1) -> Tensor":
        lambda *a: forward_marginal(*a),
    "rigid_compose_update(Tensor rigids7, Tensor update6, Tensor mask) -> Tensor": lambda *a: rigid_compose_update(*a),
    "rigid_scale_trans(Tensor rigids7, float scale, bool divide=False) -> Tensor": lambda *a: rigid_scale_trans(*a),
    "torsion_head(Tensor u, int n_rows, bool normalize=True, float eps=1e-8, Tensor? gt_sin_cos=None, Tensor? fixed_mask=None) -> Tensor":
        lambda *a: torsion_head(*a),
    "frames_to_backbone(Tensor rigids7, Tensor psi, Tensor? aatype) -> Tensor": lambda r, p, a: frames_to_backbone(r, p, a)[0],
}


def register_torch_ops():
    global _registered
    if _registered:
        return
    lib = torch.library.Library("str2str_amd", "DEF")
    impl = torch.library.Library("str2str_amd", "IMPL", "CUDA")
    for schema, fn in _TORCH_OPS.items():
        lib.define(schema)
        impl.impl(schema.split("(")[0], fn)
    register_torch_ops._libs = (lib, impl)
    _registered = True
```

Baseline: 31.37 conformations/s.

## Feed edge transition from class table and per-pair index instead of expanded pair tensor

When the edge embedding collapses to a small set of classes, the embed now writes only a per-pair int class index (or -1 for masked pairs) plus a compact class table, not the full B×N×N×128 fp32 pair tensor. The first edge transition gathers each pair's 128-float input row from the table through the index. This removes a large write and re-read of the expanded pair tensor. In exchange it adds an indexed gather that depends on cache hits, a new kernel variant, and a fallback path that materialises the full tensor when the fused projection is absent.

```diff
diff --git a/str2str_amd/build.py b/str2str_amd/build.py
--- a/str2str_amd/build.py
+++ b/str2str_amd/build.py
@@ -39,6 +39,7 @@
     "pair_mlp_f16_b.hip": ["-mllvm", "-pragma-unroll-threshold=10000000", "-fno-slp-vectorize"],
     "pair_mlp_f16_c.hip": ["-mllvm", "-pragma-unroll-threshold=10000000", "-fno-slp-vectorize"],
     "pair_mlp_f16_d.hip": ["-mllvm", "-pragma-unroll-threshold=10000000", "-fno-slp-vectorize"],
+    "pair_mlp_f16_e.hip": ["-mllvm", "-pragma-unroll-threshold=10000000", "-fno-slp-vectorize"],
     "pair_embed_expand.hip": [],
     "ipa_attention.hip": ["-mllvm", "-pragma-unroll-threshold=10000000"],
     "ipa_attention_f16w.hip": ["-mllvm", "-pragma-unroll-threshold=10000000", "-fno-slp-vectorize"],
diff --git a/str2str_amd/csrc/pair_embed_expand.hip b/str2str_amd/csrc/pair_embed_expand.hip
--- a/str2str_amd/csrc/pair_embed_expand.hip
+++ b/str2str_amd/csrc/pair_embed_expand.hip
@@ -9,13 +9,13 @@
 
 typedef float f32x4 __attribute__((ext_vector_type(4)));
 
-template <bool PROJ>
+template <bool PROJ, bool REC168 = PROJ>
 __global__ void __launch_bounds__(256) edge_embed_expand_kernel(
     const float* __restrict__ table, const int* __restrict__ fixed_cls, const float* __restrict__ bin_lower,
     const long long* __restrict__ residue_idx, const float* __restrict__ ca, const float* __restrict__ mask,
     const float* __restrict__ proj_b, float* __restrict__ out, float* __restrict__ attn_bias, float* __restrict__ pair_z,
     long long M, int N, int rel_off, int n_rel, int n_bins, int out_tiled) {
-    constexpr unsigned kRec = PROJ ? s2s::kEeRecProj : s2s::kEeRecPlain;
+    constexpr unsigned kRec = REC168 ? s2s::kEeRecProj : s2s::kEeRecPlain;
     __shared__ __attribute__((aligned(16))) float s_bins[s2s::kEeBinSlots];
     const unsigned lane = threadIdx.x & 63, h = lane >> 5, wave = threadIdx.x >> 6;
     s2s::ee_fill_bins(s_bins, bin_lower, n_bins);
@@ -33,7 +33,9 @@
     const float em = mask ? __fmul_rn(mask[bi], mask[bj]) : 1.0f;
     const float* rec = table + (unsigned long long)row * kRec;
 
-    if (out_tiled) {
+    if (out_tiled == 2) {
+        if (valid && h == 0) reinterpret_cast<int*>(out)[p] = em == 0.f ? -1 : (int)row;
+    } else if (out_tiled) {
         float* o = out + (unsigned long long)(p0 >> 5) * 4096u + lane * 4u;
         f32x4 v[16];
 #pragma unroll
@@ -98,7 +100,7 @@
                                      float* proj_attn_bias, float* proj_pair_z, int n_samples, int n_res, int rel_offset, int n_rel,
                                      int n_bins, void* stream) {
     if (n_samples <= 0 || n_res <= 0) return 0;
-    if (n_bins < 1 || n_bins > 32 || (out_tiled & ~1) || n_rel < 1) return (int)hipErrorInvalidValue;
+    if (n_bins < 1 || n_bins > 32 || out_tiled < 0 || out_tiled > 2 || n_rel < 1) return (int)hipErrorInvalidValue;
     if ((proj_attn_bias != nullptr) != (proj_pair_z != nullptr) || (proj_attn_bias && !proj_bias_cat64)) return (int)hipErrorInvalidValue;
     const long long NN = (long long)n_res * n_res;
     if (NN >= (1ll << 31)) return (int)hipErrorInvalidValue;
@@ -106,20 +108,25 @@
     long long cap = cap_env ? atoll(cap_env) : 0;
     if (cap <= 0 || cap > (1ll << 31) - 1) cap = (1ll << 31) - 1;
     long long chunk = cap / NN;
-    if (out_tiled && chunk < n_samples) chunk -= chunk % tile_aligned_samples(NN);
+    if (out_tiled == 1 && chunk < n_samples) chunk -= chunk % tile_aligned_samples(NN);
     if (chunk < 1) return (int)hipErrorInvalidValue;
     for (long long b0 = 0; b0 < n_samples; b0 += chunk) {
         const long long nb = n_samples - b0 < chunk ? n_samples - b0 : chunk;
         const long long M = nb * NN, rows0 = b0 * n_res;
         const unsigned grid = (unsigned)((M + 127) / 128);
         const float* mk = mask ? mask + rows0 : nullptr;
+        float* o = out + (out_tiled == 2 ? b0 * NN : b0 * NN * 128);
         if (proj_attn_bias)
             hipLaunchKernelGGL(edge_embed_expand_kernel<true>, dim3(grid), dim3(256), 0, (hipStream_t)stream, table, fixed_cls + rows0,
-                               bin_lower, residue_idx + rows0, ca_xyz + rows0 * 3, mk, proj_bias_cat64, out + b0 * NN * 128, proj_attn_bias + b0 * 8 * NN,
+                               bin_lower, residue_idx + rows0, ca_xyz + rows0 * 3, mk, proj_bias_cat64, o, proj_attn_bias + b0 * 8 * NN,
                                proj_pair_z + b0 * NN * 32, M, n_res, rel_offset, n_rel, n_bins, out_tiled);
+        else if (proj_bias_cat64)
+            hipLaunchKernelGGL((edge_embed_expand_kernel<false, true>), dim3(grid), dim3(256), 0, (hipStream_t)stream, table, fixed_cls + rows0,
+                               bin_lower, residue_idx + rows0, ca_xyz + rows0 * 3, mk, (const float*)nullptr, o, (float*)nullptr,
+                               (float*)nullptr, M, n_res, rel_offset, n_rel, n_bins, out_tiled);
         else
             hipLaunchKernelGGL(edge_embed_expand_kernel<false>, dim3(grid), dim3(256), 0, (hipStream_t)stream, table, fixed_cls + rows0,
-                               bin_lower, residue_idx + rows0, ca_xyz + rows0 * 3, mk, (const float*)nullptr, out + b0 * NN * 128, (float*)nullptr,
+                               bin_lower, residue_idx + rows0, ca_xyz + rows0 * 3, mk, (const float*)nullptr, o, (float*)nullptr,
                                (float*)nullptr, M, n_res, rel_offset, n_rel, n_bins, out_tiled);
     }
     return (int)hipGetLastError();
diff --git a/str2str_amd/csrc/pair_mlp_f16.hip b/str2str_amd/csrc/pair_mlp_f16.hip
--- a/str2str_amd/csrc/pair_mlp_f16.hip
+++ b/str2str_amd/csrc/pair_mlp_f16.hip
@@ -43,13 +43,14 @@
 __device__ float s2s_one[1] = {1.0f};
 
 
-template <bool PROJ, bool STAGE>
+template <bool PROJ, bool STAGE, bool BYCLS = false>
 __global__ void __launch_bounds__(256) edge_transition_f16_kernel(
     const float* __restrict__ edge, const float* __restrict__ node_ab, const float* __restrict__ node_p,
     const char* __restrict__ wblob, const float* __restrict__ b2,
     const float* __restrict__ gamma, const float* __restrict__ beta, const float* __restrict__ mask,
     float* __restrict__ out, long long M, int N, float ln_eps, int io_layout, unsigned mask_stride, const float* __restrict__ proj_b,
-    float* __restrict__ proj_bias_out, float* __restrict__ proj_pz_out, int* __restrict__ range_flag, float sk) {
+    float* __restrict__ proj_bias_out, float* __restrict__ proj_pz_out, int* __restrict__ range_flag, float sk,
+    const int* __restrict__ cls_idx) {
     constexpr int kStages = kStagesBase + (PROJ ? 1 : 0);
     constexpr int kSlots = 8 * kStages;
     constexpr int kRing = PROJ ? 4 : 2, kAhead = PROJ ? 2 : 1;
@@ -155,6 +156,27 @@
         const f32x4 v = __builtin_nontemporal_load(reinterpret_cast<const f32x4*>(r + g * in_step));
         return make_float4(v.x, v.y, v.z, v.w);
     };
+#ifndef S2S_ET_CLS_NT
+#define S2S_ET_CLS_NT 0
+#endif
+#ifndef S2S_ET_CLS_SLOT
+#define S2S_ET_CLS_SLOT 200
+#endif
+    const unsigned cls_rec = (io_layout & 16) ? s2s::kEeRecProj : s2s::kEeRecPlain;
+    auto cls_pair = [&](long long wg_tile) -> unsigned {
+        const unsigned p = ((unsigned)wg_tile * 4u + (unsigned)wave) * 32u + ((unsigned)lane & 31u);
+        return p < (unsigned)M ? p : (unsigned)M - 1u;
+    };
+    auto cls_off = [&](int cls) -> unsigned { return ((unsigned)(cls + 1) * cls_rec + 4u * (unsigned)h) * 4u; };
+    auto ldrow_cls = [&](unsigned off, int g) -> float4 {
+        const f32x4* q = reinterpret_cast<const f32x4*>(reinterpret_cast<const char*>(edge) + off + 32 * g);
+#if S2S_ET_CLS_NT
+        const f32x4 v = __builtin_nontemporal_load(q);
+#else
+        const f32x4 v = *q;
+#endif
+        return make_float4(v.x, v.y, v.z, v.w);
+    };
     const long long n_wt = (M + 127) / 128;
     long long wt = blockIdx.x;
     PairCtx cur = setup(wt);
@@ -167,8 +189,14 @@
     };
     {
         float4 xv[16];
-#pragma unroll
-        for (int i = 0; i < 16; ++i) xv[i] = ldrow(erow_of(cur), i);
+        if constexpr (BYCLS) {
+            const unsigned off = cls_off(cls_idx[cur.p]);
+#pragma unroll
+            for (int i = 0; i < 16; ++i) xv[i] = ldrow_cls(off, i);
+        } else {
+#pragma unroll
+            for (int i = 0; i < 16; ++i) xv[i] = ldrow(erow_of(cur), i);
+        }
         for (int i = threadIdx.x; i < 768; i += 256)
             s_vec[i] = i < 384 ? sk * b2[i] : (i < 512 ? 0.f : (i < 640 ? gamma[i - 512] : beta[i - 640]));
         if (PROJ && threadIdx.x < 64) s_vec[768 + threadIdx.x] = proj_b[threadIdx.x];
@@ -330,6 +358,7 @@
     bool has_next = false;
     PairCtx nxt = cur;
     float4 xv[16];
+    unsigned ncls = 0;
     f16x8 xpn[8][2];
     f16x8 xq[8][2];
     auto slot = [&](auto sc) {
@@ -351,14 +380,21 @@
             fetch(st_next & (kRing - 1), 0, fr[(ns + 1) & 1]);
         }
         constexpr int kXv0 = 208;
+        if constexpr (BYCLS && s == S2S_ET_CLS_SLOT) ncls = (unsigned)cls_idx[cls_pair(has_next ? wt_next : wt)];
+        if constexpr (BYCLS && s == kXv0 + 1) ncls = cls_off((int)ncls);
         if constexpr (s == kXv0) nxt = setup(has_next ? wt_next : wt);
         if constexpr (s == kXv0 + 3) stage_load(nxt);
         if constexpr (s == kXv0 + 8) stage_store();
         if constexpr (s > kXv0 && s <= kXv0 + 16 && ((s & 3) == 1 || (s & 3) == 2)) {
             constexpr int i = 4 * ((s - kXv0) / 4) + 2 * ((s & 3) - 1);
-            const float* er = erow_of(nxt);
-            xv[i] = ldrow(er, i);
-            xv[i + 1] = ldrow(er, i + 1);
+            if constexpr (BYCLS) {
+                xv[i] = ldrow_cls(ncls, i);
+                xv[i + 1] = ldrow_cls(ncls, i + 1);
+            } else {
+                const float* er = erow_of(nxt);
+                xv[i] = ldrow(er, i);
+                xv[i + 1] = ldrow(er, i + 1);
+            }
         }
         if constexpr (s == 236) seeds_load(nxt, 0);
         if constexpr (s == 237) { seedc_piece(nxt, 0, 0); seedc_piece(nxt, 0, 1); seedc_piece(nxt, 0, 2); seedc_piece(nxt, 0, 3); }
@@ -873,13 +909,14 @@
     return n_cu;
 }
 
-template <bool STAGE>
+template <bool STAGE, bool BYCLS = false>
 int et_launch(const float* edge, const float* node_ab, const float* node_p, const void* weight_stream, const float* b2,
               const float* ln_gamma, const float* ln_beta, const float* mask, float* out, int n_samples, int n_res, float ln_eps,
               int io_layout, const float* proj_bias_cat64, float* proj_attn_bias, float* proj_pair_z, int prescale_exp, int* range_words,
               void* stream) {
     if (n_samples <= 0 || n_res <= 0) return 0;
-    if ((io_layout & ~7) || ((io_layout & 4) && !proj_attn_bias) || (!(io_layout & 4) && !out)) return (int)hipErrorInvalidValue;
+    if ((io_layout & ~31) || ((io_layout & 4) && !proj_attn_bias) || (!(io_layout & 4) && !out)) return (int)hipErrorInvalidValue;
+    if (BYCLS != ((io_layout & 8) != 0) || (BYCLS ? ((io_layout & 1) || !proj_attn_bias) : (io_layout & 16) != 0)) return (int)hipErrorInvalidValue;
     if (prescale_exp < 0 || prescale_exp > 15) return (int)hipErrorInvalidValue;
     const float sk = ldexpf(1.0f, -prescale_exp);
     const long long NN = (long long)n_res * n_res;
@@ -897,22 +934,25 @@
         const long long M = nb * NN, rows0 = b0 * n_res;
         const long long wg_tiles = (M + 127) / 128;
         const long long grid = wg_tiles < n_cu ? wg_tiles : n_cu;
-        const float* e = edge + b0 * NN * 128;
+        const long long m32 = ((long long)n_samples * NN + 31) / 32 * 32;
+        const float* e = BYCLS ? edge + m32 : edge + b0 * NN * 128;
+        const int* ci = BYCLS ? reinterpret_cast<const int*>(edge) + b0 * NN : nullptr;
         const float* nab = node_ab + rows0 * 896;
         const float* np = node_p + rows0 * 128;
         const float* mk = mask ? mask + rows0 : one;
         const unsigned mks = mask ? 1u : 0u;
         float* o = out ? out + b0 * NN * 128 : nullptr;
-        auto k_proj = &edge_transition_f16_kernel<true, STAGE>;
-        auto k_plain = &edge_transition_f16_kernel<false, STAGE>;
-        if (proj_attn_bias)
+        auto k_proj = &edge_transition_f16_kernel<true, STAGE, BYCLS>;
+        if (proj_attn_bias) {
             hipLaunchKernelGGL(k_proj, dim3((unsigned)grid), dim3(256), 0, (hipStream_t)stream, e, nab, np,
                                (const char*)weight_stream, b2, ln_gamma, ln_beta, mk, o, M, n_res, ln_eps, io_layout, mks, proj_bias_cat64,
-                               proj_attn_bias + b0 * 8 * NN, proj_pair_z + b0 * NN * 32, range_words, sk);
-        else
+                               proj_attn_bias + b0 * 8 * NN, proj_pair_z + b0 * NN * 32, range_words, sk, ci);
+        } else if constexpr (!BYCLS) {
+            auto k_plain = &edge_transition_f16_kernel<false, STAGE>;
             hipLaunchKernelGGL(k_plain, dim3((unsigned)grid), dim3(256), 0, (hipStream_t)stream, e, nab, np,
                                (const char*)weight_stream, b2, ln_gamma, ln_beta, mk, o, M, n_res, ln_eps, io_layout, mks,
-                               (const float*)nullptr, (float*)nullptr, (float*)nullptr, range_words, sk);
+                               (const float*)nullptr, (float*)nullptr, (float*)nullptr, range_words, sk, (const int*)nullptr);
+        }
     }
     return (int)hipGetLastError();
 }
@@ -929,8 +969,15 @@
 #if S2S_PM_PART == 2
 extern "C" int s2s_et_f16x3_short_chains(S2S_ET_ARGS) { return et_launch<false>(S2S_ET_PASS); }
 #endif
+extern "C" __attribute__((visibility("hidden"))) int s2s_et_f16x3_by_class(S2S_ET_ARGS);
+#if S2S_PM_PART == 5
+extern "C" int s2s_et_f16x3_by_class(S2S_ET_ARGS) {
+    return n_res >= 32 ? et_launch<true, true>(S2S_ET_PASS) : et_launch<false, true>(S2S_ET_PASS);
+}
+#endif
 #if S2S_PM_PART == 1
 extern "C" int s2s_edge_transition_f16x3(S2S_ET_ARGS) {
+    if (io_layout & 8) return s2s_et_f16x3_by_class(S2S_ET_PASS);
     return n_res >= 32 ? et_launch<true>(S2S_ET_PASS) : s2s_et_f16x3_short_chains(S2S_ET_PASS);
 }
 #endif
diff --git a/str2str_amd/csrc/pair_mlp_f16_e.hip b/str2str_amd/csrc/pair_mlp_f16_e.hip
--- /dev/null
+++ b/str2str_amd/csrc/pair_mlp_f16_e.hip
@@ -0,0 +1,2 @@
+#define S2S_PM_PART 5
+#include "pair_mlp_f16.hip"
diff --git a/str2str_amd/models/net/denoising_ipa.py b/str2str_amd/models/net/denoising_ipa.py
--- a/str2str_amd/models/net/denoising_ipa.py
+++ b/str2str_amd/models/net/denoising_ipa.py
@@ -37,7 +37,7 @@
 
 class EmbeddingModule(nn.Module):
     launch_switches = ("arith", "node_arith")
-    launch_modes = ("ee_classes",)
+    launch_modes = ("ee_classes", "et_by_class")
 
     def __init__(self, init_embed_size: int, node_embed_size: int, edge_embed_size: int, num_bins: int = 22,
                  min_bin: float = 1e-5, max_bin: float = 20.0, self_conditioning: bool = True):
@@ -65,6 +65,9 @@
         self.ee_classes = os.environ.get("S2S_EE_CLASSES", "auto")
         if self.ee_classes not in ("auto", "0", "1"):
             raise ValueError(f"S2S_EE_CLASSES={self.ee_classes!r}: expected auto, 0 or 1")
+        self.et_by_class = os.environ.get("S2S_ET_BY_CLASS", "auto")
+        if self.et_by_class not in ("auto", "0", "1"):
+            raise ValueError(f"S2S_ET_BY_CLASS={self.et_by_class!r}: expected auto, 0 or 1")
         self._mask01_cache = DerivedCache()
 
     def _weights(self):
@@ -205,6 +208,8 @@
             by_class = cls is not None and ops.edge_embed_classes_eligible(
                 self.ee_classes, self.arith, single_t and not per_sample, cls["n_fixed"], self._mask_is_01(node_mask), rel_cb.shape[1],
                 w["bin_tab_cb"].shape[1], B, L)
+            if edge_layout == "by_class" and not (by_class and next_proj is not None):
+                edge_layout = "tiled"
             if by_class:
                 _, node_a2, node_b2 = torch.ops.str2str_amd.embed_assemble(img.contiguous(), cls["nc2"], cls["fa2"], cls["fb2"], 1,
                                                                            cls["n_fixed"], False, True)
@@ -260,7 +265,7 @@
         node_embed, node_act, edge_embed, first_proj = self.embedder.embed(
             residue_idx=batch["residue_idx"], t=batch["t"], fixed_mask=fixed_mask, self_conditioning_ca=batch["sc_ca_t"], node_mask=node_mask,
             t_emb=batch.get("t_emb"), t_img=batch.get("t_img"), next_proj=self.translator.trunk["ipa_0"].pair_proj_weights() if fuse else None,
-            **({"edge_layout": "tiled"} if tiled else {}))
+            **({"edge_layout": "by_class" if getattr(self.embedder, "et_by_class", "0") != "0" else "tiled"} if tiled else {}))
         tb = dict(batch)
         tb["residue_mask"], tb["fixed_mask"] = node_mask, fixed_mask
         tb["rigids_t"] = batch["rigids_t"].to(dev)
diff --git a/str2str_amd/models/net/ipa.py b/str2str_amd/models/net/ipa.py
--- a/str2str_amd/models/net/ipa.py
+++ b/str2str_amd/models/net/ipa.py
@@ -262,6 +262,9 @@
         init7 = batch["rigids_t"].type(torch.float).contiguous()
         curr7 = torch.ops.str2str_amd.rigid_scale_trans(init7, self.coordinate_scaling, False)
         proj = _first_proj
+        if isinstance(edge_embed, ops.PairByClass) and not (_first_proj is not None and self.fuse_pair_projection and self.num_blocks > 1
+                                                             and T["edge_transition_0"].arith == "f16x3"):
+            edge_embed = ops.pair_untiled(edge_embed)
 
         def lin(x, w, **kw):
             return ops.node_apply(x, w, M, **kw)
diff --git a/str2str_amd/models/net/layers.py b/str2str_amd/models/net/layers.py
--- a/str2str_amd/models/net/layers.py
+++ b/str2str_amd/models/net/layers.py
@@ -183,6 +183,8 @@
         if self._shape != (128, 128, 384, 128, 2):
             raise ops.HipLibraryError(f"EdgeTransition kernel is built for c_z=128, c_s=256 (got {self._shape})")
         mask = None if edge_mask_1d is None else edge_mask_1d.type(torch.float32).contiguous()
+        if isinstance(edge_embed, ops.PairByClass) and not (self.arith == "f16x3" and next_proj is not None):
+            edge_embed = ops.pair_untiled(edge_embed)
         if self.arith == "f16x3":
             pk = self._packed()
             proj = None
@@ -190,13 +192,13 @@
                 stream = self._proj_cache.get([pk["wstream_f16"], next_proj["wp_f16x2"]],
                                               lambda: torch.cat([pk["wstream_f16"], next_proj["wp_f16x2"]]))
                 proj = (stream, next_proj["b64"])
-            tiled_in = isinstance(edge_embed, ops.PairTiled)
+            tiled_in, cls_in = isinstance(edge_embed, ops.PairTiled), isinstance(edge_embed, ops.PairByClass)
             B, N = edge_embed.shape[0], edge_embed.shape[1]
             z, bias, pz = torch.ops.str2str_amd.edge_transition_f16x3_chain(
-                edge_embed.buf if tiled_in else edge_embed.contiguous(), tiled_in, B, N, node_ab, n_p,
+                edge_embed.buf if tiled_in or cls_in else edge_embed.contiguous(), tiled_in, B, N, node_ab, n_p,
                 pk["wstream_f16"] if proj is None else proj[0], self.trunk[2].bias, self.layer_norm.weight,
                 self.layer_norm.bias, mask, self.layer_norm.eps, None if proj is None else proj[1], out_layout, int(self.prescale_exp),
-                bool(ab_kernel_form))
+                bool(ab_kernel_form), **({"in_rec": edge_embed.rec} if cls_in else {}))
             if out_layout == "tiled":
                 z = ops.PairTiled(B, N, buf=z)
             return z if proj is None else (z, bias, pz)
diff --git a/str2str_amd/ops/__init__.py b/str2str_amd/ops/__init__.py
--- a/str2str_amd/ops/__init__.py
+++ b/str2str_amd/ops/__init__.py
@@ -11,7 +11,7 @@
 from .node import (CHAIN_WIDTHS, NARROW_MAX_WORK, SMALL_ROWS, embed_assemble, ipa_projections, node_apply,
                    node_apply_chain, node_apply_multi, node_chain, node_linear, node_linear_f32, node_linear_multi, node_linear_vfrag,
                    pack_planes, row_layernorm, small_rows_variant, to_act)
-from .packing import (NODE_TG, LazyDict, PairTiled, act_alloc, column_blocked, fragment_order, node_tiles, pack_f16x2_layer, pack_f16x3_embed_stream,
+from .packing import (NODE_TG, LazyDict, PairByClass, PairTiled, act_alloc, column_blocked, fragment_order, node_tiles, pack_f16x2_layer, pack_f16x3_embed_stream,
                       pack_f16x3_stream, pack_node_layer, pack_node_weight, pack_node_weight_f32, pack_weight, padded_len, pair_tiled,
                       pair_untiled, unpack_planes, vf_alloc, xp_alloc)
 from .pair import (EE_CLASS_R, edge_embed, edge_embed_class_of_row, edge_embed_class_row, edge_embed_class_rows, edge_embed_classes_eligible,
@@ -23,7 +23,7 @@
 __all__ = [
     "ABI_VERSION", "EXPORTS", "LIB_PATH", "HipLibraryError", "KernelTimer", "WeightRangeError", "load_library",
     "RANGE_BITS", "RANGE_FAMILIES", "range_families", "range_flag", "range_flag_names", "range_flag_read", "range_flag_reset", "range_headroom",
-    "NODE_TG", "LazyDict", "PairTiled", "act_alloc", "column_blocked", "fragment_order", "node_tiles", "pack_f16x2_layer", "pack_f16x3_embed_stream",
+    "NODE_TG", "LazyDict", "PairByClass", "PairTiled", "act_alloc", "column_blocked", "fragment_order", "node_tiles", "pack_f16x2_layer", "pack_f16x3_embed_stream",
     "pack_f16x3_stream", "pack_node_layer", "pack_node_weight", "pack_node_weight_f32", "pack_weight", "padded_len", "pair_tiled", "pair_untiled",
     "unpack_planes", "vf_alloc", "xp_alloc",
     "edge_embed", "edge_embed_f16x3", "edge_transition", "edge_transition_f16x3", "pair_project",
diff --git a/str2str_amd/ops/packing.py b/str2str_amd/ops/packing.py
--- a/str2str_amd/ops/packing.py
+++ b/str2str_amd/ops/packing.py
@@ -84,6 +84,32 @@
         return self
 
 
+class PairByClass:
+    __slots__ = ("buf", "B", "N", "rec", "expand")
+
+    def __init__(self, B: int, N: int, buf: torch.Tensor, rec: int, expand=None):
+        self.B, self.N, self.rec, self.buf, self.expand = int(B), int(N), int(rec), buf, expand
+        if self.rec not in (128, 168) or buf.dtype != torch.float32 or buf.ndim != 1 or not buf.is_contiguous() or (buf.numel() - self.M32) % self.rec:
+            raise HipLibraryError("PairByClass: buffer must be a flat contiguous fp32 tensor of M32 index words and records of 128 or 168 floats")
+
+    @staticmethod
+    def index_words(B: int, N: int) -> int:
+        return -(-(int(B) * int(N) * int(N)) // 32) * 32
+
+    M32 = property(lambda self: self.index_words(self.B, self.N))
+    shape = property(lambda self: (self.B, self.N, self.N, 128))
+    device = property(lambda self: self.buf.device)
+    is_cuda = property(lambda self: self.buf.is_cuda)
+    index = property(lambda self: self.buf[:self.B * self.N * self.N].view(torch.int32).view(self.B, self.N, self.N))
+    records = property(lambda self: self.buf[self.M32:].view(-1, self.rec))
+
+    def data_ptr(self):
+        return self.buf.data_ptr()
+
+    def contiguous(self):
+        return self
+
+
 def pair_tiled(z: torch.Tensor) -> PairTiled:
     B, N = z.shape[0], z.shape[1]
     M = B * N * N
@@ -94,7 +120,11 @@
     return t
 
 
-def pair_untiled(t: PairTiled) -> torch.Tensor:
+def pair_untiled(t) -> torch.Tensor:
+    if isinstance(t, PairByClass):
+        if t.expand is None:
+            raise HipLibraryError("pair_untiled: this PairByClass does not come from edge_embed_classes_f16x3 (no expansion to materialise it with)")
+        return t.expand()
     M = t.B * t.N * t.N
     return t.buf.view(-1, 16, 2, 32, 4).permute(0, 3, 1, 2, 4).reshape(-1, 128)[:M].reshape(t.B, t.N, t.N, 128).contiguous()
 
diff --git a/str2str_amd/ops/pair.py b/str2str_amd/ops/pair.py
--- a/str2str_amd/ops/pair.py
+++ b/str2str_amd/ops/pair.py
@@ -1,7 +1,7 @@
 import torch
 
 from .binding import HipLibraryError, _check, _p, _req, _req_all, _req_opt, _stream, _timed, load_library
-from .packing import PairTiled, column_blocked
+from .packing import PairByClass, PairTiled, column_blocked
 from .range_guard import range_flag
 
 
@@ -17,7 +17,9 @@
                           out_layout: str = "rowmajor", prescale_exp: int = 0, ab_kernel_form: bool = False):
     lib = load_library()
     B, N = edge.shape[0], edge.shape[1]
-    in_tiled = isinstance(edge, PairTiled)
+    in_tiled, in_cls = isinstance(edge, PairTiled), isinstance(edge, PairByClass)
+    if in_cls and proj is None:
+        raise HipLibraryError("edge_transition_f16x3: a PairByClass input needs the fused projection (proj); pair_untiled materialises it")
     if not 0 <= int(prescale_exp) <= 15:
         raise HipLibraryError(f"edge_transition_f16x3: prescale_exp {prescale_exp} outside 0 .. 15")
     if tuple(edge.shape) != (B, N, N, 128) or tuple(node_ab.shape) != (B, N, 896) or tuple(node_p.shape) != (B, N, 128):
@@ -34,7 +36,7 @@
             node_ab[..., 768:] -= node_ab[..., 768:].mean(dim=-1, keepdim=True)
     if out_layout not in ("rowmajor", "tiled", "none") or (out_layout == "none" and proj is None):
         raise HipLibraryError(f"edge_transition_f16x3: out_layout {out_layout!r}" + (" needs proj" if out_layout == "none" else ""))
-    _req(edge.buf if in_tiled else edge, name="edge")
+    _req(edge.buf if in_tiled or in_cls else edge, name="edge")
     _req_all(node_ab=node_ab, node_p=node_p, b2=b2, gamma=gamma, beta=beta)
     pw, pb, pbias, ppz = _proj_outputs(proj, B, N, edge.device, torch.int16, "wstream")
     wstream = _req(wstream, torch.int16, "wstream") if proj is None else pw
@@ -49,9 +51,9 @@
         raise HipLibraryError("edge_transition: out may not alias edge")
     elif isinstance(out, PairTiled) != (out_layout == "tiled"):
         raise HipLibraryError("edge_transition_f16x3: out does not have the requested layout")
-    io = (1 if in_tiled else 0) | {"rowmajor": 0, "tiled": 2, "none": 4}[out_layout]
+    io = (1 if in_tiled else 0) | {"rowmajor": 0, "tiled": 2, "none": 4}[out_layout] | ((8 | (16 if edge.rec == 168 else 0)) if in_cls else 0)
     _check(_timed("s2s_edge_transition", lambda: lib.s2s_edge_transition_f16x3(
-        _p(edge.buf if in_tiled else edge), _p(node_ab), _p(node_p), _p(wstream), _p(b2), _p(gamma), _p(beta), _p(mask),
+        _p(edge.buf if in_tiled or in_cls else edge), _p(node_ab), _p(node_p), _p(wstream), _p(b2), _p(gamma), _p(beta), _p(mask),
         _p(out.buf if isinstance(out, PairTiled) else out), B, N, ln_eps, io, _p(pb), _p(pbias), _p(ppz), int(prescale_exp), _p(range_flag()),
         _stream())), "s2s_edge_transition_f16x3")
     return out if proj is None else (out, pbias, ppz)
@@ -173,23 +175,41 @@
     if wstream.numel() * 2 != (5 if proj is not None else 4) * 32 * 1024:
         raise HipLibraryError("s2s_edge_embed_classes_f16x3: weight stream has the wrong number of stages")
     _req_opt(mask=mask)
-    if out_layout not in ("rowmajor", "tiled"):
-        raise HipLibraryError(f"edge_embed_classes_f16x3: out_layout {out_layout!r}")
-    tiled = out_layout == "tiled"
-    if out is None:
-        out = PairTiled(B, N, dev) if tiled else torch.empty(B, N, N, 128, device=dev, dtype=torch.float32)
-    elif isinstance(out, PairTiled) != tiled:
-        raise HipLibraryError("edge_embed_classes_f16x3: out does not have the requested layout")
-    table = torch.empty(rows, 168 if proj is not None else 128, device=dev, dtype=torch.float32)
+    if out_layout not in ("rowmajor", "tiled", "by_class") or (out_layout == "by_class" and out is not None):
+        raise HipLibraryError(f"edge_embed_classes_f16x3: out_layout {out_layout!r}" + (" takes no out" if out is not None else ""))
+    by_cls = out_layout == "by_class"
+
+    def pair_out(out, tiled):
+        if out is None:
+            out = PairTiled(B, N, dev) if tiled else torch.empty(B, N, N, 128, device=dev, dtype=torch.float32)
+        elif isinstance(out, PairTiled) != tiled:
+            raise HipLibraryError("edge_embed_classes_f16x3: out does not have the requested layout")
+        return out
+
+    def expand(z, mode, pbias, ppz):
+        return lib.s2s_edge_embed_expand(_p(table), _p(fixed_cls), _p(bin_lower), _p(residue_idx), _p(ca), _p(mask), _p(pb), _p(z), mode,
+                                         _p(pbias), _p(ppz), B, N, int(rel_offset), n_rel, n_bins, _stream())
+
+    if not by_cls:
+        out = pair_out(out, out_layout == "tiled")
+    rec, m32 = 168 if proj is not None else 128, PairByClass.index_words(B, N) if by_cls else 0
+    buf = torch.empty(m32 + (rows + (1 if by_cls else 0)) * rec, device=dev, dtype=torch.float32)
+    table = buf[m32 + (rec if by_cls else 0):].view(rows, rec)
 
     def launch():
         rc = lib.s2s_edge_embed_classes_f16x3(_p(node_a2), _p(node_b2), _p(rel_table), _p(bin_table), _p(wstream), _p(b2), _p(b3), _p(gamma),
                                               _p(beta), _p(table), n_fixed, n_rel, n_bins, ln_eps, _p(pb), _p(range_flag()), _stream())
-        return rc or lib.s2s_edge_embed_expand(_p(table), _p(fixed_cls), _p(bin_lower), _p(residue_idx), _p(ca), _p(mask), _p(pb),
-                                               _p(out.buf if tiled else out), 1 if tiled else 0, _p(pbias), _p(ppz), B, N, int(rel_offset),
-                                               n_rel, n_bins, _stream())
+        if by_cls:
+            buf[m32:m32 + rec].zero_()
+        return rc or (expand(buf, 2, pbias, ppz) if by_cls else expand(out.buf if out_layout == "tiled" else out, 1 if out_layout == "tiled" else 0, pbias, ppz))
 
     _check(_timed("s2s_edge_embed", launch), "s2s_edge_embed_classes_f16x3 / s2s_edge_embed_expand")
+    if by_cls:
+        def materialise():
+            z = pair_out(None, False)
+            _check(expand(z, 0, None, None), "s2s_edge_embed_expand")
+            return z
+        out = PairByClass(B, N, buf, rec, expand=materialise)
     return out if proj is None else (out, pbias, ppz)
 
 
diff --git a/str2str_amd/ops/torch_ops.py b/str2str_amd/ops/torch_ops.py
--- a/str2str_amd/ops/torch_ops.py
+++ b/str2str_amd/ops/torch_ops.py
@@ -5,7 +5,7 @@
 from .geometry import forward_marginal, frames_to_backbone, rigid_compose_update, rigid_scale_trans, se3_step, torsion_head
 from .node import (embed_assemble, ipa_projections, node_chain, node_linear, node_linear_f32, node_linear_multi, node_linear_vfrag, pack_planes,
                    row_layernorm)
-from .packing import PairTiled
+from .packing import PairByClass, PairTiled
 from .pair import edge_embed, edge_embed_classes_f16x3, edge_embed_f16x3, edge_transition, edge_transition_f16x3, pair_project
 
 _registered = False
@@ -31,8 +31,8 @@
 
 
 def _op_edge_transition_f16x3_chain(edge, in_tiled, B, N, node_ab, node_p, wstream, b2, gamma, beta, mask, ln_eps, proj_bias64,
-                                    out_layout, prescale_exp=0, ab_kernel_form=False):
-    e = PairTiled(B, N, buf=edge) if in_tiled else edge
+                                    out_layout, prescale_exp=0, ab_kernel_form=False, in_rec=0):
+    e = PairByClass(B, N, edge, in_rec) if in_rec else (PairTiled(B, N, buf=edge) if in_tiled else edge)
     r = edge_transition_f16x3(e, node_ab, node_p, wstream, b2, gamma, beta, mask, ln_eps,
                               proj=None if proj_bias64 is None else (wstream, proj_bias64), out_layout=out_layout, prescale_exp=prescale_exp,
                               ab_kernel_form=ab_kernel_form)
@@ -48,7 +48,7 @@
         lambda e, nab, np_, ws, b2, g, b, m, eps, pe=0: edge_transition_f16x3(e, nab, np_, ws, b2, g, b, m, eps, prescale_exp=pe),
     "edge_transition_f16x3_chain(Tensor edge, bool in_tiled, int B, int N, Tensor node_ab, Tensor node_p, Tensor wstream, Tensor b2, "
     "Tensor gamma, Tensor beta, Tensor? mask, float ln_eps, Tensor? proj_bias64, str out_layout, int prescale_exp=0, "
-    "bool ab_kernel_form=False) -> (Tensor?, Tensor?, Tensor?)": _op_edge_transition_f16x3_chain,
+    "bool ab_kernel_form=False, int in_rec=0) -> (Tensor?, Tensor?, Tensor?)": _op_edge_transition_f16x3_chain,
     "edge_embed(Tensor node_a, Tensor node_b, Tensor rel_table, Tensor bin_table, Tensor bin_lower, Tensor residue_idx, Tensor ca, "
     "Tensor w2p, Tensor w3p, Tensor b2, Tensor b3, Tensor gamma, Tensor beta, Tensor? mask, int rel_offset, float ln_eps) -> Tensor":
         lambda *a: edge_embed(*a),
```

Measured after the change: 31.89 conformations/s, median of 6. 1.02x the previous value.
